# Alan-404/Conformer

Hardware: AMD Instinct MI355X
Metric: encoder audio-frames/sec (B=32,T=1000,d=512,L=16) (higher is better)
Workload: dtype f32; 1 GPU; cfg2 Conformer-L Encoder.forward: B=32/GPU, T=1000 mel frames (T'=249), d=512, 16 blocks, 8 heads, k=31, fp32, eval, random-init weights, batch-sharded replicas; per_gpu_batch=32, mel_frames=1000

## Files before the change

conformer_amd/_lib.py:

```python
from __future__ import annotations

import ctypes
import os
from ctypes import c_char_p, c_float, c_int, c_int64, c_uint64, c_void_p

_HERE = os.path.dirname(os.path.abspath(__file__))
LIB_PATH = os.environ.get("CONFORMER_AMD_LIB") or os.path.join(_HERE, "lib", "libconformer_hip.so")

_P, _I, _L, _F, _U = c_void_p, c_int, c_int64, c_float, c_uint64
ABI_VERSION = 4

SIGNATURES = {
    "cfm_version": (c_int, []),
    "cfm_abi_version": (c_int, []),
    "cfm_gemm_bias_stats_f32": (c_int, [_P, _P, _P, _P, _P, _L, _I, _I, _L, _L, _P]),
    "cfm_gemm_bias_residual_stats_f32": (c_int, [_P, _P, _P, _P, _F, _P, _P, _L, _I, _I, _L, _L, _L, _P]),
    "cfm_gemm_splitk_f32": (c_int, [_I, _P, _P, _P, _P, _F, _P, _P, _I, _L, _I, _I, _L, _L, _L, _P]),
    "cfm_gemm_lnfold_f32": (c_int, [_I, _P, _P, _I, _F, _P, _P, _P, _P, _L, _I, _I, _L, _L, _P]),
    "cfm_layernorm_fwd_stats_f32": (c_int, [_P, _P, _P, _P, _P, _L, _I, _F, _P]),
    "cfm_ffn_pack_elems": (ctypes.c_int64, [_I, _I]),
    "cfm_ffn_pack_f32": (c_int, [_P, _P, _P, _I, _I, _P]),
    "cfm_rowgemm_pack_f32": (c_int, [_P, _P, _I, _I, _I, _P]),
    "cfm_rowchain_f32": (c_int, [_I, _I, _I, _I, _P, _L, _P, _P, _P, _L, _P, _L, _P, _I, _F, _P, _P, _P, _P, _F, _I, _P, _L, _P, _P, _P, _F,
                                 _P, _P, _P, _F, _P, _L, _L, _I, _P]),
    "cfm_ffn_tile_stride_f4": (ctypes.c_int64, [_I]),
    "cfm_ffn_rotate": (c_int, []),
    "cfm_ffn_fused_f32": (c_int, [_P, _L, _P, _I, _F, _P, _P, _P, _P, _F, _P, _L, _I, _P, _P, _P, _F, _L, _I, _I, _P]),
    "cfm_strerror": (c_char_p, [_I]),
    "cfm_device_check": (c_int, []),
    "cfm_subsampled_length": (c_int64, [_L]),
    "cfm_subsampled_lengths_i64": (c_int, [_P, _P, _I, _P]),
    "cfm_layernorm_fwd_f32": (c_int, [_P, _P, _P, _P, _P, _P, _L, _I, _F, _P]),
    "cfm_gemm_bias_f32": (c_int, [_P, _P, _P, _P, _L, _I, _I, _L, _L, _P]),
    "cfm_gemm_bias_swish_f32": (c_int, [_P, _P, _P, _P, _L, _I, _I, _L, _L, _P]),
    "cfm_gemm_bias_relu_f32": (c_int, [_P, _P, _P, _P, _L, _I, _I, _L, _L, _P]),
    "cfm_gemm_bias_glu_f32": (c_int, [_P, _P, _P, _P, _L, _I, _I, _L, _L, _P]),
    "cfm_gemm_bias_residual_f32": (c_int, [_P, _P, _P, _P, _F, _P, _L, _I, _I, _L, _L, _L, _P]),
    "cfm_gemm_mfma16_f32": (c_int, [_I, _I, _P, _I, _P, _I, _P, _P, _F, _P, _I, _P, _I, _L, _I, _I, _L, _L, _L, _F, _U, _P]),
    "cfm_layernorm_fwd_out16_f32": (c_int, [_I, _P, _P, _P, _P, _P, _P, _L, _I, _F, _P]),
    "cfm_cast16_f32": (c_int, [_I, _P, _P, _L, _P]),
    "cfm_cast16_multi_f32": (c_int, [_I, _P, _I, _P]),
    "cfm_relpos_attention_mfma16_f32": (c_int, [_I, _P, _P, _P, _L, _P, _L, _P, _P, _P, _P, _L, _P, _I, _I, _I, _I, _F, _U, _P]),
    "cfm_relpos_attention_rows_mfma16_f32": (c_int, [_I, _P, _P, _P, _L, _P, _L, _P, _P, _P, _P, _L, _I, _I, _I, _I, _I, _I, _P]),
    "cfm_relpos_attention_io16_mfma16_f32": (c_int, [_I, _P, _P, _P, _I, _L, _P, _L, _P, _P, _P, _P, _I, _L, _I, _I, _I, _I, _P]),
    "cfm_subsample_conv2_relu_mfma16_f32": (c_int, [_I, _P, _I, _P, _I, _P, _P, _I, _I, _I, _I, _I, _P]),
    "cfm_subsample_conv1_relu_out16_f32": (c_int, [_I, _P, _P, _P, _P, _I, _I, _I, _I, _P]),
    "cfm_gemm_bwd_batched_mfma16_f32": (c_int, [_I, _P, _I, _L, _P, _I, _I, _L, _P, _I, _L, _F, _P, _L, _I, _I, _I, _L, _I, _I, _I, _I,
                                                _L, _L, _L, _L, _L, _L, _F, _U, _I, _P]),
    "cfm_subsample_conv2_bwd_weight_mfma16_f32": (c_int, [_I, _P, _P, _P, _I, _I, _I, _I, _P]),
    "cfm_subsample_conv2_bwd_input_mfma16_f32": (c_int, [_I, _P, _P, _P, _I, _I, _I, _I, _P]),
    "cfm_subsample_conv2_rowtab_elems": (ctypes.c_int64, [_I, _I, _I]),
    "cfm_subsample_conv2_bwd_weight_h16_mfma16_f32": (c_int, [_I, _P, _I, _P, _P, _P, _P, _I, _I, _I, _I, _P]),
    "cfm_relu_bwd_out16_f32": (c_int, [_I, _P, _P, _P, _L, _P]),
    "cfm_dwconv_bn_swish_fwd_out16_f32": (c_int, [_I, _P, _P, _P, _P, _P, _P, _P, _F, _P, _I, _I, _I, _I, _P]),
    "cfm_glu_bwd_out16_f32": (c_int, [_I, _P, _P, _P, _L, _I, _P]),
    "cfm_subsample_conv2_bwd_input_fwdkernel_mfma16_f32": (c_int, [_I, _P, _I, _P, _P, _P, _I, _I, _I, _I, _P]),
    "cfm_subsample_conv2_bwd_input_fwdkernel_out16_mfma16_f32": (c_int, [_I, _P, _I, _P, _P, _P, _I, _I, _I, _I, _P]),
    "cfm_subsample_conv1_bwd_d16_f32": (c_int, [_I, _P, _P, _P, _P, _P, _P, _I, _I, _I, _I, _P]),
    "cfm_reflect_pad_f32": (c_int, [_P, _P, _I, _L, _I, _L, _P]),
    "cfm_power_mel_log_f32": (c_int, [_P, _L, _P, _P, _I, _I, _I, _I, _F, _P]),
    "cfm_power_mel_log_mfma_f32": (c_int, [_P, _L, _P, _P, _I, _I, _I, _I, _I, _F, _P]),
    "cfm_dft_frames_f32": (c_int, [_P, _P, _P, _L, _I, _I, _I, _P]),
    "cfm_specaugment_apply_f32": (c_int, [_P, _I, _I, _I, _P, _I, _F, _P]),
    "cfm_gemm_bias_swish_save_f32": (c_int, [_P, _P, _P, _P, _P, _L, _I, _I, _L, _L, _P]),
    "cfm_gemm_bwd_f32": (c_int, [_P, _I, _L, _P, _I, _L, _P, _L, _F, _P, _L, _I, _I, _L, _I, _P]),
    "cfm_gemm_bwd_batched_f32": (c_int, [_P, _I, _L, _P, _I, _L, _P, _L, _F, _P, _L, _I, _I, _L, _I, _I, _I, _I,
                                         _L, _L, _L, _L, _L, _L, _F, _U, _P]),
    "cfm_gemm_train_f32": (c_int, [_I, _P, _P, _P, _P, _F, _P, _P, _L, _I, _I, _L, _L, _L, _F, _U, _P]),
    "cfm_relpos_attention_train_f32": (c_int, [_P, _P, _P, _L, _P, _L, _P, _P, _P, _P, _L, _P, _I, _I, _I, _I, _F, _U, _P]),
    "cfm_dropout_f32": (c_int, [_P, _P, _L, _F, _U, _P]),
    "cfm_dropout_out16_f32": (c_int, [_I, _P, _P, _L, _F, _U, _P]),
    "cfm_layernorm_bwd_dx_f32": (c_int, [_P, _P, _P, _P, _P, _P, _P, _L, _I, _P]),
    "cfm_layernorm_bwd_params_f32": (c_int, [_P, _P, _P, _P, _P, _P, _L, _I, _P]),
    "cfm_layernorm_bwd_f32": (c_int, [_P, _P, _P, _P, _P, _P, _P, _P, _P, _L, _I, _P, ctypes.c_size_t, _P]),
    "cfm_layernorm_bwd_workspace_bytes": (ctypes.c_size_t, [_L, _I]),
    "cfm_colsum_f32": (c_int, [_P, _L, _L, _I, _F, _P, _P]),
    "cfm_glu_fwd_f32": (c_int, [_P, _P, _L, _I, _P]),
    "cfm_glu_bwd_f32": (c_int, [_P, _P, _P, _L, _I, _P]),
    "cfm_dwconv_bn_swish_bwd_f32": (c_int, [_P, _P, _P, _P, _P, _P, _P, _P, _F, _I, _P, _P, _P, _P, _P, _P,
                                            _I, _I, _I, _I, _P]),
    "cfm_dwconv_bn_stats_workspace_bytes": (ctypes.c_size_t, [_I, _I, _I]),
    "cfm_dwconv_bn_stats_f32": (c_int, [_P, _P, _P, _P, _P, _P, _P, _F, _I, _I, _I, _I, _P, ctypes.c_size_t, _P]),
    "cfm_debug_attention_bwd_trace_f32": (c_int, [_P]),
    "cfm_debug_attention_bwd_trace_mfma16": (c_int, [_P]),
    "cfm_debug_gemm_mfma16_trace": (c_int, [_P]),
    "cfm_debug_gemm_mfma16_force_tile": (c_int, [_I]),
    "cfm_debug_gemm_last_tile": (c_int, [_I, _P]),
    "cfm_relpos_attention_bwd_mfma16_f32": (c_int, [_I, _P, _P, _P, _L, _P, _L, _P, _P, _P, _P, _P, _L, _P, _P, _P, _P, _L, _P, _L,
                                                    _P, _P, _I, _I, _I, _I, _F, _U, _P]),
    "cfm_relpos_attention_bwd_f32": (c_int, [_P, _P, _P, _L, _P, _L, _P, _P, _P, _P, _P, _L, _P, _P, _P, _P, _L, _P, _L, _P, _P,
                                             _I, _I, _I, _I, _F, _U, _I, _P]),
    "cfm_relu_bwd_f32": (c_int, [_P, _P, _P, _L, _P]),
    "cfm_subsample_conv2_bwd_weight_f32": (c_int, [_P, _P, _P, _I, _I, _I, _I, _P]),
    "cfm_pack_conv2_weight_t_f32": (c_int, [_P, _P, _I, _P]),
    "cfm_subsample_conv2_bwd_input_f32": (c_int, [_P, _P, _P, _I, _I, _I, _I, _P]),
    "cfm_subsample_conv1_bwd_f32": (c_int, [_P, _P, _P, _P, _P, _P, _I, _I, _I, _I, _P]),
    "cfm_adam_step_f32": (c_int, [_P, _I, _F, _F, _F, _F, _F, _F, _P]),
    "cfm_greedy_ctc_decode_f32": (c_int, [_P, _P, _P, _P, _P, _I, _I, _I, _I, _I, _P]),
    "cfm_ctc_beam_workspace_bytes": (ctypes.c_size_t, [_I, _I, _I, _I]),
    "cfm_ctc_beam_decode_f32": (c_int, [_P, _P, _I, _I, _I, _I, _I, _I, _F, _F, _I, _P, ctypes.c_size_t, _P, _P, _P, _P, _P]),
    "cfm_ngram_lm_pack_bytes": (ctypes.c_size_t, [_I, _P, _I, _L, _I, _L]),
    "cfm_ngram_lm_pack": (c_int, [_I, _P, _P, _P, _P, _I, _P, _P, _I, _I, _I, _I, _P, _P, _P, _P, ctypes.c_size_t]),
    "cfm_ngram_lm_score_f64": (c_int, [_P, _P, _P, _I, _I, _P, _P]),
    "cfm_ctc_beam_lm_workspace_bytes": (ctypes.c_size_t, [_I, _I, _I, _I]),
    "cfm_ctc_beam_lm_decode_f32": (c_int, [_P, _P, _I, _I, _I, _I, _I, _I, _F, _F, _I, _P, ctypes.c_double, ctypes.c_double,
                                           ctypes.c_double, _I, _P, ctypes.c_size_t, _P, _P, _P, _P, _P, _P]),
    "cfm_hotword_pack_bytes": (ctypes.c_size_t, [_I, _L, _I, _L, _I, _L]),
    "cfm_hotword_pack": (c_int, [_I, _P, _P, _I, _P, _P, _I, _P, _P, _P, _P, ctypes.c_size_t]),
    "cfm_hotword_count": (c_int, [_P, _P, _P, _I, ctypes.c_double, _P, _P, _P]),
    "cfm_ctc_beam_hw_workspace_bytes": (ctypes.c_size_t, [_I, _I, _I, _I]),
    "cfm_ctc_beam_hw_decode_f32": (c_int, [_P, _P, _I, _I, _I, _I, _I, _I, _F, _F, _I, _P, ctypes.c_double, ctypes.c_double,
                                           ctypes.c_double, _I, _P, ctypes.c_double, _P, ctypes.c_size_t, _P, _P, _P, _P, _P,
                                           _P]),
    "cfm_ctc_beam_stream_state_bytes": (ctypes.c_size_t, [_I, _I, _I, _I, _I, _I]),
    "cfm_ctc_beam_stream_init": (c_int, [_I, _I, _I, _I, _P, _I, _P, _P, ctypes.c_size_t, _P]),
    "cfm_ctc_beam_stream_step_f32": (c_int, [_P, _P, _I, _I, _I, _I, _I, _I, _F, _F, _I, _P, ctypes.c_double, ctypes.c_double,
                                             ctypes.c_double, _I, _P, ctypes.c_double, _P, ctypes.c_size_t, _I, _I, _P, _P, _P,
                                             _P, _P, _P]),
    "cfm_ctc_beam_stream_finish_f32": (c_int, [_I, _I, _I, _I, _P, ctypes.c_double, ctypes.c_double, ctypes.c_double, _I, _P,
                                               ctypes.c_double, _P, ctypes.c_size_t, _I, _P, _P, _P, _P, _P, _P]),
    "cfm_ctc_beam_stream_reset_slots": (c_int, [_I, _I, _I, _I, _P, _I, _P, _P, _I, _P, ctypes.c_size_t, _P]),
    "cfm_lstm_fwd_carry_f32": (c_int, [_P, _P, _P, _P, _P, _P, _P, _P, _I, _I, _I, _P]),
    "cfm_lstm_fwd_frag_carry_f32": (c_int, [_P, _P, _P, _P, _P, _P, _P, _P, _P, _I, _I, _I, _P]),
    "cfm_lstm_fwd_mfma16_carry_f32": (c_int, [_I, _P, _P, _P, _P, _P, _P, _P, _P, _P, _I, _I, _I, _P]),
    "cfm_lstm_fwd_f32": (c_int, [_P, _P, _P, _P, _P, _P, _P, _I, _I, _I, _P]),
    "cfm_lstm_fwd_frag_f32": (c_int, [_P, _P, _P, _P, _P, _P, _P, _P, _I, _I, _I, _P]),
    "cfm_lstm_bwd_frag_f32": (c_int, [_P, _P, _P, _P, _P, _P, _P, _P, _I, _I, _I, _P]),
    "cfm_debug_lstm_trace": (c_int, [_P]),
    "cfm_debug_dw16_trace": (c_int, [_P]),
    "cfm_linear_bwd_weight_mfma16_f32": (c_int, [_I, _P, _I, _L, _P, _I, _L, _P, _L, _P, _I, _I, _L, _F, _P]),
    "cfm_lstm_fwd_mfma16_f32": (c_int, [_I, _P, _P, _P, _P, _P, _P, _P, _P, _I, _I, _I, _P]),
    "cfm_lstm_bwd_mfma16_f32": (c_int, [_I, _P, _P, _P, _P, _P, _P, _P, _P, _I, _I, _I, _P]),
    "cfm_lstm_bwd_f32": (c_int, [_P, _P, _P, _P, _P, _P, _P, _I, _I, _I, _P]),
    "cfm_swish_bn_eval_f32": (c_int, [_P, _P, _P, _P, _P, _F, _P, _L, _I, _P]),
    "cfm_swish_bn_stats_f32": (c_int, [_P, _P, _P, _P, _P, _F, _L, _I, _P]),
    "cfm_swish_bn_bwd_f32": (c_int, [_P, _P, _P, _P, _P, _F, _I, _P, _P, _P, _L, _I, _P]),
    "cfm_split_pack_elems": (ctypes.c_int64, [_I, _I, _I]),
    "cfm_split_pack_bf16_f32": (c_int, [_I, _P, _P, _I, _I, _P]),
    "cfm_gemm_split_bf16_f32": (c_int, [_I, _I, _P, _P, _P, _P, _F, _P, _L, _I, _I, _L, _L, _L, _P]),
    "cfm_subsample_conv2_relu_split_bf16_f32": (c_int, [_I, _P, _P, _P, _P, _I, _I, _I, _I, _P]),
    "cfm_ctc_workspace_floats": (ctypes.c_int64, [_I, _I, _I]),
    "cfm_ctc_loss_fwd_f32": (c_int, [_P, _P, _P, _L, _L, _P, _P, _I, _I, _I, _I, _I, _P, _P, _P]),
    "cfm_ctc_loss_bwd_f32": (c_int, [_P, _P, _P, _L, _L, _P, _P, _I, _I, _I, _I, _I, _P, _P, _P, _P]),
    "cfm_ctc_align_workspace_bytes": (ctypes.c_size_t, [_I, _I, _I]),
    "cfm_ctc_align_f32": (c_int, [_P, _P, _P, _P, _I, _I, _I, _I, _I, _P, ctypes.c_size_t, _P, _P, _P, _P, _P, _P, _P, _P]),
    "cfm_relpos_attention_rows_f32": (c_int, [_P, _P, _P, _L, _P, _L, _P, _P, _P, _P, _L, _I, _I, _I, _I, _I, _I, _I, _P, _P]),
    "cfm_relpos_attention_slots_f32": (c_int, [_P, _P, _P, _L, _P, _L, _P, _P, _P, _P, _P, _P, _L, _I, _I, _I, _I, _I, _I, _P, _P]),
    "cfm_relpos_attention_slots_mfma16_f32": (c_int, [_I, _P, _P, _P, _I, _L, _P, _L, _P, _P, _P, _P, _P, _P, _L, _I, _I, _I, _I, _I, _I,
                                                      _P, _P]),
    "cfm_debug_attention_trace_f32": (c_int, [_P, _P, _P, _L, _P, _L, _P, _P, _P, _P, _L, _I, _I, _I, _I, _P, _P]),
    "cfm_debug_set_bwd_tile": (c_int, [_I]),
    "cfm_debug_set_attention_waves": (c_int, [_I]),
    "cfm_debug_gemm_cfg_f32": (c_int, [_I, _P, _P, _P, _P, _F, _P, _L, _I, _I, _P, _P]),
    "cfm_debug_set_conv2_bk": (c_int, [_I]),
    "cfm_debug_ffn_trace": (c_int, [_P, _I]),
    "cfm_debug_ffn_variant": (c_int, [_I]),
    "cfm_debug_ffn_layout": (c_int, [_I, _I]),
    "cfm_relpos_table_f32": (c_int, [_P, _P, _I, _I, _P]),
    "cfm_relpos_attention_fwd_f32": (c_int, [_P, _P, _P, _L, _P, _L, _P, _P, _P, _P, _L, _P, _I, _I, _I, _I, _P]),
    "cfm_dwconv_bn_swish_fwd_f32": (c_int, [_P, _P, _P, _P, _P, _P, _P, _F, _P, _I, _I, _I, _I, _P]),
    "cfm_convmod_glu_dwconv_f32": (c_int, [_P, _L, _P, _I, _F, _P, _P, _P, _P, _P, _P, _P, _P, _P, _F, _P, _L, _I, _I, _I, _I, _P]),
    "cfm_debug_convmod_variant": (c_int, [_I]),
    "cfm_subsample_conv1_relu_f32": (c_int, [_P, _P, _P, _P, _I, _I, _I, _I, _P]),
    "cfm_pack_conv2_weight_f32": (c_int, [_P, _P, _I, _P]),
    "cfm_subsample_conv2_relu_f32": (c_int, [_P, _P, _P, _P, _I, _I, _I, _I, _P]),
    "cfm_pack_linear_weight_f32": (c_int, [_P, _P, _I, _I, _I, _P]),
    "cfm_conv2_wino_plane_elems": (c_int64, [_I, _I, _I, _I]),
    "cfm_pack_conv2_wino_weight_f32": (c_int, [_P, _P, _I, _P]),
    "cfm_subsample_conv2_wino_relu_f32": (c_int, [_P, _P, _P, _P, _P, _I, _I, _I, _I, _P]),
}


class ConformerHipError(RuntimeError):
    pass


_lib = None


def load() -> ctypes.CDLL:
    global _lib
    if _lib is not None:
        return _lib
    if not os.path.exists(LIB_PATH):
        raise ConformerHipError(
            f"{LIB_PATH} is missing: build it with `python -m conformer_amd.build` "
            "(there is no CPU/eager fallback for the Conformer hot path)")
    import torch
    lib = ctypes.CDLL(LIB_PATH, mode=ctypes.RTLD_GLOBAL)
    try:
        lib.cfm_abi_version.restype = c_int
        got = int(lib.cfm_abi_version())
    except AttributeError:
        got = 0
    if got != ABI_VERSION:
        raise ConformerHipError(f"{LIB_PATH} implements C-ABI revision {got}, this binding needs {ABI_VERSION}: rebuild it with "
                                "`python -m conformer_amd.build`")
    for name, (res, args) in SIGNATURES.items():
        fn = getattr(lib, name)
        fn.restype = res
        fn.argtypes = args
    _lib = lib
    return lib


class CastItem(ctypes.Structure):
    _fields_ = [("src", ctypes.c_void_p), ("dst", ctypes.c_void_p), ("rows", ctypes.c_int64), ("cols", ctypes.c_int64),
                ("transpose", ctypes.c_int)]


CALLS = [0]


def check(status: int, what: str) -> None:
    CALLS[0] += 1
    if status != 0:
        msg = load().cfm_strerror(status).decode()
        raise ConformerHipError(f"{what} failed: {msg} (status {status})")
```

conformer_amd/csrc/conv2_wino_f32.hip:

```cpp
#include <algorithm>
#include <utility>

#include "gemm_shared.h"

namespace {

#define WINO_MFMA_SLICE(FA, FB)                                                                             \
    _Pragma("unroll") for (int e = 0; e < 4; ++e)                                                           \
    _Pragma("unroll") for (int mt = 0; mt < TM; ++mt)                                                       \
    _Pragma("unroll") for (int nt = 0; nt < TN; ++nt)                                                       \
        acc[mt][nt] = __builtin_amdgcn_mfma_f32_32x32x2f32(FB[nt][e], FA[mt][e], acc[mt][nt], 0, 0, 0)

template <typename Fn, int... I>
__device__ __forceinline__ void static_for_seq(Fn& f, std::integer_sequence<int, I...>) {
    (f(std::integral_constant<int, I>{}), ...);
}
template <int N, typename Fn>
__device__ __forceinline__ void static_for(Fn&& f) {
    static_for_seq(f, std::make_integer_sequence<int, N>{});
}

__host__ __device__ constexpr int wino_nt(int a) { return a == 1 ? 1 : 2; }
__host__ __device__ constexpr int wino_terms(int p) { return wino_nt(p / 3) * wino_nt(p % 3); }

struct WinoArgs {
    const float* h1; const float* w; float* planes;
    int64_t M;
    unsigned h1_bytes;
    int T1, F1, C, TI, TJ, nb;
    int odd_t, odd_f;
    unsigned tiles_n;
    unsigned grp_blk[4];
    unsigned grp_tm[3][4];
    unsigned grp_pat[3];
};


template <int ST, int SF>
__device__ __forceinline__ void wino_tile(const WinoArgs& g, int p, int64_t m0, int n0, float* lds) {
    constexpr int BM = 256, BN = 256, WN = 4, TM = 4, TN = 2, BK = 16, LDSR = BK + 4, NT = ST * SF, SPC = 2 * NT;
    constexpr int NPX = (ST == 2 ? 2 : 1) * (SF == 2 ? 2 : 1);
    float* As = lds;
    float* Bs = lds + 2 * BM * LDSR;
    const int a = p / 3, b = p - 3 * (p / 3);
    const int sg_t = a >> 1, sg_f = b >> 1;

    const int tid = threadIdx.x, lane = tid & 63;
    const int wave = __builtin_amdgcn_readfirstlane(tid >> 6);
    const int wr = wave / WN, wc = wave % WN;
    const int li = lane & 31, hf = lane >> 5;

    constexpr int CPR = BK / 4, RPP = 512 / CPR, PA = BM / RPP, PB = BN / RPP;
    const int chunk = tid & (CPR - 1), srow = tid / CPR;
    unsigned row_off[PA];
    const int TJp = g.TJ - (b == 2 ? g.odd_f : 0);
    const int64_t pos_per_b = (int64_t)(g.TI - (a == 2 ? g.odd_t : 0)) * TJp, Mp = g.nb * pos_per_b;
#pragma unroll
    for (int i = 0; i < PA; ++i) {
        int64_t m = m0 + srow + RPP * i;
        if (m >= Mp) m = Mp - 1;
        const int64_t bb = m / pos_per_b;
        const int r = (int)(m - bb * pos_per_b);
        const int ib = r / TJp, jb = r - ib * TJp;
        row_off[i] = (unsigned)((((bb * g.T1 + 4 * ib) * g.F1 + 4 * jb) * (int64_t)g.C + chunk * 4) * 4);
    }
    const __amdgpu_buffer_rsrc_t h1_rsrc = __builtin_amdgcn_make_buffer_rsrc(const_cast<float*>(g.h1), (short)0, (int)g.h1_bytes, 0x00020000);
    const unsigned pix_t[3] = {(unsigned)((ST == 2 ? 4 * sg_t : 2) * g.F1 * g.C * 4), (unsigned)(2 * g.F1 * g.C * 4),
                               (unsigned)((1 + 2 * sg_t) * g.F1 * g.C * 4)};
    const unsigned pix_f[3] = {(unsigned)((SF == 2 ? 4 * sg_f : 2) * g.C * 4), (unsigned)(2 * g.C * 4), (unsigned)((1 + 2 * sg_f) * g.C * 4)};
    int64_t woff = 0;
    for (int q = 0; q < p; ++q) woff += wino_terms(q);
    const int K = NT * g.C;
    const __amdgpu_buffer_rsrc_t w_rsrc = __builtin_amdgcn_make_buffer_rsrc(const_cast<float*>(g.w + woff * g.C * g.C), (short)0,
                                                                            K * g.C * 4, 0x00020000);
    const unsigned w_off = (unsigned)(((n0 + srow) * K + chunk * 4) * 4), w_step = (unsigned)(RPP * K * 4);

    f32x4 raw[PA][NPX], rb[PB];
    auto load_tile = [&](auto U_, int c32, int half) __attribute__((always_inline)) {
        constexpr int U = decltype(U_)::value, UT = U / SF, UF = U % SF;
        constexpr int NXT = (ST == 2 && UT == 0) ? 2 : 1, NYF = (SF == 2 && UF == 0) ? 2 : 1;
        constexpr int X1 = ST == 2 ? (UT == 0 ? 0 : 2) : 0, Y1 = SF == 2 ? (UF == 0 ? 0 : 2) : 0;
        const unsigned ci4 = (unsigned)(32 * c32 + 16 * half) * 4;
#pragma unroll
        for (int x = 0; x < NXT; ++x)
#pragma unroll
            for (int y = 0; y < NYF; ++y) {
                const unsigned po = pix_t[X1 + x] + pix_f[Y1 + y] + ci4;
#pragma unroll
                for (int i = 0; i < PA; ++i)
                    raw[i][x * NYF + y] = __builtin_bit_cast(f32x4, __builtin_amdgcn_raw_buffer_load_b128(h1_rsrc, row_off[i], po, 0));
            }
        const unsigned k4 = (unsigned)(NT * 32 * c32 + 32 * U + 16 * half) * 4;
#pragma unroll
        for (int i = 0; i < PB; ++i) rb[i] = __builtin_bit_cast(f32x4, __builtin_amdgcn_raw_buffer_load_b128(w_rsrc, w_off, k4 + w_step * i, 0));
    };
    auto store_tile = [&](auto U_, int buf) __attribute__((always_inline)) {
        constexpr int U = decltype(U_)::value, UT = U / SF, UF = U % SF;
        constexpr int NXT = (ST == 2 && UT == 0) ? 2 : 1, NYF = (SF == 2 && UF == 0) ? 2 : 1;
#pragma unroll
        for (int i = 0; i < PA; ++i) {
            const f32x4* px = raw[i];
            f32x4 v;
            if constexpr (NXT == 2 && NYF == 2) v = (px[0] - px[1]) - (px[2] - px[3]);
            else if constexpr (NXT * NYF == 2) v = px[0] - px[1];
            else v = px[0];
            *reinterpret_cast<f32x4*>(As + (buf * BM + srow + RPP * i) * LDSR + chunk * 4) = v;
        }
#pragma unroll
        for (int i = 0; i < PB; ++i)
            *reinterpret_cast<f32x4*>(Bs + (buf * BN + srow + RPP * i) * LDSR + chunk * 4) = rb[i];
    };

    f32x16 acc[TM][TN];
#pragma unroll
    for (int i = 0; i < TM; ++i)
#pragma unroll
        for (int j = 0; j < TN; ++j)
#pragma unroll
            for (int r = 0; r < 16; ++r) acc[i][j][r] = 0.f;

    const int a_row = wr * (BM / 2) + li, b_row = wc * (BN / WN) + li;
    f32x4 fa0[TM], fb0[TN], fa1[TM], fb1[TN];
    auto read_frags = [&](f32x4 (&fa)[TM], f32x4 (&fb)[TN], int buf, int c) __attribute__((always_inline)) {
#pragma unroll
        for (int t = 0; t < TM; ++t)
            fa[t] = *reinterpret_cast<const f32x4*>(As + (buf * BM + a_row + 32 * t) * LDSR + 8 * c + 4 * hf);
#pragma unroll
        for (int t = 0; t < TN; ++t)
            fb[t] = *reinterpret_cast<const f32x4*>(Bs + (buf * BN + b_row + 32 * t) * LDSR + 8 * c + 4 * hf);
    };

    const int nch = g.C / 32;
    load_tile(std::integral_constant<int, 0>{}, 0, 0);
    store_tile(std::integral_constant<int, 0>{}, 0);
    load_tile(std::integral_constant<int, 0>{}, 0, 1);
    __syncthreads();
    read_frags(fa0, fb0, 0, 0);
    for (int c32 = 0; c32 < nch; ++c32) {
        static_for<SPC>([&](auto S_) __attribute__((always_inline)) {
            constexpr int S = decltype(S_)::value;
            constexpr int S1 = (S + 1) % SPC, S2 = (S + 2) % SPC;
            const int cur = S & 1;
            const bool more = S + 1 < SPC || c32 + 1 < nch;
            read_frags(fa1, fb1, cur, 1);
            __builtin_amdgcn_sched_barrier(0);
            WINO_MFMA_SLICE(fa0, fb0);
            __builtin_amdgcn_sched_barrier(0);
            if (more) store_tile(std::integral_constant<int, S1 / 2>{}, cur ^ 1);
            load_tile(std::integral_constant<int, S2 / 2>{}, S + 2 < SPC ? c32 : min(c32 + 1, nch - 1), S2 & 1);
            __syncthreads();
            if (more) read_frags(fa0, fb0, cur ^ 1, 0);
            __builtin_amdgcn_sched_barrier(0);
            WINO_MFMA_SLICE(fa1, fb1);
            __builtin_amdgcn_sched_barrier(0);
        });
    }

    __syncthreads();
    GemmArgs ge{};
    ge.C = g.planes + (int64_t)p * g.M * g.C;
    ge.M = Mp; ge.N = g.C; ge.K = K; ge.ldc = g.C; ge.alpha = 1.f;
    gemm_epilogue_rows<BM, BN, EPI_BIAS, TM, TN, 2, false, EPF_INFER | EPF_NO_BIAS, WN>(ge, acc, m0, n0, wr, wc, lane,
                                                                                        lds + wave * 32 * (32 * TN + 4));
}

__global__ __launch_bounds__(512, 2) void conv2_wino_gemm_kernel(const WinoArgs g) {
    constexpr int LDS_STAGE = 2 * (256 + 256) * 20;
    static_assert(8 * 32 * (32 * 2 + 4) <= LDS_STAGE, "the row-major epilogue scratch must fit the staging buffers");
    __shared__ __attribute__((aligned(16))) float lds[LDS_STAGE];
    const unsigned bid = blockIdx.x;
    const int grp = bid < g.grp_blk[1] ? 0 : (bid < g.grp_blk[2] ? 1 : 2);
    const unsigned local = bid - g.grp_blk[grp], per_xcd = (g.grp_blk[grp + 1] - g.grp_blk[grp]) / 8;
    unsigned tile = (local & 7u) * per_xcd + (local >> 3);
    unsigned k = 0, lo = 0;
    for (; k < 4; ++k) {
        const unsigned seg = (g.grp_tm[grp][k] - lo) * (4 - k) * g.tiles_n;
        if (tile < seg) break;
        tile -= seg;
        lo = g.grp_tm[grp][k];
    }
    if (k == 4) return;
    const unsigned tn = tile % g.tiles_n, rest = tile / g.tiles_n;
    const unsigned pi = k + rest % (4 - k), tm = lo + rest / (4 - k);
    const int p = (int)((g.grp_pat[grp] >> (4 * pi)) & 15u);
    const int64_t m0 = (int64_t)tm * 256;
    const int n0 = (int)tn * 256;
    const int nta = wino_nt(p / 3), ntb = wino_nt(p % 3);
    if (nta == 2 && ntb == 2) wino_tile<2, 2>(g, p, m0, n0, lds);
    else if (nta == 2) wino_tile<2, 1>(g, p, m0, n0, lds);
    else if (ntb == 2) wino_tile<1, 2>(g, p, m0, n0, lds);
    else wino_tile<1, 1>(g, p, m0, n0, lds);
}

__global__ __launch_bounds__(256) void conv2_wino_combine_kernel(const float* __restrict__ planes, const float* __restrict__ b2,
                                                                 float* __restrict__ h2, int64_t M, int T2, int F2, int TI,
                                                                 int TJ, int C) {
    const int c4n = C / 4;
    const int64_t idx = (int64_t)blockIdx.x * blockDim.x + threadIdx.x;
    if (idx >= M * c4n) return;
    const int64_t m = idx / c4n;
    const int c = (int)(idx - m * c4n) * 4;
    const int64_t per_b = (int64_t)TI * TJ;
    const int64_t bb = m / per_b;
    const int r = (int)(m - bb * per_b);
    const int ib = r / TJ, jb = r - ib * TJ;
    const int64_t plane = M * (int64_t)C;
    const int TIs = TI - (T2 & 1), TJs = TJ - (F2 & 1);
    f32x4 P[9];
#pragma unroll
    for (int q = 0; q < 9; ++q) {
        const bool st = q / 3 == 2, sf = q % 3 == 2;
        const int64_t mq = (bb * (st ? TIs : TI) + ib) * (sf ? TJs : TJ) + jb;
        P[q] = f32x4{0.f, 0.f, 0.f, 0.f};
        if ((!st || ib < TIs) && (!sf || jb < TJs))
            P[q] = __builtin_nontemporal_load(reinterpret_cast<const f32x4*>(planes + q * plane + mq * C + c));
    }
    const f32x4 bias = *reinterpret_cast<const f32x4*>(b2 + c);
#pragma unroll
    for (int rt = 0; rt < 2; ++rt) {
        const int t2 = 2 * ib + rt;
        if (t2 >= T2) continue;
        const f32x4 u0 = P[3 * rt + 0] + P[3 * rt + 1], u1 = P[3 * rt + 1] + P[3 * rt + 2];
        const f32x4 v0 = P[3 * rt + 3] + P[3 * rt + 4], v1 = P[3 * rt + 4] + P[3 * rt + 5];
#pragma unroll
        for (int s = 0; s < 2; ++s) {
            const int f2 = 2 * jb + s;
            if (f2 >= F2) continue;
            const f32x4 y = (s == 0 ? u0 + v0 : u1 + v1) + bias;
            f32x4 o;
#pragma unroll
            for (int e = 0; e < 4; ++e) o[e] = fmaxf(y[e], 0.f);
            *reinterpret_cast<f32x4*>(h2 + (((bb * T2 + t2) * F2) + f2) * (int64_t)C + c) = o;
        }
    }
}

__global__ __launch_bounds__(256) void pack_conv2_wino_kernel(const float* __restrict__ w2, float* __restrict__ wp, int C) {
    const int p = blockIdx.y, nt = wino_terms(p);
    const int64_t idx = (int64_t)blockIdx.x * blockDim.x + threadIdx.x;
    const int64_t K = (int64_t)nt * C;
    if (idx >= K * C) return;
    const int64_t co = idx / K;
    const int k = (int)(idx - co * K);
    const int c32 = k / (32 * nt), rem = k - c32 * 32 * nt, u = rem / 32, ci = 32 * c32 + (rem & 31);
    int64_t off = 0;
    for (int q = 0; q < p; ++q) off += wino_terms(q);
    const int a = p / 3, b = p % 3, sfn = wino_nt(b);
    const int ut = u / sfn, uf = u % sfn;
    auto taps = [](int pat, int term, int (&tp)[2]) {
        if (pat == 1) { tp[0] = 0; tp[1] = 2; return 2; }
        tp[0] = term == 0 ? 2 * (pat >> 1) : 1;
        return 1;
    };
    int tt[2], tf[2];
    const int ntt = taps(a, ut, tt), ntf = taps(b, uf, tf);
    double s = 0.0;
    const float* wc = w2 + (co * C + ci) * 9;
    for (int x = 0; x < ntt; ++x)
        for (int y = 0; y < ntf; ++y) s += (double)wc[tf[y] * 3 + tt[x]];
    wp[off * C * C + idx] = (float)s;
}

}

extern "C" int64_t cfm_conv2_wino_plane_elems(int B, int F1, int T1, int C) {
    if (B <= 0 || F1 < 3 || T1 < 3 || C <= 0) return 0;
    const int64_t TI = ((T1 - 1) / 2 + 1) / 2, TJ = ((F1 - 1) / 2 + 1) / 2;
    return 9 * (int64_t)B * TI * TJ * C;
}

extern "C" int cfm_pack_conv2_wino_weight_f32(const float* w2, float* wp, int C, cfm_stream_t stream) {
    CFM_REQUIRE(w2 && wp, CFM_ERR_NULL);
    CFM_REQUIRE(C > 0 && C % 32 == 0, CFM_ERR_BAD_SHAPE);
    const int64_t most = 4 * (int64_t)C * C;
    hipLaunchKernelGGL(pack_conv2_wino_kernel, dim3((unsigned)((most + 255) / 256), 9), dim3(256), 0,
                       static_cast<hipStream_t>(stream), w2, wp, C);
    return cfm_launch_status();
}

extern "C" int cfm_subsample_conv2_wino_relu_f32(const float* h1, const float* wp, const float* b2, float* planes, float* h2,
                                                 int B, int F1, int T1, int C, cfm_stream_t stream) {
    CFM_REQUIRE(h1 && wp && b2 && planes && h2, CFM_ERR_NULL);
    CFM_REQUIRE(B > 0 && F1 >= 3 && T1 >= 3, CFM_ERR_BAD_SHAPE);
    CFM_REQUIRE(C > 0 && C % 256 == 0, CFM_ERR_UNSUPPORTED);
    CFM_REQUIRE(CFM_ALIGNED16(h1) && CFM_ALIGNED16(wp) && CFM_ALIGNED16(b2) && CFM_ALIGNED16(planes) && CFM_ALIGNED16(h2),
                CFM_ERR_ALIGN);
    const int64_t utt_bytes = (int64_t)T1 * F1 * C * 4, limit = (1LL << 32) - (1LL << 26);
    CFM_REQUIRE(utt_bytes <= limit && 5LL * F1 * C * 4 < (1LL << 26), CFM_ERR_UNSUPPORTED);
    const int T2 = (T1 - 1) / 2, F2 = (F1 - 1) / 2;
    WinoArgs g{};
    g.w = wp;
    g.T1 = T1; g.F1 = F1; g.C = C; g.TI = (T2 + 1) / 2; g.TJ = (F2 + 1) / 2;
    g.odd_t = T2 & 1; g.odd_f = F2 & 1;
    g.tiles_n = (unsigned)(C / 256);
    const int64_t per_b = (int64_t)g.TI * g.TJ;
    const int group = (int)std::min<int64_t>(B, limit / utt_bytes);
    hipStream_t s = static_cast<hipStream_t>(stream);
    for (int b0 = 0; b0 < B; b0 += group) {
        const int nb = std::min(group, B - b0);
        g.h1 = h1 + b0 * (utt_bytes / 4);
        g.h1_bytes = (unsigned)(nb * utt_bytes);
        g.M = nb * per_b;
        g.nb = nb;
        g.planes = planes + 9 * (b0 * per_b) * C;
        static const int group_pat[3][4] = {{0, 2, 6, 8}, {1, 7, 3, 5}, {-1, -1, -1, 4}};
        g.grp_blk[0] = 0;
        for (int q = 0; q < 3; ++q) {
            int pat[4];
            unsigned tm[4], total = 0;
            for (int i = 0; i < 4; ++i) {
                const int p = group_pat[q][i];
                const int64_t Mp = p < 0 ? 0 : (int64_t)nb * (g.TI - (p / 3 == 2 ? g.odd_t : 0)) * (g.TJ - (p % 3 == 2 ? g.odd_f : 0));
                const unsigned t = (unsigned)((Mp + 255) / 256);
                int j = i;
                for (; j > 0 && tm[j - 1] > t; --j) { tm[j] = tm[j - 1]; pat[j] = pat[j - 1]; }
                tm[j] = t; pat[j] = p < 0 ? 0 : p;
                total += t;
            }
            g.grp_pat[q] = 0;
            for (int i = 0; i < 4; ++i) { g.grp_tm[q][i] = tm[i]; g.grp_pat[q] |= (unsigned)pat[i] << (4 * i); }
            g.grp_blk[q + 1] = g.grp_blk[q] + (total * g.tiles_n + 7) / 8 * 8;
        }
        hipLaunchKernelGGL(conv2_wino_gemm_kernel, dim3(g.grp_blk[3]), dim3(512), 0, s, g);
        int st = cfm_launch_status();
        if (st) return st;
        const int64_t threads = g.M * (C / 4);
        hipLaunchKernelGGL(conv2_wino_combine_kernel, dim3((unsigned)((threads + 255) / 256)), dim3(256), 0, s, g.planes, b2,
                           h2 + (int64_t)b0 * T2 * F2 * C, g.M, T2, F2, g.TI, g.TJ, C);
        st = cfm_launch_status();
        if (st) return st;
    }
    return 0;
}
```

conformer_amd/model/utils/convolution.py:

```python
from typing import Optional, Tuple

import torch
import torch.nn as nn
import torch.nn.functional as F

from ... import autograd as ag
from ... import ops
from ._guard import PackCache, active_dropout, refuse_dropout
from .activation import GLU, Swish


class ConvolutionModule(nn.Module):
    def __init__(self, channels: int, kernel_size: int, dropout_rate: float = 0.0) -> None:
        super().__init__()
        self.layer_norm = nn.LayerNorm(normalized_shape=channels)
        self.pointwise_conv_1 = nn.Conv1d(channels, channels * 2, kernel_size=1)
        self.glu = GLU(dim=1)
        self.deepwise_conv = nn.Conv1d(channels, channels, kernel_size=kernel_size, padding=(kernel_size - 1) // 2,
                                       groups=channels)
        self.batch_norm = nn.BatchNorm1d(num_features=channels)
        self.swish = Swish()
        self.pointwise_conv_2 = nn.Conv1d(channels, channels, kernel_size=1)
        self.dropout = nn.Dropout(p=dropout_rate)
        self._packs = PackCache()

    def depthwise_eval(self, g: torch.Tensor, for_gemm: bool = False) -> torch.Tensor:
        bn = self.batch_norm
        return ops.dwconv_bn_swish(g, self.deepwise_conv.weight, self.deepwise_conv.bias, bn.weight, bn.bias,
                                   bn.running_mean, bn.running_var, bn.eps, for_gemm=for_gemm)

    def fused(self, x: torch.Tensor, residual: Optional[torch.Tensor] = None, stats: Optional[torch.Tensor] = None,
              emit_stats: bool = False, stream=None):
        refuse_dropout(self, "ConvolutionModule")
        bn = self.batch_norm
        train_bn = bn.training or bn.running_mean is None
        if train_bn and (bn.momentum is None or not bn.track_running_stats):
            raise NotImplementedError("ConvolutionModule: only the default BatchNorm1d(momentum=0.1, "
                                      "track_running_stats=True) is built")
        if train_bn and not ag.needs_grad(self, x, residual):
            h = ops.layernorm(x, self.layer_norm.weight, self.layer_norm.bias, self.layer_norm.eps, for_gemm=True)
            g = ops.linear_glu(h, self.pointwise_conv_1.weight, self.pointwise_conv_1.bias)
            bm, bv = ops.dwconv_bn_batch_stats(g, self.deepwise_conv.weight, self.deepwise_conv.bias, bn.running_mean,
                                               bn.running_var, bn.momentum)
            bn.num_batches_tracked += 1
            s = ops.dwconv_bn_swish(g, self.deepwise_conv.weight, self.deepwise_conv.bias, bn.weight, bn.bias, bm, bv,
                                    bn.eps, for_gemm=True)
            if residual is None:
                return ops.linear(s, self.pointwise_conv_2.weight, self.pointwise_conv_2.bias)
            return ops.linear_residual(s, self.pointwise_conv_2.weight, self.pointwise_conv_2.bias, residual, 1.0)
        if ag.needs_grad(self, x, residual):
            if residual is not None and residual is not x:
                raise NotImplementedError("ConvolutionModule.fused: pass residual=x (block.py:23)")
            out = ag.ConvModuleFn.apply(x, self.layer_norm.weight, self.layer_norm.bias, self.pointwise_conv_1.weight,
                                        self.pointwise_conv_1.bias, self.deepwise_conv.weight, self.deepwise_conv.bias,
                                        bn.weight, bn.bias, bn.running_mean, bn.running_var,
                                        self.pointwise_conv_2.weight, self.pointwise_conv_2.bias,
                                        self.layer_norm.eps, bn.eps, train_bn, bn.momentum if train_bn else 0.0,
                                        active_dropout(self.dropout))
            if train_bn:
                bn.num_batches_tracked += 1
            return out if residual is not None else out - x
        if stats is not None:
            ln, pw1 = self.layer_norm, self.pointwise_conv_1
            wf, bf, cs = self._packs.get("ln_fold", (pw1.weight, pw1.bias, ln.weight, ln.bias),
                                         lambda: ops.fold_layernorm(pw1.weight, pw1.bias, ln.weight, ln.bias))
            dw = self.deepwise_conv
            if stream is None and x.dim() == 3 and ops.convmod_fused_ok(x.shape[0], x.shape[1], x.shape[2], dw.weight.shape[-1]):
                g = None
                s = ops.convmod_glu_dwconv(x, stats, wf, bf, cs, ln.eps, dw.weight, dw.bias, bn.weight, bn.bias, bn.running_mean,
                                           bn.running_var, bn.eps)
            else:
                g = ops.linear_lnfold(x, stats, wf, bf, cs, ln.eps, glu=True)
        else:
            h = ops.layernorm(x, self.layer_norm.weight, self.layer_norm.bias, self.layer_norm.eps, for_gemm=stream is None)
            g = ops.linear_glu(h, self.pointwise_conv_1.weight, self.pointwise_conv_1.bias)
        if g is not None:
            s = self.depthwise_eval(g, for_gemm=True) if stream is None else stream.depthwise(self, g)
        if residual is None:
            if emit_stats:
                return ops.linear(s, self.pointwise_conv_2.weight, self.pointwise_conv_2.bias, emit_stats=True)
            return ops.linear(s, self.pointwise_conv_2.weight, self.pointwise_conv_2.bias)
        return ops.linear_residual(s, self.pointwise_conv_2.weight, self.pointwise_conv_2.bias, residual, 1.0, emit_stats=emit_stats)

    def forward(self, x: torch.Tensor) -> torch.Tensor:
        return self.fused(x)


class ConvolutionSubsampling(nn.Module):
    def __init__(self, channels: int) -> None:
        super().__init__()
        self.conv_1 = nn.Conv2d(1, channels, kernel_size=3, stride=2)
        self.act_1 = nn.ReLU()
        self.conv_2 = nn.Conv2d(channels, channels, kernel_size=3, stride=2)
        self.act_2 = nn.ReLU()
        self._packs = PackCache()

    @staticmethod
    def out_lengths(lengths: Optional[torch.Tensor]) -> Optional[torch.Tensor]:
        if lengths is None:
            return None
        if lengths.is_cuda and lengths.dtype == torch.int64:
            return ops.subsampled_lengths(lengths)
        return torch.div(torch.div(lengths - 1, 2, rounding_mode="floor") - 1, 2, rounding_mode="floor")

    def channel_last(self, x: torch.Tensor) -> torch.Tensor:
        if ag.needs_grad(self, x):
            if x.requires_grad:
                raise NotImplementedError("ConvolutionSubsampling: the gradient w.r.t. the input spectrogram is not "
                                          "built (the reference never needs it: the input is data)")
            return ag.SubsampleStemFn.apply(x, self.conv_1.weight, self.conv_1.bias, self.conv_2.weight, self.conv_2.bias)
        w2p = self._packs.get("w2p", (self.conv_2.weight,), lambda: ops.pack_conv2_weight(self.conv_2.weight))
        w2w = None
        if ops.conv2_winograd_ok(self.conv_2.weight.shape[0]):
            w2w = self._packs.get("w2w", (self.conv_2.weight,), lambda: ops.pack_conv2_wino_weight(self.conv_2.weight))
        return ops.subsample_stem(x, self.conv_1.weight, self.conv_1.bias, w2p, self.conv_2.bias, w2w=w2w)

    def forward(self, x: torch.Tensor, lengths: Optional[torch.Tensor] = None) -> Tuple[torch.Tensor, Optional[torch.Tensor]]:
        h = self.channel_last(x)
        if h.dtype != torch.float32:
            h = h.float()
        B, T2, _ = h.shape
        C = self.conv_1.out_channels
        h = h.view(B, T2, -1, C).transpose(2, 3).reshape(B, T2, -1)
        return h, self.out_lengths(lengths)


class DepthWiseSeperableConvolution(nn.Module):

    def __init__(self, in_channels: int, out_channels: int) -> None:
        super().__init__()
        self.depth_wise_conv = nn.Conv2d(in_channels, out_channels, kernel_size=3, stride=2, groups=in_channels)
        self.point_wise_conv = nn.Conv2d(out_channels, out_channels, kernel_size=1)

    def forward(self, x: torch.Tensor):
        return self.point_wise_conv(self.depth_wise_conv(x))


class DownsamplingConvolution(nn.Module):

    def __init__(self, channels: int) -> None:
        super().__init__()
        self.conv_1 = DepthWiseSeperableConvolution(1, channels)
        self.conv_2 = DepthWiseSeperableConvolution(channels, channels)

    def forward(self, x: torch.Tensor, lengths: Optional[torch.Tensor]):
        h = F.relu(self.conv_2(F.relu(self.conv_1(x.unsqueeze(1)))))
        B, C, Fp, Tp = h.shape
        h = h.permute(0, 3, 1, 2).reshape(B, Tp, C * Fp)
        return h, ConvolutionSubsampling.out_lengths(lengths)
```

conformer_amd/ops.py:

```python
from __future__ import annotations

import threading
import ctypes
from typing import Optional, Tuple

import torch

from . import _lib
from ._derived import DerivedCache


def _stream() -> int:
    return torch.cuda.current_stream().cuda_stream


def _req(t: torch.Tensor, name: str, dtype=torch.float32) -> torch.Tensor:
    if not isinstance(t, torch.Tensor) or not t.is_cuda:
        raise _lib.ConformerHipError(
            f"{name}: expected a tensor on a HIP device, got {getattr(t, 'device', type(t))}; "
            "the Conformer hot path only exists as gfx950 kernels (no CPU fallback)")
    if t.dtype != dtype:
        raise _lib.ConformerHipError(f"{name}: expected dtype {dtype}, got {t.dtype}")
    return t if t.is_contiguous() else t.contiguous()


def _p(t: Optional[torch.Tensor]) -> Optional[int]:
    return None if t is None else t.data_ptr()


def _f32_like(t: torch.Tensor) -> torch.Tensor:
    return torch.empty(t.shape, device=t.device, dtype=torch.float32)


PREC_F32, PREC_BF16, PREC_FP16 = 0, 1, 2
_DT16 = {PREC_BF16: torch.bfloat16, PREC_FP16: torch.float16}
_tls = threading.local()


def mfma16_prec() -> int:
    forced = getattr(_tls, "forced", None)
    if forced is not None:
        return forced
    if not torch.is_autocast_enabled("cuda"):
        return PREC_F32
    dt = torch.get_autocast_dtype("cuda")
    if dt == torch.bfloat16:
        return PREC_BF16
    if dt == torch.float16:
        return PREC_FP16
    raise _lib.ConformerHipError(f"autocast dtype {dt} is not supported by the gfx950 path")


class precision:

    def __init__(self, prec: int) -> None:
        self.prec, self.prev = prec, None

    def __enter__(self):
        self.prev = getattr(_tls, "forced", None)
        _tls.forced = self.prec
        return self

    def __exit__(self, *exc):
        _tls.forced = self.prev
        return False


def bf16_mfma_active() -> bool:
    return mfma16_prec() == PREC_BF16


_WEIGHT_COPIES = DerivedCache()
def weight16(w: torch.Tensor, prec: int, transposed: bool = False) -> Optional[torch.Tensor]:
    if w.shape[-1] % 8 or w.numel() % 4 or (transposed and w.shape[0] % 8):
        return None
    def make() -> torch.Tensor:
        if transposed:
            out = torch.empty(w.shape[1], w.shape[0], device=w.device, dtype=_DT16[prec])
            item = (_lib.CastItem * 1)()
            item[0].src, item[0].dst, item[0].rows, item[0].cols, item[0].transpose = w.data_ptr(), out.data_ptr(), w.shape[0], w.shape[1], 1
            _lib.check(_lib.load().cfm_cast16_multi_f32(prec, ctypes.addressof(item), 1, _stream()), "cfm_cast16_multi_f32")
        else:
            out = torch.empty(w.shape, device=w.device, dtype=_DT16[prec])
            _lib.check(_lib.load().cfm_cast16_f32(prec, w.data_ptr(), out.data_ptr(), w.numel(), _stream()), "cfm_cast16_f32")
        return out
    return _WEIGHT_COPIES.get((w.data_ptr(), transposed), (w,), make, extra=prec)


def refresh_weight16(params) -> int:
    by_prec = {}
    def queue(p, transposed, prec, shape2, out) -> bool:
        ok = len(shape2) == 2 and shape2[0] * shape2[1] == p.numel() and p.is_contiguous()
        if ok:
            by_prec.setdefault(prec, []).append((p.detach().reshape(shape2), out, transposed))
        return ok
    for p in params:
        for t in (False, True):
            _WEIGHT_COPIES.refresh((p.data_ptr(), t), (p,), lambda prec, shapes, out: queue(p, t, prec, shapes[0], out))
    n = 0
    for prec, items in by_prec.items():
        arr = (_lib.CastItem * len(items))()
        for i, (w2, out, transposed) in enumerate(items):
            arr[i].src, arr[i].dst = w2.data_ptr(), out.data_ptr()
            arr[i].rows, arr[i].cols, arr[i].transpose = w2.shape[0], w2.shape[1], int(transposed)
        _lib.check(_lib.load().cfm_cast16_multi_f32(prec, ctypes.addressof(arr), len(items), _stream()), "cfm_cast16_multi_f32")
        n += len(items)
    return n


_ZERO_BIAS = {}


def _zero_bias(n: int, device) -> torch.Tensor:
    t = _ZERO_BIAS.get((n, device))
    if t is None:
        t = _ZERO_BIAS[(n, device)] = torch.zeros(n, device=device, dtype=torch.float32)
    return t


_FP32_MATMUL = {"native": 0, "bf16x6": 3, "bf16x3": 2}
_fp32_planes = _FP32_MATMUL[__import__("os").environ.get("CONFORMER_AMD_FP32_MATMUL", "native")]


def set_fp32_matmul(mode: str) -> str:
    global _fp32_planes
    if mode not in _FP32_MATMUL:
        raise ValueError(f"fp32 matmul mode must be one of {sorted(_FP32_MATMUL)}, got {mode!r}")
    prev = fp32_matmul()
    _fp32_planes = _FP32_MATMUL[mode]
    return prev


def fp32_matmul() -> str:
    return {v: k for k, v in _FP32_MATMUL.items()}[_fp32_planes]


def weight_split(w: torch.Tensor, planes: int) -> Optional[torch.Tensor]:
    if w.dim() != 2 or w.shape[1] % 16:
        return None
    def make() -> torch.Tensor:
        lib = _lib.load()
        n, k = w.shape
        out = torch.empty(int(lib.cfm_split_pack_elems(planes, n, k)), device=w.device, dtype=torch.bfloat16)
        _lib.check(lib.cfm_split_pack_bf16_f32(planes, w.data_ptr(), out.data_ptr(), n, k, _stream()), "cfm_split_pack_bf16_f32")
        return out
    return _WEIGHT_COPIES.get((w.data_ptr(), "split"), (w,), make, extra=planes)


def unpack_weight_split(packed: torch.Tensor, planes: int, n: int, k: int) -> torch.Tensor:
    nb, ks = (n + 31) // 32, k // 16
    p = packed.view(nb, ks, planes, 2, 32, 8)
    return p.permute(2, 0, 4, 1, 3, 5).reshape(planes, nb * 32, k)[:, :n]


def _split_gemm(epi: int, a, w2, b, c, m, n, k, res=None, alpha: float = 1.0):
    if not _fp32_planes or a.dtype != torch.float32 or c.dtype != torch.float32:
        return None
    ws = weight_split(w2, _fp32_planes) if (epi != 3 or n % 32 == 0) else None
    if ws is None:
        return None
    _lib.check(_lib.load().cfm_gemm_split_bf16_f32(_fp32_planes, epi, a.data_ptr(), ws.data_ptr(), b.data_ptr(), _p(res), alpha,
                                                   c.data_ptr(), m, n, k, k, n, n, _stream()), "cfm_gemm_split_bf16_f32")
    return c


def out16_ok(k: int) -> int:
    prec = mfma16_prec()
    return prec if prec and k % 8 == 0 else 0


def _mfma16_gemm(prec: int, epi: int, a, w2, b, c, m, n, k, res=None, alpha: float = 1.0, z=None, drop_p: float = 0.0,
                 seed: int = 0):
    w16 = weight16(w2, prec)
    a16 = a.dtype != torch.float32
    if a16 and (w16 is None or a.dtype != _DT16[prec]):
        raise _lib.ConformerHipError(f"16-bit A operand ({a.dtype}) does not match the precision mode / weight shape")
    st = _lib.load().cfm_gemm_mfma16_f32(prec, epi, a.data_ptr(), int(a16), (w2 if w16 is None else w16).data_ptr(),
                                         int(w16 is not None), b.data_ptr(), _p(res), alpha, c.data_ptr(),
                                         int(c.dtype != torch.float32), _p(z), int(z is not None and z.dtype != torch.float32),
                                         m, n, k, k, n, n, float(drop_p), int(seed), _stream())
    _lib.check(st, "cfm_gemm_mfma16_f32")
    return c


def subsampled_length(n: int) -> int:
    return int(_lib.load().cfm_subsampled_length(int(n)))


def subsampled_lengths(lengths: torch.Tensor) -> torch.Tensor:
    lengths = _req(lengths, "lengths", torch.int64)
    out = torch.empty(lengths.shape, device=lengths.device, dtype=torch.int64)
    if lengths.numel():
        _lib.check(_lib.load().cfm_subsampled_lengths_i64(lengths.data_ptr(), out.data_ptr(), lengths.numel(), _stream()),
                   "cfm_subsampled_lengths_i64")
    return out


_LN_FOLD = __import__("os").environ.get("CONFORMER_AMD_LN_FOLD", "1") != "0"


def set_ln_fold(on: bool) -> bool:
    global _LN_FOLD
    prev, _LN_FOLD = _LN_FOLD, bool(on)
    return prev


def ln_fold_ok(d: int) -> bool:
    return bool(_LN_FOLD and not _fp32_planes and mfma16_prec() == PREC_F32 and d in (32, 64, 128, 256, 512))


def fold_layernorm(w: torch.Tensor, b: torch.Tensor, gamma: torch.Tensor, beta: torch.Tensor):
    w2 = w.detach().reshape(w.shape[0], -1)
    wf = (w2 * gamma.detach()[None, :]).contiguous()
    bf = (b.detach().double() + w2.double() @ beta.detach().double()).float().contiguous()
    cs = wf.double().sum(dim=1).float().contiguous()
    return wf, bf, cs


def linear_lnfold(a, stats, wf, bf, cs, eps: float, act: str = "none", glu: bool = False) -> torch.Tensor:
    a = _req(a, "A"); wf = _req(wf, "Wf"); bf = _req(bf, "bias_f"); cs = _req(cs, "colsum"); stats = _req(stats, "ln_stats")
    k = a.shape[-1]
    m = a.numel() // k
    n = wf.shape[0] // 2 if glu else wf.shape[0]
    if wf.shape[1] != k or stats.dim() != 3 or stats.shape[0] != m or stats.shape[2] != 2:
        raise _lib.ConformerHipError(f"linear_lnfold: A(...,{k}), Wf{tuple(wf.shape)}, stats{tuple(stats.shape)} do not match")
    c = torch.empty(*a.shape[:-1], n, device=a.device, dtype=torch.float32)
    epi = 3 if glu else {"none": 0, "swish": 1}[act]
    _lib.check(_lib.load().cfm_gemm_lnfold_f32(epi, a.data_ptr(), stats.data_ptr(), stats.shape[1], float(eps), wf.data_ptr(),
                                               bf.data_ptr(), cs.data_ptr(), c.data_ptr(), m, n, k, k, n, _stream()),
               "cfm_gemm_lnfold_f32")
    return c


_FFN_FUSED = __import__("os").environ.get("CONFORMER_AMD_FFN_FUSED", "1") != "0"


def set_ffn_fused(on: bool) -> bool:
    global _FFN_FUSED
    prev, _FFN_FUSED = _FFN_FUSED, bool(on)
    return prev


def ffn_fused_ok(d: int, hidden: int, rows: int) -> bool:
    if not (_FFN_FUSED and ln_fold_ok(d) and d in (128, 256, 512) and hidden % 128 == 0):
        return False
    blocks = (rows + 31) // 32
    rounds = (blocks + 255) // 256
    return blocks >= 0.9 * 256 * rounds


_FFN_LAYOUT_ENV = __import__("os").environ.get("CONFORMER_AMD_FFN_ROTATE")


def ffn_pack(w1f: torch.Tensor, w2: torch.Tensor) -> torch.Tensor:
    w1f = _req(w1f, "W1f"); w2 = _req(w2, "W2")
    hidden, d = w1f.shape
    if tuple(w2.shape) != (d, hidden):
        raise _lib.ConformerHipError(f"ffn_pack: W1f{tuple(w1f.shape)} and W2{tuple(w2.shape)} do not match")
    lib = _lib.load()
    if _FFN_LAYOUT_ENV is not None:
        lib.cfm_debug_ffn_layout(-1, int(_FFN_LAYOUT_ENV))
    wp = torch.zeros(int(lib.cfm_ffn_pack_elems(d, hidden)), device=w1f.device, dtype=torch.float32)
    _lib.check(lib.cfm_ffn_pack_f32(w1f.data_ptr(), w2.data_ptr(), wp.data_ptr(), d, hidden, _stream()), "cfm_ffn_pack_f32")
    return wp


def ffn_fused(x: torch.Tensor, stats: torch.Tensor, wp: torch.Tensor, b1f: torch.Tensor, cs: torch.Tensor, b2: torch.Tensor,
              alpha: float, eps: float, emit_stats: bool = False, closing_ln=None):
    x = _req(x, "x"); stats = _req(stats, "ln_stats"); wp = _req(wp, "Wp"); b1f = _req(b1f, "b1f"); cs = _req(cs, "colsum")
    b2 = _req(b2, "b2")
    d = x.shape[-1]
    rows = x.numel() // d
    hidden = b1f.numel()
    if stats.dim() != 3 or stats.shape[0] != rows or stats.shape[2] != 2 or wp.numel() != int(_lib.load().cfm_ffn_pack_elems(d, hidden)) or b2.numel() != d:
        raise _lib.ConformerHipError(f"ffn_fused: x(...,{d}), stats{tuple(stats.shape)}, Wp({wp.numel()}), hidden {hidden} do not match")
    y = torch.empty(x.shape, device=x.device, dtype=torch.float32)
    st_out, g2, bt2, eps2, mode = None, None, None, 0.0, 0
    if closing_ln is not None:
        g2 = _req(closing_ln[0], "ln.weight"); bt2 = _req(closing_ln[1], "ln.bias"); eps2 = float(closing_ln[2]); mode = 2
        if emit_stats:
            st_out = torch.empty(rows, 1, 2, device=x.device, dtype=torch.float32)
    elif emit_stats:
        mode = 1
        st_out = torch.empty(rows, d // 32, 2, device=x.device, dtype=torch.float32)
    _lib.check(_lib.load().cfm_ffn_fused_f32(x.data_ptr(), d, stats.data_ptr(), stats.shape[1], float(eps), wp.data_ptr(),
                                             b1f.data_ptr(), cs.data_ptr(), b2.data_ptr(), float(alpha), y.data_ptr(), d, mode,
                                             None if st_out is None else st_out.data_ptr(),
                                             None if g2 is None else g2.data_ptr(), None if bt2 is None else bt2.data_ptr(),
                                             eps2, rows, d, hidden, _stream()), "cfm_ffn_fused_f32")
    return (y, st_out) if emit_stats else y


_ROWCHAIN = __import__("os").environ.get("CONFORMER_AMD_ROWCHAIN", "0") == "1"


def set_rowchain(on: bool) -> bool:
    global _ROWCHAIN
    prev, _ROWCHAIN = _ROWCHAIN, bool(on)
    return prev


def rowchain_ok(d: int, hidden: int, rows: int) -> bool:
    return bool(_ROWCHAIN and ffn_fused_ok(d, hidden, rows))


def rowgemm_pack(w: torch.Tensor, glu: bool = False) -> torch.Tensor:
    w = _req(w.reshape(w.shape[0], -1), "W")
    n, d = w.shape
    wp = torch.empty(n * d, device=w.device, dtype=torch.float32)
    _lib.check(_lib.load().cfm_rowgemm_pack_f32(w.data_ptr(), wp.data_ptr(), n, d, 1 if glu else 0, _stream()), "cfm_rowgemm_pack_f32")
    return wp


def _rowchain(pre, core, post, mode, x, d, *, wpre=None, bpre=None, res=None, y1=None, stats=None, ln_eps=0.0, ffn=None, b2=None,
              alpha=0.0, y=None, stats_out=None, ln2=None, wpost=None, bpost=None, cspost=None, post_eps=0.0, z=None):
    rows = x.numel() // d
    ptr = lambda t: None if t is None else t.data_ptr()
    wp, b1f, cs1 = ffn if ffn is not None else (None, None, None)
    hidden = 0 if b1f is None else b1f.numel()
    g2, bt2, eps2 = ln2 if ln2 is not None else (None, None, 0.0)
    st = _lib.load().cfm_rowchain_f32(pre, core, post, mode, x.data_ptr(), d, ptr(wpre), ptr(bpre), ptr(res), d, ptr(y1), d,
                                      ptr(stats), 0 if stats is None else stats.shape[1], float(ln_eps), ptr(wp), ptr(b1f), ptr(cs1),
                                      ptr(b2), float(alpha), hidden, ptr(y), d, ptr(stats_out), ptr(g2), ptr(bt2), float(eps2),
                                      ptr(wpost), ptr(bpost), ptr(cspost), float(post_eps), ptr(z), 0 if z is None else z.shape[-1],
                                      rows, d, _stream())
    _lib.check(st, "cfm_rowchain_f32")


def rowchain_ffn_qkv(x, stats, ffn, b2, alpha: float, ffn_eps: float, wqkv_p, bqkv_f, csqkv, att_eps: float):
    x = _req(x, "x"); stats = _req(stats, "ln_stats")
    d = x.shape[-1]
    y = torch.empty(x.shape, device=x.device, dtype=torch.float32)
    qkv = torch.empty(*x.shape[:-1], 3 * d, device=x.device, dtype=torch.float32)
    _rowchain(0, 1, 1, 0, x, d, stats=stats, ln_eps=ffn_eps, ffn=ffn, b2=_req(b2, "b2"), alpha=alpha, y=y, wpost=wqkv_p,
              bpost=bqkv_f, cspost=csqkv, post_eps=att_eps, z=qkv)
    return y, qkv


def rowchain_out_glu(ctx, wout_p, bout, res, wglu_p, bglu_f, csglu, conv_eps: float):
    ctx = _req(ctx, "ctx"); res = _req(res, "residual")
    d = ctx.shape[-1]
    y2 = torch.empty(ctx.shape, device=ctx.device, dtype=torch.float32)
    g = torch.empty(ctx.shape, device=ctx.device, dtype=torch.float32)
    _rowchain(1, 0, 2, 0, ctx, d, wpre=wout_p, bpre=_req(bout, "bias"), res=res, y1=y2, ln_eps=conv_eps, wpost=wglu_p, bpost=bglu_f,
              cspost=csglu, z=g)
    return y2, g


def rowchain_pw2_ffn_ln(c, wpw2_p, bpw2, res, ffn, b2, alpha: float, ffn_eps: float, closing_ln, want_stats: bool = False):
    c = _req(c, "c"); res = _req(res, "residual")
    d = c.shape[-1]
    out = torch.empty(c.shape, device=c.device, dtype=torch.float32)
    st = torch.empty(c.numel() // d, 1, 2, device=c.device, dtype=torch.float32) if want_stats else None
    _rowchain(1, 1, 0, 2, c, d, wpre=wpw2_p, bpre=_req(bpw2, "bias"), res=res, ln_eps=ffn_eps, ffn=ffn, b2=_req(b2, "b2"), alpha=alpha,
              y=out, stats_out=st, ln2=(_req(closing_ln[0], "ln.weight"), _req(closing_ln[1], "ln.bias"), float(closing_ln[2])))
    return out, st


def layernorm(x: torch.Tensor, weight: torch.Tensor, bias: torch.Tensor, eps: float = 1e-5,
              out: Optional[torch.Tensor] = None, for_gemm: bool = False, emit_stats: bool = False):
    x = _req(x, "x"); weight = _req(weight, "weight"); bias = _req(bias, "bias")
    d = x.shape[-1]
    rows = x.numel() // d
    if emit_stats:
        y = torch.empty(x.shape, device=x.device, dtype=torch.float32)
        stats = torch.empty(rows, 1, 2, device=x.device, dtype=torch.float32)
        _lib.check(_lib.load().cfm_layernorm_fwd_stats_f32(x.data_ptr(), weight.data_ptr(), bias.data_ptr(), y.data_ptr(),
                                                           stats.data_ptr(), rows, d, eps, _stream()), "cfm_layernorm_fwd_stats_f32")
        return y, stats
    p16 = out16_ok(d) if for_gemm and out is None else 0
    if p16:
        y = torch.empty(x.shape, device=x.device, dtype=_DT16[p16])
        _lib.check(_lib.load().cfm_layernorm_fwd_out16_f32(p16, x.data_ptr(), weight.data_ptr(), bias.data_ptr(), y.data_ptr(),
                                                           None, None, rows, d, eps, _stream()), "cfm_layernorm_fwd_out16_f32")
        return y
    y = _f32_like(x) if out is None else _req(out, "out")
    if y.shape != x.shape:
        raise _lib.ConformerHipError(f"layernorm: out{tuple(y.shape)} does not match x{tuple(x.shape)}")
    st = _lib.load().cfm_layernorm_fwd_f32(x.data_ptr(), weight.data_ptr(), bias.data_ptr(), y.data_ptr(),
                                           None, None, rows, d, eps, _stream())
    _lib.check(st, "cfm_layernorm_fwd_f32")
    return y


def _gemm_common(a: torch.Tensor, w: torch.Tensor, b: torch.Tensor):
    a = _req(a, "A", a.dtype if isinstance(a, torch.Tensor) and a.dtype in _DT16.values() else torch.float32)
    w = _req(w, "W"); b = _req(b, "bias")
    k = a.shape[-1]
    m = a.numel() // k
    w2 = w.reshape(w.shape[0], -1)
    if w2.shape[1] != k:
        raise _lib.ConformerHipError(f"GEMM shape mismatch: A(...,{k}) vs W{tuple(w.shape)}")
    return a, w2, b, m, w2.shape[0], k


def _splitk(m: int, n: int, k: int) -> int:
    tiles = ((m + 63) // 64) * ((n + 63) // 64)
    if tiles > 192 or k < 1024 or n % 4 or m < 1:
        return 0
    return max(2, min(8, k // 512, -(-768 // tiles)))


def _splitk_gemm(epi: int, a, w2, b, c, m, n, k, res=None, alpha: float = 1.0):
    sp = _splitk(m, n, k)
    if not sp or a.dtype != torch.float32 or c.dtype != torch.float32 or _fp32_planes or mfma16_prec():
        return None
    ws = torch.empty(sp * m * n, device=a.device, dtype=torch.float32)
    _lib.check(_lib.load().cfm_gemm_splitk_f32(epi, a.data_ptr(), w2.data_ptr(), b.data_ptr(), _p(res), alpha, c.data_ptr(),
                                               ws.data_ptr(), sp, m, n, k, k, n, n, _stream()), "cfm_gemm_splitk_f32")
    return c


def linear(a, w, b, act: str = "none", for_gemm: bool = False, emit_stats: bool = False):
    a, w2, b, m, n, k = _gemm_common(a, w, b)
    if emit_stats:
        if act != "none" or not ln_fold_ok(n) or a.dtype != torch.float32:
            raise _lib.ConformerHipError("linear(emit_stats=True) needs the native fp32 path, act='none' and ln_fold_ok(N)")
        c = torch.empty(*a.shape[:-1], n, device=a.device, dtype=torch.float32)
        stats = torch.empty(m, n // 32, 2, device=a.device, dtype=torch.float32)
        _lib.check(_lib.load().cfm_gemm_bias_stats_f32(a.data_ptr(), w2.data_ptr(), b.data_ptr(), c.data_ptr(), stats.data_ptr(),
                                                       m, n, k, k, n, _stream()), "cfm_gemm_bias_stats_f32")
        return c, stats
    prec = mfma16_prec()
    p16 = out16_ok(n) if for_gemm else 0
    c = torch.empty(*a.shape[:-1], n, device=a.device, dtype=_DT16[p16] if p16 else torch.float32)
    if prec:
        return _mfma16_gemm(prec, {"none": 0, "swish": 1, "relu": 2}[act], a, w2, b, c, m, n, k)
    if _split_gemm({"none": 0, "swish": 1, "relu": 2}[act], a, w2, b, c, m, n, k) is not None:
        return c
    if act != "relu" and _splitk_gemm({"none": 0, "swish": 1}[act], a, w2, b, c, m, n, k) is not None:
        return c
    fn = {"none": "cfm_gemm_bias_f32", "swish": "cfm_gemm_bias_swish_f32", "relu": "cfm_gemm_bias_relu_f32"}[act]
    st = getattr(_lib.load(), fn)(a.data_ptr(), w2.data_ptr(), b.data_ptr(), c.data_ptr(), m, n, k, k, n, _stream())
    _lib.check(st, fn)
    return c


def linear_glu(a, w, b) -> torch.Tensor:
    a, w2, b, m, n2, k = _gemm_common(a, w, b)
    n = n2 // 2
    c = torch.empty(*a.shape[:-1], n, device=a.device, dtype=torch.float32)
    prec = mfma16_prec()
    if prec:
        return _mfma16_gemm(prec, 3, a, w2, b, c, m, n, k)
    if _split_gemm(3, a, w2, b, c, m, n, k) is not None:
        return c
    st = _lib.load().cfm_gemm_bias_glu_f32(a.data_ptr(), w2.data_ptr(), b.data_ptr(), c.data_ptr(), m, n, k, k, n,
                                           _stream())
    _lib.check(st, "cfm_gemm_bias_glu_f32")
    return c


def linear_residual(a, w, b, res: torch.Tensor, alpha: float = 1.0, emit_stats: bool = False):
    a, w2, b, m, n, k = _gemm_common(a, w, b)
    res = _req(res, "residual")
    if emit_stats:
        if not ln_fold_ok(n) or a.dtype != torch.float32:
            raise _lib.ConformerHipError("linear_residual(emit_stats=True) needs the native fp32 path and ln_fold_ok(N)")
        c = torch.empty(*a.shape[:-1], n, device=a.device, dtype=torch.float32)
        stats = torch.empty(m, n // 32, 2, device=a.device, dtype=torch.float32)
        _lib.check(_lib.load().cfm_gemm_bias_residual_stats_f32(a.data_ptr(), w2.data_ptr(), b.data_ptr(), res.data_ptr(), alpha,
                                                                c.data_ptr(), stats.data_ptr(), m, n, k, k, n, n, _stream()),
                   "cfm_gemm_bias_residual_stats_f32")
        return c, stats
    c = torch.empty(*a.shape[:-1], n, device=a.device, dtype=torch.float32)
    prec = mfma16_prec()
    if prec:
        return _mfma16_gemm(prec, 4, a, w2, b, c, m, n, k, res, alpha)
    if _split_gemm(4, a, w2, b, c, m, n, k, res, alpha) is not None:
        return c
    if _splitk_gemm(4, a, w2, b, c, m, n, k, res, alpha) is not None:
        return c
    st = _lib.load().cfm_gemm_bias_residual_f32(a.data_ptr(), w2.data_ptr(), b.data_ptr(), res.data_ptr(), alpha,
                                                c.data_ptr(), m, n, k, k, n, n, _stream())
    _lib.check(st, "cfm_gemm_bias_residual_f32")
    return c


def relpos_table(div_term: torch.Tensor, t: int) -> torch.Tensor:
    dt = _req(div_term, "div_term").reshape(-1)
    d = 2 * dt.numel()
    pe = torch.empty(2 * t - 1, d, device=dt.device, dtype=torch.float32)
    st = _lib.load().cfm_relpos_table_f32(dt.data_ptr(), pe.data_ptr(), t, d, _stream())
    _lib.check(st, "cfm_relpos_table_f32")
    return pe


def _req_pos(pos: torch.Tensor, T: int, d: int) -> None:
    if not (isinstance(pos, torch.Tensor) and pos.is_cuda and pos.dtype == torch.float32 and pos.dim() == 2
            and pos.stride(1) == 1 and pos.shape == (2 * T - 1, d)):
        raise _lib.ConformerHipError(f"pos: expected a ({2 * T - 1},{d}) fp32 HIP tensor with unit column stride")


def _key_split(B: int, n_heads: int, q_rows: int, T: int, keys_hint: Optional[int]) -> int:
    tiles = ((T if keys_hint is None else min(int(keys_hint), T)) + 31) // 32
    blocks = B * n_heads * ((q_rows + 127) // 128)
    return max(1, min(16, tiles // 8, -(-1024 // blocks)))


def _key_split16(B: int, n_heads: int, q_rows: int, T: int, keys_hint: Optional[int]) -> int:
    tiles = ((T if keys_hint is None else min(int(keys_hint), T)) + 31) // 32
    blocks = B * n_heads * ((q_rows + 127) // 128)
    return max(1, min(16, tiles // 8, 512 // blocks))


def relpos_attention(qkv: torch.Tensor, pos: torch.Tensor, u: torch.Tensor, v: torch.Tensor,
                     lengths: Optional[torch.Tensor], n_heads: int, for_gemm: bool = False) -> torch.Tensor:
    u = _req(u, "content_bias"); v = _req(v, "position_bias")
    prec = mfma16_prec()
    q16 = bool(prec) and isinstance(qkv, torch.Tensor) and qkv.dtype == _DT16[prec]
    if q16:
        if not (qkv.is_cuda and qkv.is_contiguous() and qkv.shape[-1] % 24 == 0):
            raise _lib.ConformerHipError("16-bit qkv: expected a contiguous HIP tensor with d % 8 == 0")
    else:
        qkv = _req(qkv, "qkv")
    B, T, d3 = qkv.shape
    d = d3 // 3
    dh = d // n_heads
    _req_pos(pos, T, d)
    ldp = pos.stride(0)
    if lengths is not None:
        lengths = _req(lengths, "lengths", torch.int64)
    base = qkv.data_ptr()
    c16 = bool(prec and for_gemm and d % 8 == 0)
    if q16 or c16:
        esz = 2 if q16 else 4
        ctx = torch.empty(B, T, d, device=qkv.device, dtype=_DT16[prec] if c16 else torch.float32)
        st = _lib.load().cfm_relpos_attention_io16_mfma16_f32(prec, base, base + esz * d, base + 2 * esz * d, int(q16), d3,
                                                              pos.data_ptr(), ldp, u.data_ptr(), v.data_ptr(), _p(lengths),
                                                              ctx.data_ptr(), int(c16), d, B, T, n_heads, dh, _stream())
        _lib.check(st, "cfm_relpos_attention_io16_mfma16_f32")
        return ctx
    ctx = torch.empty(B, T, d, device=qkv.device, dtype=torch.float32)
    if prec:
        st = _lib.load().cfm_relpos_attention_mfma16_f32(prec, base, base + 4 * d, base + 8 * d, d3, pos.data_ptr(), ldp,
                                                         u.data_ptr(), v.data_ptr(), _p(lengths), ctx.data_ptr(), d, None,
                                                         B, T, n_heads, dh, 0.0, 0, _stream())
        _lib.check(st, "cfm_relpos_attention_mfma16_f32")
        return ctx
    st = _lib.load().cfm_relpos_attention_fwd_f32(base, base + 4 * d, base + 8 * d, d3, pos.data_ptr(), ldp,
                                                  u.data_ptr(), v.data_ptr(), _p(lengths), ctx.data_ptr(), d, None,
                                                  B, T, n_heads, dh, _stream())
    _lib.check(st, "cfm_relpos_attention_fwd_f32")
    return ctx


def relpos_attention_rows(qkv: torch.Tensor, pos: torch.Tensor, u: torch.Tensor, v: torch.Tensor, lengths: torch.Tensor,
                          n_heads: int, q_begin: int, q_count: int, ctx: torch.Tensor, keys_hint: Optional[int] = None
                          ) -> torch.Tensor:
    qkv = _req(qkv, "qkv"); u = _req(u, "content_bias"); v = _req(v, "position_bias"); ctx = _req(ctx, "ctx")
    B, T, d3 = qkv.shape
    d = d3 // 3
    _req_pos(pos, T, d)
    if ctx.shape != (B, T, d) or not qkv.is_contiguous() or not ctx.is_contiguous():
        raise _lib.ConformerHipError("relpos_attention_rows: qkv (B,T,3d) and ctx (B,T,d) must be contiguous cache buffers")
    lengths = _req(lengths, "lengths", torch.int64)
    prec = mfma16_prec()
    if prec != PREC_F32:
        base = qkv.data_ptr()
        st = _lib.load().cfm_relpos_attention_rows_mfma16_f32(prec, base, base + 4 * d, base + 8 * d, d3, pos.data_ptr(), pos.stride(0),
                                                              u.data_ptr(), v.data_ptr(), lengths.data_ptr(), ctx.data_ptr(), d, B, T,
                                                              n_heads, d // n_heads, int(q_begin), int(q_count), _stream())
        _lib.check(st, "cfm_relpos_attention_rows_mfma16_f32")
        return ctx
    nsplit = _key_split(B, n_heads, q_count, T, keys_hint)
    ws = torch.empty(nsplit * B * q_count * (d + n_heads), device=qkv.device, dtype=torch.float32) if nsplit > 1 else None
    base = qkv.data_ptr()
    st = _lib.load().cfm_relpos_attention_rows_f32(base, base + 4 * d, base + 8 * d, d3, pos.data_ptr(), pos.stride(0),
                                                   u.data_ptr(), v.data_ptr(), lengths.data_ptr(), ctx.data_ptr(), d, B, T,
                                                   n_heads, d // n_heads, int(q_begin), int(q_count), nsplit, _p(ws), _stream())
    _lib.check(st, "cfm_relpos_attention_rows_f32")
    return ctx


def relpos_attention_slots(qkv: torch.Tensor, pos: torch.Tensor, u: torch.Tensor, v: torch.Tensor, lengths: torch.Tensor,
                           n_heads: int, q_begin: torch.Tensor, q_count: torch.Tensor, q_max: int,
                           ctx: Optional[torch.Tensor] = None, keys_hint: Optional[int] = None) -> torch.Tensor:
    u = _req(u, "content_bias"); v = _req(v, "position_bias")
    prec = mfma16_prec()
    q16 = isinstance(qkv, torch.Tensor) and qkv.dtype in (torch.bfloat16, torch.float16)
    if q16:
        if not prec or qkv.dtype != _DT16[prec]:
            raise _lib.ConformerHipError(f"relpos_attention_slots: a {qkv.dtype} cache needs torch.autocast of that type")
        if not (qkv.is_cuda and qkv.dim() == 3 and qkv.shape[-1] % 24 == 0):
            raise _lib.ConformerHipError("relpos_attention_slots: 16-bit qkv: expected a (S,T,3d) HIP tensor with d % 8 == 0")
    else:
        qkv = _req(qkv, "qkv")
    B, T, d3 = qkv.shape
    d = d3 // 3
    q_max = int(q_max)
    _req_pos(pos, T, d)
    if not qkv.is_contiguous():
        raise _lib.ConformerHipError("relpos_attention_slots: qkv (S,T,3d) must be a contiguous cache buffer")
    if ctx is None:
        ctx = torch.empty(B, q_max, d, device=qkv.device, dtype=torch.float32)
    ctx = _req(ctx, "ctx")
    if ctx.shape != (B, q_max, d) or not ctx.is_contiguous():
        raise _lib.ConformerHipError(f"relpos_attention_slots: ctx must be a contiguous ({B},{q_max},{d}) tensor")
    lengths = _req(lengths, "lengths", torch.int64)
    q_begin = _req(q_begin, "q_begin", torch.int64)
    q_count = _req(q_count, "q_count", torch.int64)
    for name, t in (("lengths", lengths), ("q_begin", q_begin), ("q_count", q_count)):
        if t.shape != (B,) or not t.is_contiguous():
            raise _lib.ConformerHipError(f"relpos_attention_slots: {name} must be a contiguous ({B},) int64 tensor")
    nsplit = (_key_split16 if prec else _key_split)(B, n_heads, q_max, T, keys_hint)
    ws = torch.empty(nsplit * B * q_max * (d + n_heads), device=qkv.device, dtype=torch.float32) if nsplit > 1 else None
    base = qkv.data_ptr()
    if prec != PREC_F32:
        esz = 2 if q16 else 4
        st = _lib.load().cfm_relpos_attention_slots_mfma16_f32(prec, base, base + esz * d, base + 2 * esz * d, int(q16), d3,
                                                               pos.data_ptr(), pos.stride(0), u.data_ptr(), v.data_ptr(),
                                                               q_begin.data_ptr(), q_count.data_ptr(), lengths.data_ptr(),
                                                               ctx.data_ptr(), d, B, T, n_heads, d // n_heads, q_max, nsplit,
                                                               _p(ws), _stream())
        _lib.check(st, "cfm_relpos_attention_slots_mfma16_f32")
        return ctx
    st = _lib.load().cfm_relpos_attention_slots_f32(base, base + 4 * d, base + 8 * d, d3, pos.data_ptr(), pos.stride(0),
                                                    u.data_ptr(), v.data_ptr(), q_begin.data_ptr(), q_count.data_ptr(),
                                                    lengths.data_ptr(), ctx.data_ptr(), d, B, T, n_heads, d // n_heads, q_max,
                                                    nsplit, _p(ws), _stream())
    _lib.check(st, "cfm_relpos_attention_slots_f32")
    return ctx


def dwconv_bn_swish(g, w, b, bn_w, bn_b, bn_mean, bn_var, eps: float = 1e-5, for_gemm: bool = False) -> torch.Tensor:
    g = _req(g, "g"); w = _req(w, "dw weight"); b = _req(b, "dw bias")
    B, T, C = g.shape
    K = w.shape[-1]
    p16 = out16_ok(C) if for_gemm and K in (3, 7, 15, 31) else 0
    if p16:
        y = torch.empty(g.shape, device=g.device, dtype=_DT16[p16])
        st = _lib.load().cfm_dwconv_bn_swish_fwd_out16_f32(p16, g.data_ptr(), w.data_ptr(), b.data_ptr(), _req(bn_w, "bn_w").data_ptr(),
                                                           _req(bn_b, "bn_b").data_ptr(), _req(bn_mean, "bn_mean").data_ptr(),
                                                           _req(bn_var, "bn_var").data_ptr(), eps, y.data_ptr(), B, T, C, K,
                                                           _stream())
        _lib.check(st, "cfm_dwconv_bn_swish_fwd_out16_f32")
        return y
    y = _f32_like(g)
    st = _lib.load().cfm_dwconv_bn_swish_fwd_f32(g.data_ptr(), w.data_ptr(), b.data_ptr(), _req(bn_w, "bn_w").data_ptr(),
                                                 _req(bn_b, "bn_b").data_ptr(), _req(bn_mean, "bn_mean").data_ptr(),
                                                 _req(bn_var, "bn_var").data_ptr(), eps, y.data_ptr(), B, T, C, K,
                                                 _stream())
    _lib.check(st, "cfm_dwconv_bn_swish_fwd_f32")
    return y


_CONVMOD_FUSED = __import__("os").environ.get("CONFORMER_AMD_CONVMOD_FUSED", "1") != "0"
_CONVMOD_MIN_ROW_EFF = 0.875


def set_convmod_fused(on: bool) -> bool:
    global _CONVMOD_FUSED
    prev, _CONVMOD_FUSED = _CONVMOD_FUSED, bool(on)
    return prev


def convmod_chunks(T: int, K: int) -> int:
    return 1 if T <= 256 else 1 + (T - 256 + (256 - K)) // (257 - K)


def convmod_fused_ok(B: int, T: int, C: int, K: int) -> bool:
    if not (_CONVMOD_FUSED and ln_fold_ok(C) and C % 64 == 0 and K in (3, 7, 15, 31) and B > 0 and T > 0):
        return False
    chunks = convmod_chunks(T, K)
    blocks = B * chunks * (C // 64)
    rounds = (blocks + 255) // 256
    return blocks >= 0.9 * 256 * rounds and T >= _CONVMOD_MIN_ROW_EFF * 256 * chunks


def convmod_glu_dwconv(x, stats, wf, bf, cs, ln_eps: float, w, b, bn_w, bn_b, bn_mean, bn_var, bn_eps: float = 1e-5) -> torch.Tensor:
    x = _req(x, "x"); stats = _req(stats, "ln_stats"); wf = _req(wf, "Wf"); bf = _req(bf, "bias_f"); cs = _req(cs, "colsum")
    w = _req(w, "dw weight"); b = _req(b, "dw bias")
    if x.dim() != 3:
        raise _lib.ConformerHipError(f"convmod_glu_dwconv: x must be (B, T, C), got {tuple(x.shape)}")
    B, T, C = x.shape
    K = w.shape[-1]
    if (tuple(wf.shape) != (2 * C, C) or stats.dim() != 3 or stats.shape[0] != B * T or stats.shape[2] != 2 or w.numel() != C * K
            or bf.numel() != 2 * C or cs.numel() != 2 * C or b.numel() != C):
        raise _lib.ConformerHipError(f"convmod_glu_dwconv: x{tuple(x.shape)}, Wf{tuple(wf.shape)}, stats{tuple(stats.shape)}, "
                                     f"dw weight{tuple(w.shape)} do not match")
    bn = [_req(t, n) for t, n in ((bn_w, "bn_w"), (bn_b, "bn_b"), (bn_mean, "bn_mean"), (bn_var, "bn_var"))]
    if any(t.numel() != C for t in bn):
        raise _lib.ConformerHipError(f"convmod_glu_dwconv: the BatchNorm tensors must have {C} values")
    y = torch.empty(B, T, C, device=x.device, dtype=torch.float32)
    if B * T:
        _lib.check(_lib.load().cfm_convmod_glu_dwconv_f32(x.data_ptr(), C, stats.data_ptr(), stats.shape[1], float(ln_eps), wf.data_ptr(),
                                                          bf.data_ptr(), cs.data_ptr(), w.data_ptr(), b.data_ptr(), bn[0].data_ptr(),
                                                          bn[1].data_ptr(), bn[2].data_ptr(), bn[3].data_ptr(), float(bn_eps),
                                                          y.data_ptr(), C, B, T, C, K, _stream()), "cfm_convmod_glu_dwconv_f32")
    return y


def pack_conv2_weight(w2: torch.Tensor) -> torch.Tensor:
    w2 = _req(w2, "conv_2.weight")
    C = w2.shape[0]
    out = torch.empty(C, 9 * C, device=w2.device, dtype=torch.float32)
    _lib.check(_lib.load().cfm_pack_conv2_weight_f32(w2.data_ptr(), out.data_ptr(), C, _stream()), "cfm_pack_conv2_weight_f32")
    return out


_CONV2_WINOGRAD = __import__("os").environ.get("CONFORMER_AMD_CONV2_WINOGRAD", "1") == "1"


def set_conv2_winograd(on: bool) -> bool:
    global _CONV2_WINOGRAD
    prev, _CONV2_WINOGRAD = _CONV2_WINOGRAD, bool(on)
    return prev


def conv2_winograd_ok(C: int) -> bool:
    return bool(_CONV2_WINOGRAD and C % 256 == 0 and not mfma16_prec() and not _fp32_planes)


def pack_conv2_wino_weight(w2: torch.Tensor) -> torch.Tensor:
    w2 = _req(w2, "conv_2.weight")
    C = w2.shape[0]
    out = torch.empty(25 * C * C, device=w2.device, dtype=torch.float32)
    _lib.check(_lib.load().cfm_pack_conv2_wino_weight_f32(w2.data_ptr(), out.data_ptr(), C, _stream()),
               "cfm_pack_conv2_wino_weight_f32")
    return out


def pack_linear_weight(wl: torch.Tensor, C: int, F2: int) -> torch.Tensor:
    wl = _req(wl, "linear.weight")
    out = _f32_like(wl)
    _lib.check(_lib.load().cfm_pack_linear_weight_f32(wl.data_ptr(), out.data_ptr(), wl.shape[0], C, F2, _stream()),
               "cfm_pack_linear_weight_f32")
    return out


def subsample_stem(x: torch.Tensor, w1, b1, w2p, b2, w2w=None) -> torch.Tensor:
    x = _req(x, "x"); w1 = _req(w1, "conv_1.weight"); b1 = _req(b1, "conv_1.bias")
    w2p = _req(w2p, "packed conv_2.weight"); b2 = _req(b2, "conv_2.bias")
    B, F, T = x.shape
    C = w1.shape[0]
    F1, T1 = (F - 1) // 2, (T - 1) // 2
    F2, T2 = (F1 - 1) // 2, (T1 - 1) // 2
    lib = _lib.load()
    p16 = out16_ok(C) if C % 64 == 0 else 0
    if p16:
        h1 = torch.empty(B, T1, F1, C, device=x.device, dtype=_DT16[p16])
        _lib.check(lib.cfm_subsample_conv1_relu_out16_f32(p16, x.data_ptr(), w1.data_ptr(), b1.data_ptr(), h1.data_ptr(), B, F,
                                                          T, C, _stream()), "cfm_subsample_conv1_relu_out16_f32")
        h2 = torch.empty(B, T2, F2 * C, device=x.device, dtype=_DT16[p16])
    else:
        h1 = torch.empty(B, T1, F1, C, device=x.device, dtype=torch.float32)
        _lib.check(lib.cfm_subsample_conv1_relu_f32(x.data_ptr(), w1.data_ptr(), b1.data_ptr(), h1.data_ptr(), B, F, T, C,
                                                    _stream()), "cfm_subsample_conv1_relu_f32")
        h2 = torch.empty(B, T2, F2 * C, device=x.device, dtype=torch.float32)
        if w2w is not None and conv2_winograd_ok(C):
            planes = torch.empty(int(lib.cfm_conv2_wino_plane_elems(B, F1, T1, C)), device=x.device, dtype=torch.float32)
            _lib.check(lib.cfm_subsample_conv2_wino_relu_f32(h1.data_ptr(), _req(w2w, "Winograd conv_2.weight").data_ptr(),
                                                             b2.data_ptr(), planes.data_ptr(), h2.data_ptr(), B, F1, T1, C,
                                                             _stream()), "cfm_subsample_conv2_wino_relu_f32")
            return h2
    _conv2_relu(lib, h1, w2p, b2, h2, B, F1, T1, C)
    return h2


def _conv2_relu(lib, h1, w2p, b2, h2, B, F1, T1, C):
    prec = mfma16_prec()
    if prec and C % 64 == 0:
        w16 = weight16(w2p, prec)
        _lib.check(lib.cfm_subsample_conv2_relu_mfma16_f32(prec, h1.data_ptr(), int(h1.dtype != torch.float32),
                                                           (w2p if w16 is None else w16).data_ptr(), int(w16 is not None),
                                                           b2.data_ptr(), h2.data_ptr(), int(h2.dtype != torch.float32), B, F1,
                                                           T1, C, _stream()), "cfm_subsample_conv2_relu_mfma16_f32")
    elif _fp32_planes and C % 64 == 0:
        ws = weight_split(w2p.view(C, 9 * C), _fp32_planes)
        _lib.check(lib.cfm_subsample_conv2_relu_split_bf16_f32(_fp32_planes, h1.data_ptr(), ws.data_ptr(), b2.data_ptr(),
                                                               h2.data_ptr(), B, F1, T1, C, _stream()),
                   "cfm_subsample_conv2_relu_split_bf16_f32")
    else:
        _lib.check(lib.cfm_subsample_conv2_relu_f32(h1.data_ptr(), w2p.data_ptr(), b2.data_ptr(), h2.data_ptr(), B, F1, T1,
                                                    C, _stream()), "cfm_subsample_conv2_relu_f32")


_ZERO_ARENA = {}
_ZERO_CHUNK = 16 << 20


def _zeros_split(device, dtype, *shapes):
    sizes = [int(torch.Size(sh).numel()) for sh in shapes]
    padded = [(n + 3) // 4 * 4 for n in sizes]
    total = sum(padded)
    if total >= _ZERO_CHUNK // 4 or torch.cuda.is_current_stream_capturing():
        buf, off = torch.zeros(total, device=device, dtype=dtype), 0
    else:
        key = (device, dtype, torch.cuda.current_stream(device).cuda_stream)
        ent = _ZERO_ARENA.get(key)
        if ent is None or ent[1] + total > ent[0].numel():
            ent = [torch.zeros(_ZERO_CHUNK, device=device, dtype=dtype), 0]
            _ZERO_ARENA[key] = ent
        buf, off = ent[0], ent[1]
        ent[1] = off + total
    outs = []
    for sh, n, pn in zip(shapes, sizes, padded):
        outs.append(buf[off:off + n].view(sh))
        off += pn
    return outs


def layernorm_train(x, weight, bias, eps: float = 1e-5, for_gemm: bool = False):
    x = _req(x, "x"); weight = _req(weight, "weight"); bias = _req(bias, "bias")
    d = x.shape[-1]
    rows = x.numel() // d
    mean = torch.empty(rows, device=x.device, dtype=torch.float32)
    rstd = torch.empty(rows, device=x.device, dtype=torch.float32)
    p16 = out16_ok(d) if for_gemm else 0
    if p16:
        y = torch.empty(x.shape, device=x.device, dtype=_DT16[p16])
        _lib.check(_lib.load().cfm_layernorm_fwd_out16_f32(p16, x.data_ptr(), weight.data_ptr(), bias.data_ptr(), y.data_ptr(),
                                                           mean.data_ptr(), rstd.data_ptr(), rows, d, eps, _stream()),
                   "cfm_layernorm_fwd_out16_f32")
        return y, mean, rstd
    y = _f32_like(x)
    st = _lib.load().cfm_layernorm_fwd_f32(x.data_ptr(), weight.data_ptr(), bias.data_ptr(), y.data_ptr(),
                                           mean.data_ptr(), rstd.data_ptr(), rows, d, eps, _stream())
    _lib.check(st, "cfm_layernorm_fwd_f32")
    return y, mean, rstd


def layernorm_bwd(x, weight, dy, mean, rstd, dres=None):
    x = _req(x, "x"); dy = _req(dy, "dy"); weight = _req(weight, "weight")
    d = x.shape[-1]
    rows = x.numel() // d
    lib = _lib.load()
    dx = _f32_like(x)
    if dres is not None:
        dres = _req(dres, "dres")
    dw, db = _zeros_split(x.device, x.dtype, (d,), (d,))
    if d <= 2048:
        nws = int(lib.cfm_layernorm_bwd_workspace_bytes(rows, d))
        ws = torch.empty(nws // 4, device=x.device, dtype=torch.float32)
        _lib.check(lib.cfm_layernorm_bwd_f32(x.data_ptr(), weight.data_ptr(), dy.data_ptr(), mean.data_ptr(), rstd.data_ptr(),
                                             _p(dres), dx.data_ptr(), dw.data_ptr(), db.data_ptr(), rows, d, ws.data_ptr(), nws,
                                             _stream()),
                   "cfm_layernorm_bwd_f32")
        return dx, dw, db
    _lib.check(lib.cfm_layernorm_bwd_dx_f32(x.data_ptr(), weight.data_ptr(), dy.data_ptr(), mean.data_ptr(),
                                            rstd.data_ptr(), _p(dres), dx.data_ptr(), rows, d, _stream()),
               "cfm_layernorm_bwd_dx_f32")
    _lib.check(lib.cfm_layernorm_bwd_params_f32(x.data_ptr(), dy.data_ptr(), mean.data_ptr(), rstd.data_ptr(),
                                                dw.data_ptr(), db.data_ptr(), rows, d, _stream()),
               "cfm_layernorm_bwd_params_f32")
    return dx, dw, db


def linear_swish_save(a, w, b):
    a, w2, b, m, n, k = _gemm_common(a, w, b)
    c = torch.empty(*a.shape[:-1], n, device=a.device, dtype=torch.float32)
    z = _f32_like(c)
    st = _lib.load().cfm_gemm_bias_swish_save_f32(a.data_ptr(), w2.data_ptr(), b.data_ptr(), c.data_ptr(), z.data_ptr(),
                                                  m, n, k, k, n, _stream())
    _lib.check(st, "cfm_gemm_bias_swish_save_f32")
    return c, z


_SEED_GEN = {}


def _mix64(*vals: int) -> int:
    z = 0x243F6A8885A308D3
    for v in vals:
        z = ((z ^ (v & 0xFFFFFFFFFFFFFFFF)) * 0x9E3779B97F4A7C15) & 0xFFFFFFFFFFFFFFFF
        z ^= z >> 29
        z = (z * 0xBF58476D1CE4E5B9) & 0xFFFFFFFFFFFFFFFF
        z ^= z >> 32
    return z & 0x3FFFFFFFFFFFFFFF


def _rank() -> int:
    import os
    if torch.distributed.is_available() and torch.distributed.is_initialized():
        return torch.distributed.get_rank()
    return int(os.environ.get("RANK", "0"))


def new_seeds(n: int):
    if torch.cuda.is_available():
        g = torch.cuda.default_generators[torch.cuda.current_device()]
        seed, off = g.initial_seed(), g.get_offset()
        g.set_offset(off + 4 * n)
        return [_mix64(seed, _rank(), off + 4 * i) for i in range(n)]
    key = (torch.initial_seed(), _rank())
    if _SEED_GEN.get("key") != key:
        _SEED_GEN["key"], _SEED_GEN["off"] = key, 0
    off = _SEED_GEN["off"]
    _SEED_GEN["off"] = off + 4 * n
    return [_mix64(key[0], key[1], off + 4 * i) for i in range(n)]


def linear_train(epi: str, a, w, b, *, residual=None, alpha: float = 1.0, drop_p: float = 0.0, seed: int = 0,
                 save_z: bool = False, for_gemm: bool = False):
    a, w2, b, m, n, k = _gemm_common(a, w, b)
    p16 = out16_ok(n) if for_gemm else 0
    c = torch.empty(*a.shape[:-1], n, device=a.device, dtype=_DT16[p16] if p16 else torch.float32)
    z = torch.empty(*a.shape[:-1], n, device=a.device, dtype=_DT16[p16] if p16 and epi == "swish" else torch.float32) if save_z else None
    code = {"bias": 0, "swish": 1, "residual": 4}[epi]
    if residual is not None:
        residual = _req(residual, "residual")
    prec = mfma16_prec()
    if prec:
        _mfma16_gemm(prec, code, a, w2, b, c, m, n, k, residual, alpha, z, drop_p, seed)
        return (c, z) if save_z else c
    st = _lib.load().cfm_gemm_train_f32(code, a.data_ptr(), w2.data_ptr(), b.data_ptr(), _p(residual), alpha, c.data_ptr(),
                                        _p(z), m, n, k, k, n, n, float(drop_p), int(seed), _stream())
    _lib.check(st, "cfm_gemm_train_f32")
    return (c, z) if save_z else c


def dropout_apply(x, drop_p: float, seed: int, for_gemm: bool = False):
    x = _req(x, "x")
    prec = mfma16_prec() if for_gemm else 0
    if prec and x.numel() % 8 == 0 and x.shape[-1] % 8 == 0:
        y = torch.empty(x.shape, device=x.device, dtype=_DT16[prec])
        _lib.check(_lib.load().cfm_dropout_out16_f32(prec, x.data_ptr(), y.data_ptr(), x.numel(), float(max(drop_p, 0.0)), int(seed),
                                                     _stream()), "cfm_dropout_out16_f32")
        return y
    if drop_p <= 0.0:
        return x
    y = _f32_like(x)
    _lib.check(_lib.load().cfm_dropout_f32(x.data_ptr(), y.data_ptr(), x.numel(), float(drop_p), int(seed), _stream()),
               "cfm_dropout_f32")
    return y


def glu_fwd(z):
    z = _req(z, "z")
    n = z.shape[-1] // 2
    rows = z.numel() // (2 * n)
    y = torch.empty(*z.shape[:-1], n, device=z.device, dtype=torch.float32)
    _lib.check(_lib.load().cfm_glu_fwd_f32(z.data_ptr(), y.data_ptr(), rows, n, _stream()), "cfm_glu_fwd_f32")
    return y


def glu_bwd(z, dy, for_gemm: bool = False):
    z = _req(z, "z"); dy = _req(dy, "dy")
    n = dy.shape[-1]
    rows = dy.numel() // n
    p16 = out16_ok(2 * n) if for_gemm and n % 8 == 0 else 0
    if p16:
        dz = torch.empty(z.shape, device=z.device, dtype=_DT16[p16])
        _lib.check(_lib.load().cfm_glu_bwd_out16_f32(p16, z.data_ptr(), dy.data_ptr(), dz.data_ptr(), rows, n, _stream()),
                   "cfm_glu_bwd_out16_f32")
        return dz
    dz = _f32_like(z)
    _lib.check(_lib.load().cfm_glu_bwd_f32(z.data_ptr(), dy.data_ptr(), dz.data_ptr(), rows, n, _stream()),
               "cfm_glu_bwd_f32")
    return dz


def colsum(x2d, alpha: float = 1.0, rows=None, cols=None, ld=None, out=None):
    rows = x2d.shape[0] if rows is None else rows
    cols = x2d.shape[1] if cols is None else cols
    ld = x2d.stride(0) if ld is None else ld
    if out is None:
        out = torch.zeros(cols, device=x2d.device, dtype=x2d.dtype)
    _lib.check(_lib.load().cfm_colsum_f32(x2d.data_ptr(), ld, rows, cols, alpha, out.data_ptr(), _stream()),
               "cfm_colsum_f32")
    return out


def gemm_bwd(A, a_col: bool, B, b_col: bool, I: int, J: int, Kc: int, *, alpha: float = 1.0, Z=None, out=None,
             lda=None, ldb=None, ldc=None, ldz=None, allow_split: bool = False, accumulate: bool = False,
             nbatch: int = 1, nb1: int = 1, sa=(0, 0), sb=(0, 0), sc=(0, 0), a_ptr=None, b_ptr=None, c_ptr=None,
             drop_p: float = 0.0, drop_seed: int = 0, prec: int = 0, b16: bool = False, pad4: bool = False,
             c16: bool = False):
    lda = A.stride(-2) if lda is None else lda
    ldb = B.stride(-2) if ldb is None else ldb
    if out is None:
        out = (torch.zeros if allow_split else torch.empty)(I, J, device=A.device, dtype=_DT16[prec] if c16 else A.dtype)
    ldc = out.stride(-2) if ldc is None else ldc
    ldz = 0 if Z is None else (Z.stride(-2) if ldz is None else ldz)
    head = (A.data_ptr() if a_ptr is None else a_ptr, int(a_col), lda, B.data_ptr() if b_ptr is None else b_ptr, int(b_col))
    z16 = Z is not None and Z.dtype != torch.float32
    tail = (ldb, _p(Z), int(z16), ldz, alpha, out.data_ptr() if c_ptr is None else c_ptr, ldc, int(c16), I, J, Kc, int(allow_split),
            int(accumulate), nbatch, nb1, sa[0], sa[1], sb[0], sb[1], sc[0], sc[1], float(drop_p), int(drop_seed))
    if prec:
        _lib.check(_lib.load().cfm_gemm_bwd_batched_mfma16_f32(prec, *head, int(b16), *tail, int(pad4), _stream()),
                   "cfm_gemm_bwd_batched_mfma16_f32")
    else:
        if b16 or c16 or z16:
            raise _lib.ConformerHipError("16-bit operands / results need a 16-bit precision mode")
        _lib.check(_lib.load().cfm_gemm_bwd_batched_f32(*head, *tail[:2], *tail[3:7], *tail[8:], _stream()), "cfm_gemm_bwd_batched_f32")
    return out


def linear_bwd(x2d, w, dy2d, *, alpha: float = 1.0, Z=None, need_dx: bool = True, drop_p: float = 0.0, drop_seed: int = 0,
               dx16: bool = False):
    m, k = x2d.shape
    n = w.shape[0]
    w2 = w.reshape(n, -1)
    dx = None
    prec = mfma16_prec()
    dy16 = dy2d.dtype != torch.float32
    z_ok = Z is not None and n % 8 == 0 and k % 8 == 0 and Z.stride(0) % 8 == 0
    if dy16 and not (prec and dy2d.dtype == _DT16[prec]):
        raise _lib.ConformerHipError("a 16-bit dY needs the matching 16-bit precision mode")
    if dy16 and not (n % 8 == 0 and k % 8 == 0 and (z_ok or (Z is None and alpha == 1.0))):
        dy2d, dy16 = dy2d.float(), False
    if x2d.dtype != torch.float32:
        if not (prec and x2d.dtype == _DT16[prec]):
            raise _lib.ConformerHipError("a 16-bit x needs the matching 16-bit precision mode")
        if k % 8 or x2d.stride(0) % 8 or x2d.stride(1) != 1:
            x2d = x2d.float()
    if dy2d.stride(0) & 3:
        padded = torch.zeros(m, (n + 3) // 4 * 4, device=dy2d.device, dtype=dy2d.dtype)
        padded[:, :n] = dy2d
        dy2d = padded[:, :n]
    if need_dx and dy16 and Z is None:
        wt16 = weight16(w2, prec, transposed=True)
        dx = torch.empty(m, k, device=dy2d.device, dtype=torch.float32)
        _lib.check(_lib.load().cfm_gemm_mfma16_f32(prec, 0, dy2d.data_ptr(), 1, wt16.data_ptr(), 1, _zero_bias(k, dy2d.device).data_ptr(),
                                                   None, 1.0, dx.data_ptr(), 0, None, 0, m, k, n, dy2d.stride(0), k, k, 0.0, 0, _stream()),
                   "cfm_gemm_mfma16_f32")
    elif need_dx and prec and z_ok:
        wt16 = weight16(w2, prec, transposed=True)
        dx = torch.empty(m, k, device=dy2d.device, dtype=_DT16[prec] if dx16 else torch.float32)
        _lib.check(_lib.load().cfm_gemm_mfma16_f32(prec, 5, dy2d.data_ptr(), int(dy16), wt16.data_ptr(), 1, None, None, alpha, dx.data_ptr(),
                                                   int(dx16), Z.data_ptr(), int(Z.dtype != torch.float32), m, k, n, dy2d.stride(0),
                                                   Z.stride(0), k, float(drop_p), int(drop_seed), _stream()), "cfm_gemm_mfma16_f32")
    elif need_dx:
        w16 = weight16(w2, prec) if prec else None
        c16 = bool(dx16 and prec and Z is not None and k % 8 == 0 and n % 8 == 0)
        dx = gemm_bwd(dy2d, False, w2 if w16 is None else w16, True, m, k, n, alpha=alpha, Z=Z, drop_p=drop_p,
                      drop_seed=drop_seed, prec=prec, b16=w16 is not None, c16=c16)
    dw, db = _zeros_split(dy2d.device, torch.float32, (n, k), (n,))
    x16 = x2d.dtype != torch.float32
    if (prec and (x16 or dy16) and n % 8 == 0 and k % 8 == 0 and x2d.stride(1) == 1 and dy2d.stride(1) == 1
            and x2d.stride(0) % (8 if x16 else 4) == 0 and dy2d.stride(0) % (8 if dy16 else 4) == 0
            and x2d.data_ptr() % 16 == 0 and dy2d.data_ptr() % 16 == 0):
        _lib.check(_lib.load().cfm_linear_bwd_weight_mfma16_f32(prec, dy2d.data_ptr(), int(dy16), dy2d.stride(0), x2d.data_ptr(),
                                                                int(x16), x2d.stride(0), dw.data_ptr(), k, db.data_ptr(), n, k, m,
                                                                alpha, _stream()), "cfm_linear_bwd_weight_mfma16_f32")
    else:
        if dy16:
            raise _lib.ConformerHipError("a 16-bit dY needs the aligned 16-bit weight-gradient kernel (N % 8 == 0, K % 8 == 0)")
        gemm_bwd(dy2d, True, x2d, True, n, k, m, alpha=alpha, allow_split=True, out=dw, prec=prec, b16=x16)
        colsum(dy2d, alpha, out=db)
    return dx, dw.view_as(w), db


def dwconv_bn_batch_stats(g, w, b, running_mean, running_var, momentum: float = 0.1):
    g = _req(g, "g")
    B, T, C = g.shape
    K = w.shape[-1]
    lib = _lib.load()
    nws = int(lib.cfm_dwconv_bn_stats_workspace_bytes(B, T, C))
    buf = torch.empty(2 * C + (nws + 3) // 4, device=g.device, dtype=torch.float32)
    mean, var, ws = buf[:C], buf[C:2 * C], buf[2 * C:]
    st = lib.cfm_dwconv_bn_stats_f32(g.data_ptr(), w.data_ptr(), b.data_ptr(), mean.data_ptr(), var.data_ptr(),
                                     _p(running_mean), _p(running_var), momentum, B, T, C, K, ws.data_ptr(), nws, _stream())
    _lib.check(st, "cfm_dwconv_bn_stats_f32")
    return mean, var


def dwconv_bn_swish_bwd(g, dy, w, b, bn_w, bn_b, bn_mean, bn_var, eps: float = 1e-5, train_stats: bool = False):
    g = _req(g, "g"); dy = _req(dy, "dy")
    B, T, C = g.shape
    K = w.shape[-1]
    dc = _f32_like(g)
    dg = _f32_like(g)
    dw, db, dga, dbe = _zeros_split(g.device, g.dtype, tuple(w.shape), (C,), (C,), (C,))
    st = _lib.load().cfm_dwconv_bn_swish_bwd_f32(g.data_ptr(), dy.data_ptr(), w.data_ptr(), b.data_ptr(), bn_w.data_ptr(),
                                                 bn_b.data_ptr(), bn_mean.data_ptr(), bn_var.data_ptr(), eps,
                                                 int(train_stats), dc.data_ptr(), dg.data_ptr(), dw.data_ptr(), db.data_ptr(),
                                                 dga.data_ptr(), dbe.data_ptr(), B, T, C, K, _stream())
    _lib.check(st, "cfm_dwconv_bn_swish_bwd_f32")
    return dg, dw, db, dga, dbe


def relpos_attention_train(qkv, pos, u, v, lengths, n_heads, drop_p: float = 0.0, seed: int = 0):
    u = _req(u, "content_bias"); v = _req(v, "position_bias")
    qkv = _req(qkv, "qkv")
    B, T, d3 = qkv.shape
    d = d3 // 3
    dh = d // n_heads
    if not (isinstance(pos, torch.Tensor) and pos.is_cuda and pos.dtype == torch.float32 and pos.dim() == 2
            and pos.stride(1) == 1 and pos.shape == (2 * T - 1, d)):
        raise _lib.ConformerHipError(f"pos: expected a ({2 * T - 1},{d}) fp32 HIP tensor with unit column stride")
    if lengths is not None:
        lengths = _req(lengths, "lengths", torch.int64)
        if lengths.numel() != B:
            raise _lib.ConformerHipError(f"lengths: expected {B} entries, got {lengths.numel()}")
    ctx = torch.empty(B, T, d, device=qkv.device, dtype=torch.float32)
    lse = torch.empty(B, n_heads, T, device=qkv.device, dtype=torch.float32)
    base = qkv.data_ptr()
    prec = mfma16_prec()
    if prec:
        st = _lib.load().cfm_relpos_attention_mfma16_f32(prec, base, base + 4 * d, base + 8 * d, d3, pos.data_ptr(),
                                                         pos.stride(0), u.data_ptr(), v.data_ptr(), _p(lengths),
                                                         ctx.data_ptr(), d, lse.data_ptr(), B, T, n_heads, dh, float(drop_p),
                                                         int(seed), _stream())
        _lib.check(st, "cfm_relpos_attention_mfma16_f32")
        return ctx, lse
    st = _lib.load().cfm_relpos_attention_train_f32(base, base + 4 * d, base + 8 * d, d3, pos.data_ptr(), pos.stride(0),
                                                    u.data_ptr(), v.data_ptr(), _p(lengths), ctx.data_ptr(), d,
                                                    lse.data_ptr(), B, T, n_heads, dh, float(drop_p), int(seed), _stream())
    _lib.check(st, "cfm_relpos_attention_train_f32")
    return ctx, lse


def relpos_attention_bwd(qkv, pos, u, v, lengths, n_heads, ctx, lse, dctx, drop_p: float = 0.0, seed: int = 0):
    qkv = _req(qkv, "qkv"); pos = _req(pos, "pos"); ctx = _req(ctx, "ctx"); lse = _req(lse, "lse")
    dctx = _req(dctx, "dctx")
    B, T, d3 = qkv.shape
    d = d3 // 3
    dh = d // n_heads
    if pos.shape != (2 * T - 1, d) or ctx.shape != (B, T, d) or dctx.shape != (B, T, d) or lse.shape != (B, n_heads, T):
        raise _lib.ConformerHipError(f"relpos_attention_bwd: qkv{tuple(qkv.shape)} with {n_heads} heads needs pos ({2 * T - 1},{d}), "
                                     f"ctx / dctx ({B},{T},{d}) and lse ({B},{n_heads},{T}); got pos{tuple(pos.shape)}, "
                                     f"ctx{tuple(ctx.shape)}, dctx{tuple(dctx.shape)}, lse{tuple(lse.shape)}")
    if lengths is not None:
        lengths = _req(lengths, "lengths", torch.int64)
        if lengths.numel() != B:
            raise _lib.ConformerHipError(f"lengths: expected {B} entries, got {lengths.numel()}")
    ctx, dctx = ctx.contiguous(), dctx.contiguous()
    P = 2 * T - 1
    dqkv, dpos, du, dvb = _zeros_split(qkv.device, qkv.dtype, (B, T, d3), (P, d), (n_heads, dh), (n_heads, dh))
    base, dbase = qkv.data_ptr(), dqkv.data_ptr()
    args = (base, base + 4 * d, base + 8 * d, d3, pos.data_ptr(), pos.stride(0), u.data_ptr(), v.data_ptr(), _p(lengths),
            ctx.data_ptr(), dctx.data_ptr(), d, lse.data_ptr(), dbase, dbase + 4 * d, dbase + 8 * d, d3, dpos.data_ptr(), d,
            du.data_ptr(), dvb.data_ptr(), B, T, n_heads, dh, float(drop_p), int(seed))
    prec = mfma16_prec()
    if prec and dh > 16:
        _lib.check(_lib.load().cfm_relpos_attention_bwd_mfma16_f32(prec, *args, _stream()), "cfm_relpos_attention_bwd_mfma16_f32")
    else:
        _lib.check(_lib.load().cfm_relpos_attention_bwd_f32(*args, prec, _stream()), "cfm_relpos_attention_bwd_f32")
    return dqkv, dpos, du, dvb


def subsample_stem_train(x, w1, b1, w2p, b2):
    x = _req(x, "x")
    B, F, T = x.shape
    C = w1.shape[0]
    F1, T1 = (F - 1) // 2, (T - 1) // 2
    F2, T2 = (F1 - 1) // 2, (T1 - 1) // 2
    lib = _lib.load()
    p16 = out16_ok(C) if C % 64 == 0 and B * T1 * F1 * C < 2 ** 31 else 0
    if p16:
        h1 = torch.empty(B, T1, F1, C, device=x.device, dtype=_DT16[p16])
        _lib.check(lib.cfm_subsample_conv1_relu_out16_f32(p16, x.data_ptr(), w1.data_ptr(), b1.data_ptr(), h1.data_ptr(), B, F,
                                                          T, C, _stream()), "cfm_subsample_conv1_relu_out16_f32")
    else:
        h1 = torch.empty(B, T1, F1, C, device=x.device, dtype=torch.float32)
        _lib.check(lib.cfm_subsample_conv1_relu_f32(x.data_ptr(), w1.data_ptr(), b1.data_ptr(), h1.data_ptr(), B, F, T, C,
                                                    _stream()), "cfm_subsample_conv1_relu_f32")
    h2 = torch.empty(B, T2, F2 * C, device=x.device, dtype=torch.float32)
    _conv2_relu(lib, h1, w2p, b2, h2, B, F1, T1, C)
    return h2, h1


def subsample_stem_bwd(x, w1, b1, w2, h1, h2, dh2):
    lib = _lib.load()
    B, F, T = x.shape
    C = w1.shape[0]
    F1, T1 = (F - 1) // 2, (T - 1) // 2
    F2, T2 = (F1 - 1) // 2, (T1 - 1) // 2
    dh2 = _req(dh2, "dh2")
    prec = mfma16_prec() if C % 64 == 0 else 0
    h16 = h1.dtype != torch.float32
    if h16 and (not prec or h1.dtype != _DT16[prec]):
        raise _lib.ConformerHipError("a 16-bit h1 needs the matching precision mode in the backward")
    dw2p, db2, dw1, db1 = _zeros_split(x.device, torch.float32, (C, 9 * C), (C,), tuple(w1.shape), (C,))
    if h16:
        dz2 = torch.empty(dh2.shape, device=x.device, dtype=_DT16[prec])
        _lib.check(lib.cfm_relu_bwd_out16_f32(prec, h2.data_ptr(), dh2.data_ptr(), dz2.data_ptr(), dz2.numel(), _stream()),
                   "cfm_relu_bwd_out16_f32")
        rowtab = torch.empty(int(lib.cfm_subsample_conv2_rowtab_elems(B, F1, T1)), device=x.device, dtype=torch.int32)
        _lib.check(lib.cfm_subsample_conv2_bwd_weight_h16_mfma16_f32(prec, dz2.data_ptr(), 1, h1.data_ptr(), rowtab.data_ptr(),
                                                                     dw2p.data_ptr(), db2.data_ptr(), B, F1, T1, C, _stream()),
                   "cfm_subsample_conv2_bwd_weight_h16_mfma16_f32")
    else:
        dz2 = _f32_like(dh2)
        _lib.check(lib.cfm_relu_bwd_f32(h2.data_ptr(), dh2.data_ptr(), dz2.data_ptr(), dz2.numel(), _stream()),
                   "cfm_relu_bwd_f32")
        colsum(dz2.view(-1, C), out=db2)
        if prec:
            _lib.check(lib.cfm_subsample_conv2_bwd_weight_mfma16_f32(prec, dz2.data_ptr(), h1.data_ptr(), dw2p.data_ptr(), B, F1,
                                                                     T1, C, _stream()), "cfm_subsample_conv2_bwd_weight_mfma16_f32")
        else:
            _lib.check(lib.cfm_subsample_conv2_bwd_weight_f32(dz2.data_ptr(), h1.data_ptr(), dw2p.data_ptr(), B, F1, T1, C,
                                                              _stream()), "cfm_subsample_conv2_bwd_weight_f32")
    w2c = torch.empty(9 * C * C, device=x.device, dtype=torch.float32)
    _lib.check(lib.cfm_pack_conv2_weight_t_f32(w2.data_ptr(), w2c.data_ptr(), C, _stream()), "cfm_pack_conv2_weight_t_f32")
    d16 = bool(prec and h16)
    dh1 = torch.empty(h1.shape, device=h1.device, dtype=_DT16[prec] if d16 else torch.float32)
    if prec:
        w2c16 = torch.empty(9 * C * C, device=x.device, dtype=_DT16[prec])
        _lib.check(lib.cfm_cast16_f32(prec, w2c.data_ptr(), w2c16.data_ptr(), w2c.numel(), _stream()), "cfm_cast16_f32")
        fn = lib.cfm_subsample_conv2_bwd_input_fwdkernel_out16_mfma16_f32 if d16 else lib.cfm_subsample_conv2_bwd_input_fwdkernel_mfma16_f32
        _lib.check(fn(prec, dz2.data_ptr(), int(dz2.dtype != torch.float32), w2c16.data_ptr(), _zero_bias(C, x.device).data_ptr(),
                      dh1.data_ptr(), B, F1, T1, C, _stream()), "cfm_subsample_conv2_bwd_input_fwdkernel_mfma16_f32")
    else:
        _lib.check(lib.cfm_subsample_conv2_bwd_input_f32(dz2.data_ptr(), w2c.data_ptr(), dh1.data_ptr(), B, F1, T1, C,
                                                         _stream()), "cfm_subsample_conv2_bwd_input_f32")
    if d16:
        _lib.check(lib.cfm_subsample_conv1_bwd_d16_f32(prec, x.data_ptr(), w1.data_ptr(), b1.data_ptr(), dh1.data_ptr(), dw1.data_ptr(),
                                                       db1.data_ptr(), B, F, T, C, _stream()), "cfm_subsample_conv1_bwd_d16_f32")
    else:
        _lib.check(lib.cfm_subsample_conv1_bwd_f32(x.data_ptr(), w1.data_ptr(), b1.data_ptr(), dh1.data_ptr(), dw1.data_ptr(),
                                                   db1.data_ptr(), B, F, T, C, _stream()), "cfm_subsample_conv1_bwd_f32")
    dw2 = dw2p.view(C, 3, 3, C).permute(0, 3, 1, 2).contiguous()
    return dw1, db1, dw2, db2


def lstm_forward(x, w_ih, w_hh, bias, lengths=None, save: bool = False, state=None):
    x = _req(x, "x")
    return lstm_recurrence(linear(x, w_ih, bias), w_hh, lengths, save, state)


def lstm_recurrence(gx, w_hh, lengths=None, save: bool = False, state=None):
    gx = _req(gx, "gates_x"); w_hh = _req(w_hh, "weight_hh")
    B, T, _ = gx.shape
    H = w_hh.shape[1]
    hs = None
    if state is not None:
        hs, c = state
        for name, t in (("state h", hs), ("state c", c)):
            if not (isinstance(t, torch.Tensor) and t.is_cuda and t.dtype == torch.float32 and t.is_contiguous()
                    and tuple(t.shape) == (B, H)):
                raise ValueError(f"lstm_forward: {name} must be a contiguous fp32 ({B}, {H}) tensor on the HIP device")
    y = torch.empty(B, T, H, device=gx.device, dtype=torch.float32)
    if hs is None:
        c = torch.empty(B, H, device=gx.device, dtype=torch.float32)
    gates = torch.empty(B, T, 4 * H, device=gx.device, dtype=torch.float32) if save else None
    cells = torch.empty(B, T, H, device=gx.device, dtype=torch.float32) if save else None
    if lengths is not None:
        lengths = _req(lengths, "lengths", torch.int64)
    prec = mfma16_prec()
    w16 = weight16(w_hh, prec) if prec and H % 16 == 0 else None
    if w16 is not None:
        h16 = torch.empty(2 * ((B + 31) // 32) * 32 * H, device=gx.device, dtype=_DT16[prec])
        w16 = w16.view(4, H // 8, 8, H // 16, 2, 8).permute(1, 3, 4, 0, 2, 5).contiguous()
        if hs is not None:
            _lib.check(_lib.load().cfm_lstm_fwd_mfma16_carry_f32(prec, gx.data_ptr(), w16.data_ptr(), _p(lengths), y.data_ptr(),
                                                                 hs.data_ptr(), c.data_ptr(), h16.data_ptr(), _p(gates), _p(cells),
                                                                 B, T, H, _stream()), "cfm_lstm_fwd_mfma16_carry_f32")
            return (y, gates, cells) if save else y
        _lib.check(_lib.load().cfm_lstm_fwd_mfma16_f32(prec, gx.data_ptr(), w16.data_ptr(), _p(lengths), y.data_ptr(), c.data_ptr(),
                                                       h16.data_ptr(), _p(gates), _p(cells), B, T, H, _stream()),
                   "cfm_lstm_fwd_mfma16_f32")
        return (y, gates, cells) if save else y
    if H % 16 == 0:
        wf = w_hh.view(4, H // 4, 4, H // 16, 4, 4).permute(1, 3, 4, 0, 2, 5).contiguous()
        hf = torch.empty(2 * ((B + 15) // 16) * 16 * H, device=gx.device, dtype=torch.float32)
        if hs is not None:
            _lib.check(_lib.load().cfm_lstm_fwd_frag_carry_f32(gx.data_ptr(), wf.data_ptr(), _p(lengths), y.data_ptr(), hs.data_ptr(),
                                                               c.data_ptr(), hf.data_ptr(), _p(gates), _p(cells), B, T, H, _stream()),
                       "cfm_lstm_fwd_frag_carry_f32")
            return (y, gates, cells) if save else y
        _lib.check(_lib.load().cfm_lstm_fwd_frag_f32(gx.data_ptr(), wf.data_ptr(), _p(lengths), y.data_ptr(), c.data_ptr(),
                                                     hf.data_ptr(), _p(gates), _p(cells), B, T, H, _stream()),
                   "cfm_lstm_fwd_frag_f32")
        return (y, gates, cells) if save else y
    if hs is not None:
        _lib.check(_lib.load().cfm_lstm_fwd_carry_f32(gx.data_ptr(), w_hh.data_ptr(), _p(lengths), y.data_ptr(), hs.data_ptr(),
                                                      c.data_ptr(), _p(gates), _p(cells), B, T, H, _stream()), "cfm_lstm_fwd_carry_f32")
        return (y, gates, cells) if save else y
    _lib.check(_lib.load().cfm_lstm_fwd_f32(gx.data_ptr(), w_hh.data_ptr(), _p(lengths), y.data_ptr(), c.data_ptr(), _p(gates),
                                            _p(cells), B, T, H, _stream()), "cfm_lstm_fwd_f32")
    return (y, gates, cells) if save else y


def swish_bn_eval(h, bn_mean, bn_var, bn_weight, bn_bias, eps: float = 1e-5):
    h = _req(h, "h")
    C = h.shape[-1]
    out = _f32_like(h)
    _lib.check(_lib.load().cfm_swish_bn_eval_f32(h.data_ptr(), _req(bn_mean, "bn_mean").data_ptr(),
                                                 _req(bn_var, "bn_var").data_ptr(), _req(bn_weight, "bn_weight").data_ptr(),
                                                 _req(bn_bias, "bn_bias").data_ptr(), eps, out.data_ptr(), h.numel() // C, C,
                                                 _stream()), "cfm_swish_bn_eval_f32")
    return out


def lstm_backward(x, w_ih, w_hh, y, gates, cells, dy, lengths=None, need_dx: bool = True):
    lib = _lib.load()
    B, T, D = x.shape
    H = w_hh.shape[1]
    dy = _req(dy, "dy")
    dG = torch.empty(B, T, 4 * H, device=x.device, dtype=torch.float32)
    dc = torch.empty(B, H, device=x.device, dtype=torch.float32)
    prec = mfma16_prec()
    wt16 = weight16(w_hh, prec, transposed=True) if prec and H % 16 == 0 else None
    if wt16 is not None:
        wt16 = wt16.view(H // 16, 16, 4 * H // 16, 2, 8).permute(0, 2, 3, 1, 4).contiguous()
        dg16 = torch.empty(2 * ((B + 15) // 16) * 16 * 4 * H, device=x.device, dtype=_DT16[prec])
        _lib.check(lib.cfm_lstm_bwd_mfma16_f32(prec, dy.data_ptr(), gates.data_ptr(), cells.data_ptr(), wt16.data_ptr(), _p(lengths),
                                               dG.data_ptr(), dc.data_ptr(), dg16.data_ptr(), B, T, H, _stream()),
                   "cfm_lstm_bwd_mfma16_f32")
    elif H % 16 == 0:
        wtf = w_hh.t().reshape(H // 16, 16, 4 * H // 16, 4, 4).permute(0, 2, 3, 1, 4).contiguous()
        dgf = torch.empty(2 * ((B + 15) // 16) * 16 * 4 * H, device=x.device, dtype=torch.float32)
        _lib.check(lib.cfm_lstm_bwd_frag_f32(dy.data_ptr(), gates.data_ptr(), cells.data_ptr(), wtf.data_ptr(), _p(lengths),
                                             dG.data_ptr(), dc.data_ptr(), dgf.data_ptr(), B, T, H, _stream()),
                   "cfm_lstm_bwd_frag_f32")
    else:
        whh_t = w_hh.t().contiguous()
        _lib.check(lib.cfm_lstm_bwd_f32(dy.data_ptr(), gates.data_ptr(), cells.data_ptr(), whh_t.data_ptr(), _p(lengths),
                                        dG.data_ptr(), dc.data_ptr(), B, T, H, _stream()), "cfm_lstm_bwd_f32")
    dG2, x2 = dG.view(B * T, 4 * H), x.reshape(B * T, D)
    h_prev = torch.zeros(y.shape, device=y.device, dtype=torch.float32)
    h_prev[:, 1:] = y[:, :-1]
    dx = gemm_bwd(dG2, False, w_ih, True, B * T, D, 4 * H, prec=prec).view(B, T, D) if need_dx else None
    dw_ih, dw_hh, db = _zeros_split(x.device, x.dtype, (4 * H, D), (4 * H, H), (4 * H,))
    gemm_bwd(dG2, True, x2, True, 4 * H, D, B * T, allow_split=True, out=dw_ih, prec=prec)
    gemm_bwd(dG2, True, h_prev.view(B * T, H), True, 4 * H, H, B * T, allow_split=True, out=dw_hh, prec=prec)
    colsum(dG2, out=db)
    return dx, dw_ih, dw_hh, db


def swish_bn_batch_stats(h, running_mean, running_var, momentum: float = 0.1):
    h = _req(h, "h")
    C = h.shape[-1]
    mean = torch.empty(C, device=h.device, dtype=torch.float32)
    var = torch.empty(C, device=h.device, dtype=torch.float32)
    _lib.check(_lib.load().cfm_swish_bn_stats_f32(h.data_ptr(), mean.data_ptr(), var.data_ptr(), _p(running_mean),
                                                  _p(running_var), momentum, h.numel() // C, C, _stream()),
               "cfm_swish_bn_stats_f32")
    return mean, var


def swish_bn_bwd(h, dz, bn_mean, bn_var, bn_weight, eps: float = 1e-5, train_stats: bool = False):
    h = _req(h, "h"); dz = _req(dz, "dz")
    C = h.shape[-1]
    dh = _f32_like(h)
    dga, dbe = _zeros_split(h.device, h.dtype, (C,), (C,))
    _lib.check(_lib.load().cfm_swish_bn_bwd_f32(h.data_ptr(), dz.data_ptr(), bn_mean.data_ptr(), bn_var.data_ptr(),
                                                bn_weight.data_ptr(), eps, int(train_stats), dh.data_ptr(), dga.data_ptr(),
                                                dbe.data_ptr(), h.numel() // C, C, _stream()), "cfm_swish_bn_bwd_f32")
    return dh, dga, dbe


CTC_MAX_TARGET = 1023


def _ctc_geometry(logits, targets, input_lengths, target_lengths):
    logits = _req(logits, "logits")
    if logits.dim() != 3:
        raise _lib.ConformerHipError(f"ctc_loss: logits must be (B,T,V), got {tuple(logits.shape)}")
    B = logits.shape[0]
    targets = _req(targets.to(logits.device), "targets", torch.int64)
    in_len = _req(torch.as_tensor(input_lengths).to(logits.device), "input_lengths", torch.int64)
    tg_len = _req(torch.as_tensor(target_lengths).to(logits.device), "target_lengths", torch.int64)
    if in_len.numel() != B or tg_len.numel() != B:
        raise _lib.ConformerHipError("ctc_loss: input_lengths / target_lengths must hold one entry per utterance")
    if targets.dim() == 2:
        if targets.shape[0] != B:
            raise _lib.ConformerHipError("ctc_loss: 2-D targets must be (B, max_target_length)")
        off, stride, lmax = None, targets.shape[1], targets.shape[1]
    elif targets.dim() == 1:
        off = (torch.cumsum(tg_len, 0) - tg_len).contiguous()
        stride, lmax = 0, int(tg_len.max())
    else:
        raise _lib.ConformerHipError("ctc_loss: targets must be 1-D (concatenated) or 2-D (padded)")
    lmax = max(lmax, 1)
    if lmax > CTC_MAX_TARGET:
        raise NotImplementedError(f"ctc_loss: targets longer than {CTC_MAX_TARGET} labels are not built")
    return logits, targets, off, stride, in_len, tg_len, lmax


def ctc_loss_forward(logits, targets, input_lengths, target_lengths, blank: int = 0):
    logits, targets, off, stride, in_len, tg_len, lmax = _ctc_geometry(logits, targets, input_lengths, target_lengths)
    B, T, V = logits.shape
    lib = _lib.load()
    ws = torch.empty(int(lib.cfm_ctc_workspace_floats(B, T, lmax)), device=logits.device, dtype=torch.float32)
    loss = torch.empty((), device=logits.device, dtype=torch.float32)
    _lib.check(lib.cfm_ctc_loss_fwd_f32(logits.data_ptr(), targets.data_ptr(), _p(off), stride, targets.numel(),
                                        in_len.data_ptr(), tg_len.data_ptr(), B, T, V, lmax, int(blank), ws.data_ptr(),
                                        loss.data_ptr(), _stream()), "cfm_ctc_loss_fwd_f32")
    return loss, (logits, targets, off, stride, in_len, tg_len, lmax, int(blank), ws)


def ctc_loss_backward(ctx, grad_out):
    logits, targets, off, stride, in_len, tg_len, lmax, blank, ws = ctx
    B, T, V = logits.shape
    g = _req(grad_out.reshape(1), "grad_out")
    dlogits = _f32_like(logits)
    _lib.check(_lib.load().cfm_ctc_loss_bwd_f32(logits.data_ptr(), targets.data_ptr(), _p(off), stride, targets.numel(),
                                                in_len.data_ptr(), tg_len.data_ptr(), B, T, V, lmax, blank, ws.data_ptr(),
                                                g.data_ptr(), dlogits.data_ptr(), _stream()), "cfm_ctc_loss_bwd_f32")
    return dlogits


def ctc_nll(ctx) -> torch.Tensor:
    return ctx[-1][-ctx[0].shape[0]:]
```

include/conformer_hip.h:

```cpp
#ifndef CONFORMER_HIP_H
#define CONFORMER_HIP_H

#include <stddef.h>
#include <stdint.h>

#ifdef __cplusplus
extern "C" {
#endif

typedef void* cfm_stream_t;

enum cfm_status {
    CFM_OK = 0,
    CFM_ERR_BAD_SHAPE = -1,
    CFM_ERR_UNSUPPORTED = -2,
    CFM_ERR_NULL = -3,
    CFM_ERR_LAUNCH = -4,
    CFM_ERR_DEVICE = -5,
    CFM_ERR_ALIGN = -6
};

int cfm_version(void);
int cfm_abi_version(void);
#define CFM_ABI_VERSION 4
const char* cfm_strerror(int status);
int cfm_device_check(void);

int cfm_layernorm_fwd_f32(const float* x, const float* gamma, const float* beta, float* y,
                          float* mean_or_null, float* rstd_or_null,
                          int64_t rows, int d, float eps, cfm_stream_t stream);

int cfm_gemm_bias_f32(const float* A, const float* W, const float* bias, float* C,
                      int64_t M, int N, int K, int64_t lda, int64_t ldc, cfm_stream_t stream);
int cfm_gemm_bias_swish_f32(const float* A, const float* W, const float* bias, float* C,
                            int64_t M, int N, int K, int64_t lda, int64_t ldc, cfm_stream_t stream);
int cfm_gemm_bias_relu_f32(const float* A, const float* W, const float* bias, float* C,
                           int64_t M, int N, int K, int64_t lda, int64_t ldc, cfm_stream_t stream);
int cfm_gemm_bias_glu_f32(const float* A, const float* W, const float* bias, float* C,
                          int64_t M, int n_out, int K, int64_t lda, int64_t ldc, cfm_stream_t stream);
int cfm_gemm_bias_residual_f32(const float* A, const float* W, const float* bias, const float* R,
                               float alpha, float* C, int64_t M, int N, int K,
                               int64_t lda, int64_t ldr, int64_t ldc, cfm_stream_t stream);

int cfm_gemm_splitk_f32(int epi, const float* A, const float* W, const float* bias, const float* R_or_null,
                        float alpha, float* C, float* workspace, int splits, int64_t M, int N, int K,
                        int64_t lda, int64_t ldr, int64_t ldc, cfm_stream_t stream);

int cfm_gemm_bias_stats_f32(const float* A, const float* W, const float* bias, float* C, float* stats_out,
                            int64_t M, int N, int K, int64_t lda, int64_t ldc, cfm_stream_t stream);
int cfm_gemm_bias_residual_stats_f32(const float* A, const float* W, const float* bias, const float* R,
                                     float alpha, float* C, float* stats_out, int64_t M, int N, int K,
                                     int64_t lda, int64_t ldr, int64_t ldc, cfm_stream_t stream);
int cfm_gemm_lnfold_f32(int epi, const float* A, const float* ln_stats, int ln_parts, float ln_eps,
                        const float* Wf, const float* bias_f, const float* colsum, float* C,
                        int64_t M, int N, int K, int64_t lda, int64_t ldc, cfm_stream_t stream);
int cfm_layernorm_fwd_stats_f32(const float* x, const float* gamma, const float* beta, float* y,
                                float* stats_out, int64_t rows, int d, float eps, cfm_stream_t stream);

int64_t cfm_ffn_pack_elems(int d, int hidden);
int cfm_ffn_pack_f32(const float* W1f, const float* W2, float* Wp, int d, int hidden, cfm_stream_t stream);
int cfm_ffn_fused_f32(const float* X, int64_t ldx, const float* ln_stats, int ln_parts, float ln_eps, const float* Wp,
                      const float* b1f, const float* colsum1, const float* b2, float alpha, float* Y, int64_t ldy,
                      int mode, float* stats_out, const float* gamma2, const float* beta2, float eps2, int64_t M,
                      int d, int hidden, cfm_stream_t stream);

int cfm_rowgemm_pack_f32(const float* W, float* Wp, int N, int d, int glu, cfm_stream_t stream);
int cfm_rowchain_f32(int pre, int core, int post, int mode, const float* X, int64_t ldx, const float* Wpre_packed,
                     const float* bpre, const float* R, int64_t ldr, float* Y1, int64_t ldy1, const float* ln_stats,
                     int ln_parts, float ln_eps, const float* Wffn_packed, const float* b1f, const float* colsum1,
                     const float* b2, float alpha, int hidden, float* Y, int64_t ldy, float* stats_out,
                     const float* gamma2, const float* beta2, float eps2, const float* Wpost_packed, const float* bpost,
                     const float* cspost, float post_eps, float* Z, int64_t ldz, int64_t M, int d, cfm_stream_t stream);
int64_t cfm_ffn_tile_stride_f4(int d);
int cfm_ffn_rotate(void);

int cfm_relpos_table_f32(const float* div_term, float* pe, int T, int d, cfm_stream_t stream);

int cfm_relpos_attention_fwd_f32(const float* q, const float* k, const float* v, int64_t ld,
                                 const float* pos, int64_t ldp, const float* u, const float* vbias,
                                 const int64_t* lengths_or_null, float* ctx, int64_t ldo,
                                 float* lse_or_null, int B, int T, int H, int dh, cfm_stream_t stream);

int cfm_dwconv_bn_swish_fwd_f32(const float* g, const float* w, const float* bias,
                                const float* bn_weight, const float* bn_bias,
                                const float* bn_mean, const float* bn_var, float bn_eps,
                                float* y, int B, int T, int C, int K, cfm_stream_t stream);

int cfm_convmod_glu_dwconv_f32(const float* x, int64_t ldx, const float* ln_stats, int ln_parts, float ln_eps,
                               const float* Wf, const float* bias_f, const float* colsum, const float* dw_w,
                               const float* dw_b, const float* bn_w, const float* bn_b, const float* bn_mean,
                               const float* bn_var, float bn_eps, float* y, int64_t ldy, int B, int T, int C, int K,
                               cfm_stream_t stream);

int cfm_subsample_conv1_relu_f32(const float* x, const float* w1, const float* b1, float* h1,
                                 int B, int F, int T, int C, cfm_stream_t stream);
int cfm_pack_conv2_weight_f32(const float* w2, float* w2p, int C, cfm_stream_t stream);
int cfm_subsample_conv2_relu_f32(const float* h1, const float* w2p, const float* b2, float* h2,
                                 int B, int F1, int T1, int C, cfm_stream_t stream);
int cfm_pack_linear_weight_f32(const float* wl, float* wlp, int d_out, int C, int F2, cfm_stream_t stream);
int64_t cfm_conv2_wino_plane_elems(int B, int F1, int T1, int C);
int cfm_pack_conv2_wino_weight_f32(const float* w2, float* wwp, int C, cfm_stream_t stream);
int cfm_subsample_conv2_wino_relu_f32(const float* h1, const float* wwp, const float* b2, float* planes, float* h2,
                                      int B, int F1, int T1, int C, cfm_stream_t stream);

#define CFM_PREC_F32 0
#define CFM_PREC_BF16 1
#define CFM_PREC_FP16 2
int cfm_gemm_mfma16_f32(int prec, int epi, const void* A, int a_is_16bit, const void* W, int w_is_16bit,
                        const float* bias, const float* R_or_null, float alpha, void* C, int c_is_16bit,
                        void* Z_or_null, int z_is_16bit, int64_t M, int N, int K, int64_t lda, int64_t ldr,
                        int64_t ldc, float drop_p, uint64_t drop_seed, cfm_stream_t stream);
#define CFM_CAST_BATCH 48
typedef struct cfm_cast_item {
    const float* src;
    void* dst;
    int64_t rows, cols;
    int transpose;
} cfm_cast_item;
int cfm_cast16_multi_f32(int prec, const cfm_cast_item* items, int count, cfm_stream_t stream);
int cfm_layernorm_fwd_out16_f32(int prec, const float* x, const float* gamma, const float* beta, void* y16,
                                float* mean_or_null, float* rstd_or_null, int64_t rows, int d, float eps,
                                cfm_stream_t stream);
int cfm_cast16_f32(int prec, const float* src, void* dst, int64_t n, cfm_stream_t stream);
int cfm_relpos_attention_mfma16_f32(int prec, const float* q, const float* k, const float* v, int64_t ld,
                                    const float* pos, int64_t ldp, const float* u, const float* vbias,
                                    const int64_t* lengths_or_null, float* ctx, int64_t ldo, float* lse_or_null, int B,
                                    int T, int H, int dh, float drop_p, uint64_t drop_seed, cfm_stream_t stream);
int cfm_relpos_attention_rows_mfma16_f32(int prec, const float* q, const float* k, const float* v, int64_t ld,
                                         const float* pos, int64_t ldp, const float* u, const float* vbias,
                                         const int64_t* lengths, float* ctx, int64_t ldo, int B, int T, int H, int dh,
                                         int q_begin, int q_count, cfm_stream_t stream);
int cfm_relpos_attention_io16_mfma16_f32(int prec, const void* q, const void* k, const void* v, int qkv_is_16bit, int64_t ld,
                                         const float* pos, int64_t ldp, const float* u, const float* vbias,
                                         const int64_t* lengths_or_null, void* ctx, int ctx_is_16bit, int64_t ldo, int B, int T,
                                         int H, int dh, cfm_stream_t stream);
int cfm_subsample_conv2_relu_mfma16_f32(int prec, const void* h1, int h1_is_16bit, const void* w2p, int w_is_16bit,
                                        const float* b2, void* h2, int h2_is_16bit, int B, int F1, int T1, int C,
                                        cfm_stream_t stream);
int cfm_subsample_conv1_relu_out16_f32(int prec, const float* x, const float* w1, const float* b1, void* h1, int B, int F,
                                       int T, int C, cfm_stream_t stream);
int cfm_gemm_bwd_batched_mfma16_f32(int prec, const float* A, int a_col, int64_t lda, const void* B, int b_col,
                                    int b_is_16bit, int64_t ldb, const void* Z_or_null, int z_is_16bit, int64_t ldz, float alpha, void* C,
                                    int64_t ldc, int c_is_16bit, int I, int J, int64_t Kc, int allow_split, int accumulate,
                                    int nbatch, int nb1, int64_t sa0, int64_t sa1, int64_t sb0, int64_t sb1,
                                    int64_t sc0, int64_t sc1, float drop_p, uint64_t drop_seed,
                                    int operands_zero_padded4, cfm_stream_t stream);
int cfm_linear_bwd_weight_mfma16_f32(int prec, const void* dy, int dy_is_16bit, int64_t ldy, const void* x,
                                     int x_is_16bit, int64_t ldx, float* dw, int64_t ldw, float* db_or_null, int N,
                                     int K, int64_t M, float alpha, cfm_stream_t stream);
int64_t cfm_subsample_conv2_rowtab_elems(int B, int F1, int T1);
int cfm_subsample_conv2_bwd_weight_h16_mfma16_f32(int prec, const void* dz2, int dz2_is_16bit, const void* h1_16,
                                                  int* rowtab_scratch, float* dw2p, float* db2_or_null, int B, int F1, int T1,
                                                  int C, cfm_stream_t stream);
int cfm_dwconv_bn_swish_fwd_out16_f32(int prec, const float* g, const float* w, const float* bias, const float* bn_weight,
                                      const float* bn_bias, const float* bn_mean, const float* bn_var, float bn_eps,
                                      void* y16, int B, int T, int C, int K, cfm_stream_t stream);
int cfm_glu_bwd_out16_f32(int prec, const float* z, const float* dy, void* dz16, int64_t rows, int n, cfm_stream_t stream);
int cfm_relu_bwd_out16_f32(int prec, const float* y, const float* dy, void* dz16, int64_t n, cfm_stream_t stream);
int cfm_subsample_conv2_bwd_input_fwdkernel_mfma16_f32(int prec, const void* dz2, int dz2_is_16bit, const void* w2c16,
                                                       const float* zero_bias, float* dh1, int B, int F1, int T1,
                                                       int C, cfm_stream_t stream);
int cfm_subsample_conv2_bwd_input_fwdkernel_out16_mfma16_f32(int prec, const void* dz2, int dz2_is_16bit, const void* w2c16,
                                                             const float* zero_bias, void* dh1_16, int B, int F1, int T1, int C,
                                                             cfm_stream_t stream);
int cfm_subsample_conv1_bwd_d16_f32(int prec, const float* x, const float* w1, const float* b1, const void* dh1_16, float* dw1,
                                    float* db1, int B, int F, int T, int C, cfm_stream_t stream);
int cfm_subsample_conv2_bwd_weight_mfma16_f32(int prec, const float* dz2, const float* h1, float* dw2p, int B, int F1,
                                              int T1, int C, cfm_stream_t stream);
int cfm_subsample_conv2_bwd_input_mfma16_f32(int prec, const float* dz2, const float* w2c, float* dh1, int B, int F1,
                                             int T1, int C, cfm_stream_t stream);

int cfm_reflect_pad_f32(const float* x, float* xp, int B, int64_t L, int pad, int64_t ld_out, cfm_stream_t stream);
int cfm_power_mel_log_f32(const float* spec, int64_t ld_spec, const float* fb, float* out, int B, int T,
                          int n_bins, int n_mels, float floor_value, cfm_stream_t stream);
int cfm_power_mel_log_mfma_f32(const float* spec, int64_t ld_spec, const float* fbT, float* out, int B, int T,
                               int rows_per_utt, int n_bins, int n_mels, float floor_value, cfm_stream_t stream);
int cfm_dft_frames_f32(const float* wave, const float* basis, float* spec, int64_t rows, int n_cols, int n_fft,
                       int hop, cfm_stream_t stream);
int cfm_specaugment_apply_f32(float* spec, int B, int F, int T, const int* bands, int nbands, float value,
                              cfm_stream_t stream);


int cfm_gemm_bias_swish_save_f32(const float* A, const float* W, const float* bias, float* C, float* Z,
                                 int64_t M, int N, int K, int64_t lda, int64_t ldc, cfm_stream_t stream);

int cfm_gemm_bwd_f32(const float* A, int a_col, int64_t lda, const float* B, int b_col, int64_t ldb,
                     const float* Z_or_null, int64_t ldz, float alpha, float* C, int64_t ldc,
                     int I, int J, int64_t Kc, int allow_split, cfm_stream_t stream);
int cfm_gemm_bwd_batched_f32(const float* A, int a_col, int64_t lda, const float* B, int b_col, int64_t ldb,
                             const float* Z_or_null, int64_t ldz, float alpha, float* C, int64_t ldc,
                             int I, int J, int64_t Kc, int allow_split, int accumulate, int nbatch, int nb1,
                             int64_t sa0, int64_t sa1, int64_t sb0, int64_t sb1, int64_t sc0, int64_t sc1,
                             float drop_p, uint64_t drop_seed, cfm_stream_t stream);

int cfm_gemm_train_f32(int epi, const float* A, const float* W, const float* bias, const float* R_or_null,
                       float alpha, float* C, float* Z_or_null, int64_t M, int N, int K, int64_t lda,
                       int64_t ldr, int64_t ldc, float drop_p, uint64_t drop_seed, cfm_stream_t stream);
int cfm_relpos_attention_train_f32(const float* q, const float* k, const float* v, int64_t ld,
                                   const float* pos, int64_t ldp, const float* u, const float* vbias,
                                   const int64_t* lengths_or_null, float* ctx, int64_t ldo, float* lse,
                                   int B, int T, int H, int dh, float drop_p, uint64_t drop_seed,
                                   cfm_stream_t stream);
int cfm_dropout_f32(const float* x, float* y, int64_t n, float p, uint64_t seed, cfm_stream_t stream);
int cfm_dropout_out16_f32(int prec, const float* x, void* y16, int64_t n, float p, uint64_t seed, cfm_stream_t stream);

int cfm_layernorm_bwd_dx_f32(const float* x, const float* gamma, const float* dy, const float* mean,
                             const float* rstd, const float* dres_or_null, float* dx, int64_t rows, int d,
                             cfm_stream_t stream);
int cfm_layernorm_bwd_params_f32(const float* x, const float* dy, const float* mean, const float* rstd,
                                 float* dgamma, float* dbeta, int64_t rows, int d, cfm_stream_t stream);
size_t cfm_layernorm_bwd_workspace_bytes(int64_t rows, int d);
int cfm_layernorm_bwd_f32(const float* x, const float* gamma, const float* dy, const float* mean,
                          const float* rstd, const float* dres_or_null, float* dx, float* dgamma, float* dbeta,
                          int64_t rows, int d, void* workspace, size_t workspace_bytes, cfm_stream_t stream);

int cfm_colsum_f32(const float* X, int64_t ld, int64_t rows, int cols, float alpha, float* out,
                   cfm_stream_t stream);

int cfm_glu_fwd_f32(const float* z, float* y, int64_t rows, int n, cfm_stream_t stream);
int cfm_glu_bwd_f32(const float* z, const float* dy, float* dz, int64_t rows, int n, cfm_stream_t stream);

int cfm_dwconv_bn_swish_bwd_f32(const float* g, const float* dy, const float* w, const float* bias,
                                const float* bn_weight, const float* bn_bias, const float* bn_mean,
                                const float* bn_var, float bn_eps, int train_stats, float* dc_ws, float* dg,
                                float* dw, float* dbias, float* dgamma, float* dbeta, int B, int T, int C,
                                int K, cfm_stream_t stream);

size_t cfm_dwconv_bn_stats_workspace_bytes(int B, int T, int C);
int cfm_dwconv_bn_stats_f32(const float* g, const float* w, const float* bias, float* batch_mean,
                            float* batch_var, float* running_mean_or_null, float* running_var_or_null,
                            float momentum, int B, int T, int C, int K, void* workspace, size_t workspace_bytes,
                            cfm_stream_t stream);

int cfm_relpos_attention_bwd_f32(const float* q, const float* k, const float* v, int64_t ld, const float* pos,
                                 int64_t ldp, const float* u, const float* vbias, const int64_t* lengths_or_null,
                                 const float* ctx, const float* dctx, int64_t ldo, const float* lse, float* dq,
                                 float* dk, float* dv, int64_t ldg, float* dpos, int64_t lddp, float* du,
                                 float* dvbias, int B, int T, int H, int dh, float drop_p, uint64_t drop_seed,
                                 int prec, cfm_stream_t stream);

int cfm_relpos_attention_bwd_mfma16_f32(int prec, const float* q, const float* k, const float* v, int64_t ld,
                                        const float* pos, int64_t ldp, const float* u, const float* vbias,
                                        const int64_t* lengths_or_null, const float* ctx, const float* dctx, int64_t ldo,
                                        const float* lse, float* dq, float* dk, float* dv, int64_t ldg, float* dpos,
                                        int64_t lddp, float* du, float* dvbias, int B, int T, int H, int dh,
                                        float drop_p, uint64_t drop_seed, cfm_stream_t stream);

int cfm_debug_attention_bwd_trace_f32(void* trace_or_null);
int cfm_debug_attention_bwd_trace_mfma16(void* trace_or_null);
int cfm_debug_dw16_trace(void* trace_or_null);
int cfm_debug_lstm_trace(void* trace_or_null);
int cfm_debug_gemm_mfma16_force_tile(int tile);
int cfm_debug_gemm_mfma16_trace(void* trace_or_null);
int cfm_debug_gemm_last_tile(int family, int* out);

int cfm_debug_gemm_cfg_f32(int cfg, const float* A, const float* W, const float* bias, const float* R,
                           float alpha, float* C, int64_t M, int N, int K, void* trace_or_null,
                           cfm_stream_t stream);
int cfm_debug_ffn_trace(void* trace_or_null, int per_slice);
int cfm_debug_ffn_variant(int v);
int cfm_debug_convmod_variant(int v);
int cfm_debug_ffn_layout(int pad_f4, int rotate);
int cfm_debug_set_conv2_bk(int bk);

int cfm_relu_bwd_f32(const float* y, const float* dy, float* dz, int64_t n, cfm_stream_t stream);
int cfm_subsample_conv2_bwd_weight_f32(const float* dz2, const float* h1, float* dw2p, int B, int F1, int T1,
                                       int C, cfm_stream_t stream);
int cfm_pack_conv2_weight_t_f32(const float* w2, float* w2c, int C, cfm_stream_t stream);
int cfm_subsample_conv2_bwd_input_f32(const float* dz2, const float* w2c, float* dh1, int B, int F1, int T1,
                                      int C, cfm_stream_t stream);
int cfm_subsample_conv1_bwd_f32(const float* x, const float* w1, const float* b1, const float* dh1, float* dw1,
                                float* db1, int B, int F, int T, int C, cfm_stream_t stream);

typedef struct cfm_adam_tensor {
    float* param;
    const float* grad;
    float* exp_avg;
    float* exp_avg_sq;
    int64_t numel;
} cfm_adam_tensor;
int cfm_adam_step_f32(const cfm_adam_tensor* tensors, int n_tensors, float lr, float beta1, float beta2, float eps,
                      float bias_c1, float sqrt_bias_c2, cfm_stream_t stream);
int cfm_greedy_ctc_decode_f32(const float* logits, const int64_t* lengths_or_null, int64_t* frame_ids,
                              int64_t* tokens, int64_t* counts, int B, int T, int V, int pad_id, int unk_id,
                              cfm_stream_t stream);

size_t cfm_ctc_beam_workspace_bytes(int B, int T, int W, int K);
int cfm_ctc_beam_decode_f32(const float* logits, const int64_t* lengths_or_null, int B, int T, int V, int blank_id,
                            int beam_width, int max_candidates, float token_min_logp, float beam_prune_logp, int n_best,
                            void* workspace, size_t workspace_bytes, int64_t* tokens, int64_t* counts, float* scores,
                            int64_t* num_hyps, cfm_stream_t stream);

size_t cfm_ngram_lm_pack_bytes(int order, const int64_t* ngram_counts, int n_words, int64_t word_cp_total, int V,
                               int64_t tok_cp_total);
int cfm_ngram_lm_pack(int order, const int64_t* ngram_counts, const int32_t* ngram_words, const float* ngram_logp,
                      const float* ngram_backoff, int n_words, const int64_t* word_cp_offsets, const int32_t* word_cp, int bos_id,
                      int eos_id, int unk_id, int V, const int64_t* tok_cp_offsets, const int32_t* tok_cp, const int32_t* tok_kind,
                      void* out, size_t out_bytes);
int cfm_ngram_lm_score_f64(const void* lm_tables, const int32_t* words, const int64_t* offsets, int n_sentences, int boundary,
                           double* out, cfm_stream_t stream);
size_t cfm_ctc_beam_lm_workspace_bytes(int B, int T, int W, int K);
int cfm_ctc_beam_lm_decode_f32(const float* logits, const int64_t* lengths_or_null, int B, int T, int V, int blank_id,
                               int beam_width, int max_candidates, float token_min_logp, float beam_prune_logp, int n_best,
                               const void* lm_tables, double alpha, double beta, double unk_score_offset, int score_boundary,
                               void* workspace, size_t workspace_bytes, int64_t* tokens, int64_t* counts, float* scores,
                               float* am_scores, int64_t* num_hyps, cfm_stream_t stream);

size_t cfm_hotword_pack_bytes(int n_unigrams, int64_t uni_cp_total, int n_phrases, int64_t phrase_word_total, int V,
                              int64_t tok_cp_total);
int cfm_hotword_pack(int n_unigrams, const int64_t* uni_cp_offsets, const int32_t* uni_cp, int n_phrases,
                     const int64_t* phrase_offsets, const int32_t* phrase_words, int V, const int64_t* tok_cp_offsets,
                     const int32_t* tok_cp, const int32_t* tok_kind, void* out, size_t out_bytes);
int cfm_hotword_count(const void* hw_tables, const int32_t* tokens, const int64_t* offsets, int n_seqs, double weight,
                      int32_t* counts, double* bonus, int32_t* final_counts);
size_t cfm_ctc_beam_hw_workspace_bytes(int B, int T, int W, int K);
int cfm_ctc_beam_hw_decode_f32(const float* logits, const int64_t* lengths_or_null, int B, int T, int V, int blank_id,
                               int beam_width, int max_candidates, float token_min_logp, float beam_prune_logp, int n_best,
                               const void* lm_tables_or_null, double alpha, double beta, double unk_score_offset,
                               int score_boundary, const void* hw_tables, double hotword_weight, void* workspace,
                               size_t workspace_bytes, int64_t* tokens, int64_t* counts, float* scores, float* am_scores,
                               int64_t* num_hyps, cfm_stream_t stream);

size_t cfm_ctc_beam_stream_state_bytes(int B, int T_max, int W, int K, int lm, int hw);
int cfm_ctc_beam_stream_init(int B, int T_max, int beam_width, int max_candidates, const void* lm_tables_or_null,
                             int score_boundary, const void* hw_tables_or_null, void* state, size_t state_bytes,
                             cfm_stream_t stream);
int cfm_ctc_beam_stream_step_f32(const float* logits, const int64_t* lengths_or_null, int B, int Tc, int V, int blank_id,
                                 int beam_width, int max_candidates, float token_min_logp, float beam_prune_logp, int n_best,
                                 const void* lm_tables_or_null, double alpha, double beta, double unk_score_offset,
                                 int score_boundary, const void* hw_tables_or_null, double hotword_weight, void* state,
                                 size_t state_bytes, int T_max, int t_used, int64_t* tokens, int64_t* counts, float* scores,
                                 float* am_scores_or_null, int64_t* num_hyps, cfm_stream_t stream);
int cfm_ctc_beam_stream_finish_f32(int B, int beam_width, int max_candidates, int n_best, const void* lm_tables_or_null,
                                   double alpha, double beta, double unk_score_offset, int score_boundary,
                                   const void* hw_tables_or_null, double hotword_weight, void* state, size_t state_bytes,
                                   int T_max, int64_t* tokens, int64_t* counts, float* scores, float* am_scores_or_null,
                                   int64_t* num_hyps, cfm_stream_t stream);
int cfm_ctc_beam_stream_reset_slots(int B, int T_max, int beam_width, int max_candidates, const void* lm_tables_or_null,
                                    int score_boundary, const void* hw_tables_or_null, const int64_t* slots, int n_slots,
                                    void* state, size_t state_bytes, cfm_stream_t stream);

int cfm_lstm_fwd_f32(const float* gates_x, const float* w_hh, const int64_t* lengths_or_null, float* y, float* c_state,
                     float* save_gates_or_null, float* save_c_or_null, int B, int T, int H, cfm_stream_t stream);
int cfm_lstm_bwd_f32(const float* dy, const float* gates, const float* cells, const float* whh_t,
                     const int64_t* lengths_or_null, float* dgates, float* dc_state, int B, int T, int H,
                     cfm_stream_t stream);
int cfm_lstm_fwd_frag_f32(const float* gates_x, const float* w_hh_frag, const int64_t* lengths_or_null, float* y,
                          float* c_state, float* h_frag_scratch, float* save_gates_or_null, float* save_c_or_null, int B,
                          int T, int H, cfm_stream_t stream);
int cfm_lstm_bwd_frag_f32(const float* dy, const float* gates, const float* cells, const float* whh_t_frag,
                          const int64_t* lengths_or_null, float* dgates, float* dc_state, float* dg_frag_scratch, int B,
                          int T, int H, cfm_stream_t stream);
int cfm_lstm_fwd_mfma16_f32(int prec, const float* gates_x, const void* w_hh16, const int64_t* lengths_or_null, float* y,
                            float* c_state, void* h16_scratch, float* save_gates_or_null, float* save_c_or_null, int B,
                            int T, int H, cfm_stream_t stream);
int cfm_lstm_fwd_carry_f32(const float* gates_x, const float* w_hh, const int64_t* lengths_or_null, float* y, float* h_state,
                           float* c_state, float* save_gates_or_null, float* save_c_or_null, int B, int T, int H,
                           cfm_stream_t stream);
int cfm_lstm_fwd_frag_carry_f32(const float* gates_x, const float* w_hh_frag, const int64_t* lengths_or_null, float* y,
                                float* h_state, float* c_state, float* h_frag_scratch, float* save_gates_or_null,
                                float* save_c_or_null, int B, int T, int H, cfm_stream_t stream);
int cfm_lstm_fwd_mfma16_carry_f32(int prec, const float* gates_x, const void* w_hh16, const int64_t* lengths_or_null, float* y,
                                  float* h_state, float* c_state, void* h16_scratch, float* save_gates_or_null,
                                  float* save_c_or_null, int B, int T, int H, cfm_stream_t stream);
int cfm_lstm_bwd_mfma16_f32(int prec, const float* dy, const float* gates, const float* cells, const void* whh_t16,
                            const int64_t* lengths_or_null, float* dgates, float* dc_state, void* dg16_scratch, int B,
                            int T, int H, cfm_stream_t stream);
int cfm_swish_bn_eval_f32(const float* h, const float* bn_mean, const float* bn_var, const float* bn_weight,
                          const float* bn_bias, float eps, float* out, int64_t rows, int C, cfm_stream_t stream);
int cfm_swish_bn_stats_f32(const float* h, float* batch_mean, float* batch_var, float* running_mean_or_null,
                           float* running_var_or_null, float momentum, int64_t rows, int C, cfm_stream_t stream);
int cfm_swish_bn_bwd_f32(const float* h, const float* dz, const float* bn_mean, const float* bn_var,
                         const float* bn_weight, float eps, int train_stats, float* dh, float* dgamma, float* dbeta,
                         int64_t rows, int C, cfm_stream_t stream);

int64_t cfm_split_pack_elems(int planes, int N, int K);
int cfm_split_pack_bf16_f32(int planes, const float* w, void* dst, int N, int K, cfm_stream_t stream);
int cfm_gemm_split_bf16_f32(int planes, int epi, const float* A, const void* W_split, const float* bias,
                            const float* R_or_null, float alpha, float* C, int64_t M, int N, int K, int64_t lda,
                            int64_t ldr, int64_t ldc, cfm_stream_t stream);
int cfm_subsample_conv2_relu_split_bf16_f32(int planes, const float* h1, const void* w2p_split, const float* b2, float* h2,
                                            int B, int F1, int T1, int C, cfm_stream_t stream);

#define CFM_CTC_MAX_TARGET 1023
int64_t cfm_ctc_workspace_floats(int B, int T, int Lmax);
int cfm_ctc_loss_fwd_f32(const float* logits, const int64_t* targets, const int64_t* tgt_off_or_null,
                         int64_t tgt_stride, int64_t tgt_numel, const int64_t* in_len, const int64_t* tgt_len,
                         int B, int T, int V, int Lmax, int blank, float* workspace, float* loss, cfm_stream_t stream);
int cfm_ctc_loss_bwd_f32(const float* logits, const int64_t* targets, const int64_t* tgt_off_or_null,
                         int64_t tgt_stride, int64_t tgt_numel, const int64_t* in_len, const int64_t* tgt_len,
                         int B, int T, int V, int Lmax, int blank, float* workspace, const float* grad_out,
                         float* dlogits, cfm_stream_t stream);

#define CFM_CTC_ALIGN_MAX_FRAMES 16384
#define CFM_CTC_ALIGN_MAX_TARGET 4096
#define CFM_CTC_ALIGN_WAVE_MAX_TARGET 1023
size_t cfm_ctc_align_workspace_bytes(int B, int T, int Lmax);
int cfm_ctc_align_f32(const float* logits, const int64_t* targets, const int64_t* lengths_or_null,
                      const int64_t* target_lengths_or_null, int B, int T, int V, int Lmax, int blank_id, void* workspace,
                      size_t workspace_bytes, int64_t* frame_tokens, int64_t* frame_index, int64_t* token_start,
                      int64_t* token_end, float* token_score, double* score, unsigned char* ok, cfm_stream_t stream);

int cfm_relpos_attention_rows_f32(const float* q, const float* k, const float* v, int64_t ld, const float* pos,
                                  int64_t ldp, const float* u, const float* vbias, const int64_t* lengths_or_null,
                                  float* ctx, int64_t ldo, int B, int T, int H, int dh, int q_begin, int q_count,
                                  int nsplit, float* workspace_or_null, cfm_stream_t stream);
int cfm_relpos_attention_slots_f32(const float* q, const float* k, const float* v, int64_t ld, const float* pos, int64_t ldp,
                                   const float* u, const float* vbias, const int64_t* q_begin, const int64_t* q_count,
                                   const int64_t* lengths, float* ctx, int64_t ldo, int B, int T, int H, int dh, int q_max,
                                   int nsplit, float* workspace_or_null, cfm_stream_t stream);

int cfm_relpos_attention_slots_mfma16_f32(int prec, const void* q, const void* k, const void* v, int qkv_is_16bit, int64_t ld,
                                          const float* pos, int64_t ldp, const float* u, const float* vbias,
                                          const int64_t* q_begin, const int64_t* q_count, const int64_t* lengths, float* ctx,
                                          int64_t ldo, int B, int T, int H, int dh, int q_max, int nsplit,
                                          float* workspace_or_null, cfm_stream_t stream);

int cfm_debug_attention_trace_f32(const float* q, const float* k, const float* v, int64_t ld, const float* pos,
                                  int64_t ldp, const float* u, const float* vbias, const int64_t* lengths_or_null,
                                  float* ctx, int64_t ldo, int B, int T, int H, int dh, void* trace, cfm_stream_t stream);
int cfm_debug_set_attention_waves(int nw);
int cfm_debug_set_bwd_tile(int tile);

int64_t cfm_subsampled_length(int64_t n);
int cfm_subsampled_lengths_i64(const int64_t* lengths, int64_t* out, int n, cfm_stream_t stream);

#ifdef __cplusplus
}
#endif
#endif
```

Measured before the change: 1.704 million audio-frames/sec.

## Generalize conv2 Winograd to 3-output blocks per axis, default scheme 3x2

Extends the strided subsampling conv2 Winograd decomposition from 2x2 outputs per block to configurable 2 or 3 outputs per axis (time, frequency), with new interpolation patterns, weight packing, plane GEMM dispatch and a generic combine kernel. The default scheme becomes 3 in time and 2 in frequency, which lowers the number of multiplies per output in the stem convolution. It adds edge handling for partial blocks, an optional per-batch length input, and larger plane buffers. The trade-off is more plane GEMMs with fewer rows each and a heavier combine step.

New measurement: 1.719 million audio-frames/sec (median of 6 runs). No clear change (+0.9%).

```diff
diff --git a/conformer_amd/_lib.py b/conformer_amd/_lib.py
--- a/conformer_amd/_lib.py
+++ b/conformer_amd/_lib.py
@@ -168,6 +168,9 @@
     "cfm_conv2_wino_plane_elems": (c_int64, [_I, _I, _I, _I]),
     "cfm_pack_conv2_wino_weight_f32": (c_int, [_P, _P, _I, _P]),
     "cfm_subsample_conv2_wino_relu_f32": (c_int, [_P, _P, _P, _P, _P, _I, _I, _I, _I, _P]),
+    "cfm_conv2_wino3_plane_elems": (c_int64, [_I, _I, _I, _I, _I, _I]),
+    "cfm_pack_conv2_wino3_weight_f32": (c_int, [_P, _P, _I, _I, _I, _P]),
+    "cfm_subsample_conv2_wino3_relu_f32": (c_int, [_P, _P, _P, _P, _P, _P, _I, _I, _I, _I, _I, _I, _P]),
 }
 
 
diff --git a/conformer_amd/csrc/conv2_wino_f32.hip b/conformer_amd/csrc/conv2_wino_f32.hip
--- a/conformer_amd/csrc/conv2_wino_f32.hip
+++ b/conformer_amd/csrc/conv2_wino_f32.hip
@@ -20,30 +20,52 @@
     static_for_seq(f, std::make_integer_sequence<int, N>{});
 }
 
-__host__ __device__ constexpr int wino_nt(int a) { return a == 1 ? 1 : 2; }
-__host__ __device__ constexpr int wino_terms(int p) { return wino_nt(p / 3) * wino_nt(p % 3); }
-
+enum { WK1 = 0, WK2 = 1, WK1P = 2 };
+struct WinoDimPat { int kind, d0, d1, d2; float sgn; };
+__host__ __device__ constexpr int wino_np(int R) { return R == 2 ? 3 : 5; }
+__host__ __device__ constexpr WinoDimPat wino_dim_pat(int R, int a) {
+    if (R == 2) return a == 1 ? WinoDimPat{WK1, 2, 2, 2, 0.f} : WinoDimPat{WK2, 2 * a, 2, 1 + a, -1.f};
+    return a == 0 ? WinoDimPat{WK2, 0, 4, 1, -1.f} : a == 1 ? WinoDimPat{WK1P, 2, 4, 2, 1.f} : a == 2 ? WinoDimPat{WK1P, 2, 4, 2, -1.f}
+         : a == 3 ? WinoDimPat{WK2, 6, 2, 5, -1.f} : WinoDimPat{WK1, 3, 3, 3, 0.f};
+}
+__host__ __device__ constexpr int wino_nt(int R, int a) { return wino_dim_pat(R, a).kind == WK2 ? 2 : 1; }
+__host__ __device__ constexpr int wino_terms(int RT, int RF, int p) { return wino_nt(RT, p / wino_np(RF)) * wino_nt(RF, p % wino_np(RF)); }
+__host__ __device__ constexpr int wino_feed(int R, int a, int r) {
+    if (R == 2) return a == r || a == r + 1;
+    return r == 0 ? a <= 2 : r == 1 ? (a == 1 || a == 4 ? 1 : a == 2 ? -1 : 0) : (a >= 1 && a <= 3);
+}
+
+__host__ __device__ constexpr int wino_blocks(int R, int a, int n) {
+    const int rem = n % R;
+    const bool skip = R == 2 ? (a == 2 && rem == 1) : ((a == 3 && rem != 0) || (a == 4 && rem == 1));
+    return (n + R - 1) / R - (skip ? 1 : 0);
+}
+__host__ __device__ constexpr bool wino_edge_d4(int R, int a, int n) { return R == 3 && a <= 2 && n % 3 == 1; }
+
+struct WinoPat { unsigned tm, p, woff; };
 struct WinoArgs {
     const float* h1; const float* w; float* planes;
+    const int64_t* t2_len;
     int64_t M;
     unsigned h1_bytes;
-    int T1, F1, C, TI, TJ, nb;
-    int odd_t, odd_f;
+    int T1, F1, C, T2, F2, TI, TJ, nb;
     unsigned tiles_n;
     unsigned grp_blk[4];
-    unsigned grp_tm[3][4];
-    unsigned grp_pat[3];
+    unsigned grp_first[4];
+    WinoPat pat[25];
 };
 
 
-template <int ST, int SF>
-__device__ __forceinline__ void wino_tile(const WinoArgs& g, int p, int64_t m0, int n0, float* lds) {
-    constexpr int BM = 256, BN = 256, WN = 4, TM = 4, TN = 2, BK = 16, LDSR = BK + 4, NT = ST * SF, SPC = 2 * NT;
-    constexpr int NPX = (ST == 2 ? 2 : 1) * (SF == 2 ? 2 : 1);
+template <int RT, int RF, int KT, int KF>
+__device__ __forceinline__ void wino_tile(const WinoArgs& g, const WinoPat& e, int64_t m0, int n0, float* lds) {
+    constexpr int BM = 256, BN = 256, WN = 4, TM = 4, TN = 2, BK = 16, LDSR = BK + 4;
+    constexpr int ST = KT == WK2 ? 2 : 1, SF = KF == WK2 ? 2 : 1, NT = ST * SF, SPC = 2 * NT;
+    constexpr int NPX = (KT != WK1 ? 2 : 1) * (KF != WK1 ? 2 : 1);
+    constexpr bool AT = RT == 3 && KT != WK1, AF = RF == 3 && KF != WK1;
     float* As = lds;
     float* Bs = lds + 2 * BM * LDSR;
-    const int a = p / 3, b = p - 3 * (p / 3);
-    const int sg_t = a >> 1, sg_f = b >> 1;
+    const int p = (int)e.p, a = p / wino_np(RF), b = p - wino_np(RF) * a;
+    const WinoDimPat dt = wino_dim_pat(RT, a), df = wino_dim_pat(RF, b);
 
     const int tid = threadIdx.x, lane = tid & 63;
     const int wave = __builtin_amdgcn_readfirstlane(tid >> 6);
@@ -53,8 +75,10 @@
     constexpr int CPR = BK / 4, RPP = 512 / CPR, PA = BM / RPP, PB = BN / RPP;
     const int chunk = tid & (CPR - 1), srow = tid / CPR;
     unsigned row_off[PA];
-    const int TJp = g.TJ - (b == 2 ? g.odd_f : 0);
-    const int64_t pos_per_b = (int64_t)(g.TI - (a == 2 ? g.odd_t : 0)) * TJp, Mp = g.nb * pos_per_b;
+    bool zt[PA], zf[PA];
+    const int TIp = wino_blocks(RT, a, g.T2), TJp = wino_blocks(RF, b, g.F2);
+    const bool ef = AF && wino_edge_d4(RF, b, g.F2);
+    const int64_t pos_per_b = (int64_t)TIp * TJp, Mp = g.nb * pos_per_b;
 #pragma unroll
     for (int i = 0; i < PA; ++i) {
         int64_t m = m0 + srow + RPP * i;
@@ -62,24 +86,29 @@
         const int64_t bb = m / pos_per_b;
         const int r = (int)(m - bb * pos_per_b);
         const int ib = r / TJp, jb = r - ib * TJp;
-        row_off[i] = (unsigned)((((bb * g.T1 + 4 * ib) * g.F1 + 4 * jb) * (int64_t)g.C + chunk * 4) * 4);
+        row_off[i] = (unsigned)((((bb * g.T1 + 2 * RT * ib) * g.F1 + 2 * RF * jb) * (int64_t)g.C + chunk * 4) * 4);
+        zt[i] = false;
+        if constexpr (AT) {
+            const int n = g.t2_len ? (int)min(max(g.t2_len[bb], (int64_t)0), (int64_t)g.T2) : g.T2;
+            zt[i] = wino_edge_d4(RT, a, n) && ib == n / 3;
+        }
+        zf[i] = ef && jb == g.TJ - 1;
     }
     const __amdgpu_buffer_rsrc_t h1_rsrc = __builtin_amdgcn_make_buffer_rsrc(const_cast<float*>(g.h1), (short)0, (int)g.h1_bytes, 0x00020000);
-    const unsigned pix_t[3] = {(unsigned)((ST == 2 ? 4 * sg_t : 2) * g.F1 * g.C * 4), (unsigned)(2 * g.F1 * g.C * 4),
-                               (unsigned)((1 + 2 * sg_t) * g.F1 * g.C * 4)};
-    const unsigned pix_f[3] = {(unsigned)((SF == 2 ? 4 * sg_f : 2) * g.C * 4), (unsigned)(2 * g.C * 4), (unsigned)((1 + 2 * sg_f) * g.C * 4)};
-    int64_t woff = 0;
-    for (int q = 0; q < p; ++q) woff += wino_terms(q);
+    const unsigned line = (unsigned)(g.F1 * g.C * 4);
+    const unsigned pix_t[3] = {dt.d0 * line, dt.d1 * line, dt.d2 * line};
+    const unsigned pix_f[3] = {(unsigned)(df.d0 * g.C * 4), (unsigned)(df.d1 * g.C * 4), (unsigned)(df.d2 * g.C * 4)};
+    const float sg_t = dt.sgn, sg_f = df.sgn;
     const int K = NT * g.C;
-    const __amdgpu_buffer_rsrc_t w_rsrc = __builtin_amdgcn_make_buffer_rsrc(const_cast<float*>(g.w + woff * g.C * g.C), (short)0,
+    const __amdgpu_buffer_rsrc_t w_rsrc = __builtin_amdgcn_make_buffer_rsrc(const_cast<float*>(g.w + (int64_t)e.woff * g.C * g.C), (short)0,
                                                                             K * g.C * 4, 0x00020000);
     const unsigned w_off = (unsigned)(((n0 + srow) * K + chunk * 4) * 4), w_step = (unsigned)(RPP * K * 4);
 
     f32x4 raw[PA][NPX], rb[PB];
     auto load_tile = [&](auto U_, int c32, int half) __attribute__((always_inline)) {
         constexpr int U = decltype(U_)::value, UT = U / SF, UF = U % SF;
-        constexpr int NXT = (ST == 2 && UT == 0) ? 2 : 1, NYF = (SF == 2 && UF == 0) ? 2 : 1;
-        constexpr int X1 = ST == 2 ? (UT == 0 ? 0 : 2) : 0, Y1 = SF == 2 ? (UF == 0 ? 0 : 2) : 0;
+        constexpr int NXT = (KT == WK1P || (KT == WK2 && UT == 0)) ? 2 : 1, NYF = (KF == WK1P || (KF == WK2 && UF == 0)) ? 2 : 1;
+        constexpr int X1 = (KT == WK2 && UT == 1) ? 2 : 0, Y1 = (KF == WK2 && UF == 1) ? 2 : 0;
         const unsigned ci4 = (unsigned)(32 * c32 + 16 * half) * 4;
 #pragma unroll
         for (int x = 0; x < NXT; ++x)
@@ -87,22 +116,33 @@
             for (int y = 0; y < NYF; ++y) {
                 const unsigned po = pix_t[X1 + x] + pix_f[Y1 + y] + ci4;
 #pragma unroll
-                for (int i = 0; i < PA; ++i)
-                    raw[i][x * NYF + y] = __builtin_bit_cast(f32x4, __builtin_amdgcn_raw_buffer_load_b128(h1_rsrc, row_off[i], po, 0));
+                for (int i = 0; i < PA; ++i) {
+                    const bool edge = (AT && x == 1 && zt[i]) || (AF && y == 1 && zf[i]);
+                    raw[i][x * NYF + y] = __builtin_bit_cast(f32x4, __builtin_amdgcn_raw_buffer_load_b128(h1_rsrc, edge ? g.h1_bytes : row_off[i], po, 0));
+                }
             }
         const unsigned k4 = (unsigned)(NT * 32 * c32 + 32 * U + 16 * half) * 4;
 #pragma unroll
         for (int i = 0; i < PB; ++i) rb[i] = __builtin_bit_cast(f32x4, __builtin_amdgcn_raw_buffer_load_b128(w_rsrc, w_off, k4 + w_step * i, 0));
+    };
+    auto comb_t = [&](f32x4 q0, f32x4 q1) __attribute__((always_inline)) {
+        if constexpr (KT == WK2) return q0 - q1;
+        else { f32x4 v; _Pragma("unroll") for (int c = 0; c < 4; ++c) v[c] = __builtin_fmaf(sg_t, q0[c], q1[c]); return v; }
+    };
+    auto comb_f = [&](f32x4 q0, f32x4 q1) __attribute__((always_inline)) {
+        if constexpr (KF == WK2) return q0 - q1;
+        else { f32x4 v; _Pragma("unroll") for (int c = 0; c < 4; ++c) v[c] = __builtin_fmaf(sg_f, q0[c], q1[c]); return v; }
     };
     auto store_tile = [&](auto U_, int buf) __attribute__((always_inline)) {
         constexpr int U = decltype(U_)::value, UT = U / SF, UF = U % SF;
-        constexpr int NXT = (ST == 2 && UT == 0) ? 2 : 1, NYF = (SF == 2 && UF == 0) ? 2 : 1;
+        constexpr int NXT = (KT == WK1P || (KT == WK2 && UT == 0)) ? 2 : 1, NYF = (KF == WK1P || (KF == WK2 && UF == 0)) ? 2 : 1;
 #pragma unroll
         for (int i = 0; i < PA; ++i) {
             const f32x4* px = raw[i];
             f32x4 v;
-            if constexpr (NXT == 2 && NYF == 2) v = (px[0] - px[1]) - (px[2] - px[3]);
-            else if constexpr (NXT * NYF == 2) v = px[0] - px[1];
+            if constexpr (NXT == 2 && NYF == 2) v = comb_t(comb_f(px[0], px[1]), comb_f(px[2], px[3]));
+            else if constexpr (NXT == 2) v = comb_t(px[0], px[1]);
+            else if constexpr (NYF == 2) v = comb_f(px[0], px[1]);
             else v = px[0];
             *reinterpret_cast<f32x4*>(As + (buf * BM + srow + RPP * i) * LDSR + chunk * 4) = v;
         }
@@ -164,6 +204,7 @@
                                                                                         lds + wave * 32 * (32 * TN + 4));
 }
 
+template <int RT, int RF>
 __global__ __launch_bounds__(512, 2) void conv2_wino_gemm_kernel(const WinoArgs g) {
     constexpr int LDS_STAGE = 2 * (256 + 256) * 20;
     static_assert(8 * 32 * (32 * 2 + 4) <= LDS_STAGE, "the row-major epilogue scratch must fit the staging buffers");
@@ -172,29 +213,42 @@
     const int grp = bid < g.grp_blk[1] ? 0 : (bid < g.grp_blk[2] ? 1 : 2);
     const unsigned local = bid - g.grp_blk[grp], per_xcd = (g.grp_blk[grp + 1] - g.grp_blk[grp]) / 8;
     unsigned tile = (local & 7u) * per_xcd + (local >> 3);
+    const unsigned first = g.grp_first[grp], n = g.grp_first[grp + 1] - first;
     unsigned k = 0, lo = 0;
-    for (; k < 4; ++k) {
-        const unsigned seg = (g.grp_tm[grp][k] - lo) * (4 - k) * g.tiles_n;
+    for (; k < n; ++k) {
+        const unsigned t = g.pat[first + k].tm;
+        const unsigned seg = (t - lo) * (n - k) * g.tiles_n;
         if (tile < seg) break;
         tile -= seg;
-        lo = g.grp_tm[grp][k];
+        lo = t;
     }
-    if (k == 4) return;
+    if (k == n) return;
     const unsigned tn = tile % g.tiles_n, rest = tile / g.tiles_n;
-    const unsigned pi = k + rest % (4 - k), tm = lo + rest / (4 - k);
-    const int p = (int)((g.grp_pat[grp] >> (4 * pi)) & 15u);
-    const int64_t m0 = (int64_t)tm * 256;
+    const WinoPat e = g.pat[first + k + rest % (n - k)];
+    const int64_t m0 = (int64_t)(lo + rest / (n - k)) * 256;
     const int n0 = (int)tn * 256;
-    const int nta = wino_nt(p / 3), ntb = wino_nt(p % 3);
-    if (nta == 2 && ntb == 2) wino_tile<2, 2>(g, p, m0, n0, lds);
-    else if (nta == 2) wino_tile<2, 1>(g, p, m0, n0, lds);
-    else if (ntb == 2) wino_tile<1, 2>(g, p, m0, n0, lds);
-    else wino_tile<1, 1>(g, p, m0, n0, lds);
-}
-
+    const int kt = wino_dim_pat(RT, (int)e.p / wino_np(RF)).kind, kf = wino_dim_pat(RF, (int)e.p % wino_np(RF)).kind;
+    if (kt == WK2) {
+        if (kf == WK2) wino_tile<RT, RF, WK2, WK2>(g, e, m0, n0, lds);
+        else if (RF == 3 && kf == WK1P) wino_tile<RT, RF, WK2, RF == 3 ? WK1P : WK1>(g, e, m0, n0, lds);
+        else wino_tile<RT, RF, WK2, WK1>(g, e, m0, n0, lds);
+    } else if (RT == 3 && kt == WK1P) {
+        constexpr int KP = RT == 3 ? WK1P : WK1;
+        if (kf == WK2) wino_tile<RT, RF, KP, WK2>(g, e, m0, n0, lds);
+        else if (RF == 3 && kf == WK1P) wino_tile<RT, RF, KP, RF == 3 ? WK1P : WK1>(g, e, m0, n0, lds);
+        else wino_tile<RT, RF, KP, WK1>(g, e, m0, n0, lds);
+    } else {
+        if (kf == WK2) wino_tile<RT, RF, WK1, WK2>(g, e, m0, n0, lds);
+        else if (RF == 3 && kf == WK1P) wino_tile<RT, RF, WK1, RF == 3 ? WK1P : WK1>(g, e, m0, n0, lds);
+        else wino_tile<RT, RF, WK1, WK1>(g, e, m0, n0, lds);
+    }
+}
+
+template <int RT, int RF>
 __global__ __launch_bounds__(256) void conv2_wino_combine_kernel(const float* __restrict__ planes, const float* __restrict__ b2,
                                                                  float* __restrict__ h2, int64_t M, int T2, int F2, int TI,
                                                                  int TJ, int C) {
+    constexpr int NA = wino_np(RT), NB = wino_np(RF);
     const int c4n = C / 4;
     const int64_t idx = (int64_t)blockIdx.x * blockDim.x + threadIdx.x;
     if (idx >= M * c4n) return;
@@ -205,38 +259,56 @@
     const int r = (int)(m - bb * per_b);
     const int ib = r / TJ, jb = r - ib * TJ;
     const int64_t plane = M * (int64_t)C;
-    const int TIs = TI - (T2 & 1), TJs = TJ - (F2 & 1);
-    f32x4 P[9];
-#pragma unroll
-    for (int q = 0; q < 9; ++q) {
-        const bool st = q / 3 == 2, sf = q % 3 == 2;
-        const int64_t mq = (bb * (st ? TIs : TI) + ib) * (sf ? TJs : TJ) + jb;
+    f32x4 P[NA * NB];
+    static_for<NA * NB>([&](auto Q_) __attribute__((always_inline)) {
+        constexpr int q = decltype(Q_)::value;
+        const int TIq = wino_blocks(RT, q / NB, T2), TJq = wino_blocks(RF, q % NB, F2);
+        const int64_t mq = (bb * TIq + ib) * TJq + jb;
         P[q] = f32x4{0.f, 0.f, 0.f, 0.f};
-        if ((!st || ib < TIs) && (!sf || jb < TJs))
-            P[q] = __builtin_nontemporal_load(reinterpret_cast<const f32x4*>(planes + q * plane + mq * C + c));
-    }
+        if (ib < TIq && jb < TJq) P[q] = __builtin_nontemporal_load(reinterpret_cast<const f32x4*>(planes + q * plane + mq * C + c));
+    });
     const f32x4 bias = *reinterpret_cast<const f32x4*>(b2 + c);
-#pragma unroll
-    for (int rt = 0; rt < 2; ++rt) {
-        const int t2 = 2 * ib + rt;
-        if (t2 >= T2) continue;
-        const f32x4 u0 = P[3 * rt + 0] + P[3 * rt + 1], u1 = P[3 * rt + 1] + P[3 * rt + 2];
-        const f32x4 v0 = P[3 * rt + 3] + P[3 * rt + 4], v1 = P[3 * rt + 4] + P[3 * rt + 5];
-#pragma unroll
-        for (int s = 0; s < 2; ++s) {
-            const int f2 = 2 * jb + s;
-            if (f2 >= F2) continue;
-            const f32x4 y = (s == 0 ? u0 + v0 : u1 + v1) + bias;
-            f32x4 o;
-#pragma unroll
-            for (int e = 0; e < 4; ++e) o[e] = fmaxf(y[e], 0.f);
-            *reinterpret_cast<f32x4*>(h2 + (((bb * T2 + t2) * F2) + f2) * (int64_t)C + c) = o;
-        }
-    }
-}
-
-__global__ __launch_bounds__(256) void pack_conv2_wino_kernel(const float* __restrict__ w2, float* __restrict__ wp, int C) {
-    const int p = blockIdx.y, nt = wino_terms(p);
+    static_for<RT * RF>([&](auto O_) __attribute__((always_inline)) {
+        constexpr int rt = decltype(O_)::value / RF, s = decltype(O_)::value % RF;
+        const int t2 = RT * ib + rt, f2 = RF * jb + s;
+        if (t2 >= T2 || f2 >= F2) return;
+        f32x4 y{0.f, 0.f, 0.f, 0.f};
+        bool first_a = true;
+        static_for<NA>([&](auto A_) __attribute__((always_inline)) {
+            constexpr int a = decltype(A_)::value, sa = wino_feed(RT, a, rt);
+            if constexpr (sa != 0) {
+                f32x4 u{0.f, 0.f, 0.f, 0.f};
+                bool first_b = true;
+                static_for<NB>([&](auto B_) __attribute__((always_inline)) {
+                    constexpr int b = decltype(B_)::value, sb = wino_feed(RF, b, s);
+                    if constexpr (sb != 0) {
+                        u = first_b ? P[a * NB + b] : (sb > 0 ? u + P[a * NB + b] : u - P[a * NB + b]);
+                        first_b = false;
+                    }
+                });
+                y = first_a ? u : (sa > 0 ? y + u : y - u);
+                first_a = false;
+            }
+        });
+        y = y + bias;
+        f32x4 o;
+#pragma unroll
+        for (int e = 0; e < 4; ++e) o[e] = fmaxf(y[e], 0.f);
+        *reinterpret_cast<f32x4*>(h2 + (((bb * T2 + t2) * F2) + f2) * (int64_t)C + c) = o;
+    });
+}
+
+__device__ __forceinline__ int wino_taps(int R, int pat, int term, int (&tp)[2], double (&cf)[2]) {
+    cf[0] = cf[1] = 1.0;
+    if (R == 2 && pat == 1) { tp[0] = 0; tp[1] = 2; return 2; }
+    if (R == 3 && (pat == 1 || pat == 2)) { tp[0] = 0; tp[1] = 2; cf[0] = 0.5; cf[1] = pat == 1 ? 0.5 : -0.5; return 2; }
+    if (R == 3 && pat == 4) { tp[0] = 1; return 1; }
+    tp[0] = term == 0 ? (pat == 0 ? 0 : 2) : 1;
+    return 1;
+}
+__global__ __launch_bounds__(256) void pack_conv2_wino_kernel(const float* __restrict__ w2, float* __restrict__ wp, int C, int RT,
+                                                              int RF) {
+    const int p = blockIdx.y, nt = wino_terms(RT, RF, p);
     const int64_t idx = (int64_t)blockIdx.x * blockDim.x + threadIdx.x;
     const int64_t K = (int64_t)nt * C;
     if (idx >= K * C) return;
@@ -244,54 +316,36 @@
     const int k = (int)(idx - co * K);
     const int c32 = k / (32 * nt), rem = k - c32 * 32 * nt, u = rem / 32, ci = 32 * c32 + (rem & 31);
     int64_t off = 0;
-    for (int q = 0; q < p; ++q) off += wino_terms(q);
-    const int a = p / 3, b = p % 3, sfn = wino_nt(b);
+    for (int q = 0; q < p; ++q) off += wino_terms(RT, RF, q);
+    const int a = p / wino_np(RF), b = p % wino_np(RF), sfn = wino_nt(RF, b);
     const int ut = u / sfn, uf = u % sfn;
-    auto taps = [](int pat, int term, int (&tp)[2]) {
-        if (pat == 1) { tp[0] = 0; tp[1] = 2; return 2; }
-        tp[0] = term == 0 ? 2 * (pat >> 1) : 1;
-        return 1;
-    };
     int tt[2], tf[2];
-    const int ntt = taps(a, ut, tt), ntf = taps(b, uf, tf);
+    double ct[2], cf[2];
+    const int ntt = wino_taps(RT, a, ut, tt, ct), ntf = wino_taps(RF, b, uf, tf, cf);
     double s = 0.0;
     const float* wc = w2 + (co * C + ci) * 9;
     for (int x = 0; x < ntt; ++x)
-        for (int y = 0; y < ntf; ++y) s += (double)wc[tf[y] * 3 + tt[x]];
+        for (int y = 0; y < ntf; ++y) s += (ct[x] * cf[y]) * (double)wc[tf[y] * 3 + tt[x]];
     wp[off * C * C + idx] = (float)s;
 }
 
-}
-
-extern "C" int64_t cfm_conv2_wino_plane_elems(int B, int F1, int T1, int C) {
-    if (B <= 0 || F1 < 3 || T1 < 3 || C <= 0) return 0;
-    const int64_t TI = ((T1 - 1) / 2 + 1) / 2, TJ = ((F1 - 1) / 2 + 1) / 2;
-    return 9 * (int64_t)B * TI * TJ * C;
-}
-
-extern "C" int cfm_pack_conv2_wino_weight_f32(const float* w2, float* wp, int C, cfm_stream_t stream) {
-    CFM_REQUIRE(w2 && wp, CFM_ERR_NULL);
-    CFM_REQUIRE(C > 0 && C % 32 == 0, CFM_ERR_BAD_SHAPE);
-    const int64_t most = 4 * (int64_t)C * C;
-    hipLaunchKernelGGL(pack_conv2_wino_kernel, dim3((unsigned)((most + 255) / 256), 9), dim3(256), 0,
-                       static_cast<hipStream_t>(stream), w2, wp, C);
-    return cfm_launch_status();
-}
-
-extern "C" int cfm_subsample_conv2_wino_relu_f32(const float* h1, const float* wp, const float* b2, float* planes, float* h2,
-                                                 int B, int F1, int T1, int C, cfm_stream_t stream) {
+constexpr bool wino_scheme_ok(int rt, int rf) { return (rt == 2 || rt == 3) && (rf == 2 || rf == 3); }
+
+template <int RT, int RF>
+int wino_conv2_relu(const float* h1, const float* wp, const float* b2, float* planes, float* h2, const int64_t* t2_len, int B,
+                    int F1, int T1, int C, cfm_stream_t stream) {
     CFM_REQUIRE(h1 && wp && b2 && planes && h2, CFM_ERR_NULL);
     CFM_REQUIRE(B > 0 && F1 >= 3 && T1 >= 3, CFM_ERR_BAD_SHAPE);
     CFM_REQUIRE(C > 0 && C % 256 == 0, CFM_ERR_UNSUPPORTED);
     CFM_REQUIRE(CFM_ALIGNED16(h1) && CFM_ALIGNED16(wp) && CFM_ALIGNED16(b2) && CFM_ALIGNED16(planes) && CFM_ALIGNED16(h2),
                 CFM_ERR_ALIGN);
+    constexpr int NA = wino_np(RT), NB = wino_np(RF), NP = NA * NB;
     const int64_t utt_bytes = (int64_t)T1 * F1 * C * 4, limit = (1LL << 32) - (1LL << 26);
-    CFM_REQUIRE(utt_bytes <= limit && 5LL * F1 * C * 4 < (1LL << 26), CFM_ERR_UNSUPPORTED);
+    CFM_REQUIRE(utt_bytes <= limit && (2LL * RT + 1) * F1 * C * 4 < (1LL << 26), CFM_ERR_UNSUPPORTED);
     const int T2 = (T1 - 1) / 2, F2 = (F1 - 1) / 2;
     WinoArgs g{};
     g.w = wp;
-    g.T1 = T1; g.F1 = F1; g.C = C; g.TI = (T2 + 1) / 2; g.TJ = (F2 + 1) / 2;
-    g.odd_t = T2 & 1; g.odd_f = F2 & 1;
+    g.T1 = T1; g.F1 = F1; g.C = C; g.T2 = T2; g.F2 = F2; g.TI = (T2 + RT - 1) / RT; g.TJ = (F2 + RF - 1) / RF;
     g.tiles_n = (unsigned)(C / 256);
     const int64_t per_b = (int64_t)g.TI * g.TJ;
     const int group = (int)std::min<int64_t>(B, limit / utt_bytes);
@@ -300,35 +354,76 @@
         const int nb = std::min(group, B - b0);
         g.h1 = h1 + b0 * (utt_bytes / 4);
         g.h1_bytes = (unsigned)(nb * utt_bytes);
+        g.t2_len = t2_len ? t2_len + b0 : nullptr;
         g.M = nb * per_b;
         g.nb = nb;
-        g.planes = planes + 9 * (b0 * per_b) * C;
-        static const int group_pat[3][4] = {{0, 2, 6, 8}, {1, 7, 3, 5}, {-1, -1, -1, 4}};
+        g.planes = planes + NP * (b0 * per_b) * C;
+        unsigned n = 0;
         g.grp_blk[0] = 0;
         for (int q = 0; q < 3; ++q) {
-            int pat[4];
-            unsigned tm[4], total = 0;
-            for (int i = 0; i < 4; ++i) {
-                const int p = group_pat[q][i];
-                const int64_t Mp = p < 0 ? 0 : (int64_t)nb * (g.TI - (p / 3 == 2 ? g.odd_t : 0)) * (g.TJ - (p % 3 == 2 ? g.odd_f : 0));
-                const unsigned t = (unsigned)((Mp + 255) / 256);
-                int j = i;
-                for (; j > 0 && tm[j - 1] > t; --j) { tm[j] = tm[j - 1]; pat[j] = pat[j - 1]; }
-                tm[j] = t; pat[j] = p < 0 ? 0 : p;
-                total += t;
-            }
-            g.grp_pat[q] = 0;
-            for (int i = 0; i < 4; ++i) { g.grp_tm[q][i] = tm[i]; g.grp_pat[q] |= (unsigned)pat[i] << (4 * i); }
+            const unsigned first = g.grp_first[q] = n;
+            unsigned total = 0;
+            for (int pass = 0; pass < 2; ++pass)
+                for (int p = 0, woff = 0; p < NP; woff += wino_terms(RT, RF, p), ++p) {
+                    const int a = p / NB, b = p % NB;
+                    if (wino_terms(RT, RF, p) != 4 >> q || (q == 1 ? (wino_nt(RT, a) == 2) == (pass == 1) : pass == 1)) continue;
+                    const int64_t Mp = (int64_t)nb * wino_blocks(RT, a, T2) * wino_blocks(RF, b, F2);
+                    const unsigned t = (unsigned)((Mp + 255) / 256);
+                    unsigned j = n++;
+                    for (; j > first && g.pat[j - 1].tm > t; --j) g.pat[j] = g.pat[j - 1];
+                    g.pat[j] = WinoPat{t, (unsigned)p, (unsigned)woff};
+                    total += t;
+                }
             g.grp_blk[q + 1] = g.grp_blk[q] + (total * g.tiles_n + 7) / 8 * 8;
         }
-        hipLaunchKernelGGL(conv2_wino_gemm_kernel, dim3(g.grp_blk[3]), dim3(512), 0, s, g);
+        g.grp_first[3] = n;
+        hipLaunchKernelGGL((conv2_wino_gemm_kernel<RT, RF>), dim3(g.grp_blk[3]), dim3(512), 0, s, g);
         int st = cfm_launch_status();
         if (st) return st;
         const int64_t threads = g.M * (C / 4);
-        hipLaunchKernelGGL(conv2_wino_combine_kernel, dim3((unsigned)((threads + 255) / 256)), dim3(256), 0, s, g.planes, b2,
-                           h2 + (int64_t)b0 * T2 * F2 * C, g.M, T2, F2, g.TI, g.TJ, C);
+        hipLaunchKernelGGL((conv2_wino_combine_kernel<RT, RF>), dim3((unsigned)((threads + 255) / 256)), dim3(256), 0, s, g.planes,
+                           b2, h2 + (int64_t)b0 * T2 * F2 * C, g.M, T2, F2, g.TI, g.TJ, C);
         st = cfm_launch_status();
         if (st) return st;
     }
     return 0;
 }
+
+}
+
+extern "C" int64_t cfm_conv2_wino3_plane_elems(int B, int F1, int T1, int C, int rt, int rf) {
+    if (B <= 0 || F1 < 3 || T1 < 3 || C <= 0 || !wino_scheme_ok(rt, rf)) return 0;
+    const int64_t T2 = (T1 - 1) / 2, F2 = (F1 - 1) / 2;
+    return wino_np(rt) * wino_np(rf) * (int64_t)B * ((T2 + rt - 1) / rt) * ((F2 + rf - 1) / rf) * C;
+}
+
+extern "C" int cfm_pack_conv2_wino3_weight_f32(const float* w2, float* wp, int C, int rt, int rf, cfm_stream_t stream) {
+    CFM_REQUIRE(w2 && wp, CFM_ERR_NULL);
+    CFM_REQUIRE(C > 0 && C % 32 == 0, CFM_ERR_BAD_SHAPE);
+    CFM_REQUIRE(wino_scheme_ok(rt, rf), CFM_ERR_UNSUPPORTED);
+    const int64_t most = 4 * (int64_t)C * C;
+    hipLaunchKernelGGL(pack_conv2_wino_kernel, dim3((unsigned)((most + 255) / 256), wino_np(rt) * wino_np(rf)), dim3(256), 0,
+                       static_cast<hipStream_t>(stream), w2, wp, C, rt, rf);
+    return cfm_launch_status();
+}
+
+extern "C" int cfm_subsample_conv2_wino3_relu_f32(const float* h1, const float* wp, const float* b2, float* planes, float* h2,
+                                                  const int64_t* t2_len, int B, int F1, int T1, int C, int rt, int rf,
+                                                  cfm_stream_t stream) {
+    CFM_REQUIRE(wino_scheme_ok(rt, rf), CFM_ERR_UNSUPPORTED);
+    if (rt == 2) return rf == 2 ? wino_conv2_relu<2, 2>(h1, wp, b2, planes, h2, nullptr, B, F1, T1, C, stream)
+                                : wino_conv2_relu<2, 3>(h1, wp, b2, planes, h2, nullptr, B, F1, T1, C, stream);
+    return rf == 2 ? wino_conv2_relu<3, 2>(h1, wp, b2, planes, h2, t2_len, B, F1, T1, C, stream)
+                   : wino_conv2_relu<3, 3>(h1, wp, b2, planes, h2, t2_len, B, F1, T1, C, stream);
+}
+
+extern "C" int64_t cfm_conv2_wino_plane_elems(int B, int F1, int T1, int C) { return cfm_conv2_wino3_plane_elems(B, F1, T1, C, 2, 2); }
+
+extern "C" int cfm_pack_conv2_wino_weight_f32(const float* w2, float* wp, int C, cfm_stream_t stream) {
+    return cfm_pack_conv2_wino3_weight_f32(w2, wp, C, 2, 2, stream);
+}
+
+extern "C" int cfm_subsample_conv2_wino_relu_f32(const float* h1, const float* wp, const float* b2, float* planes, float* h2,
+                                                 int B, int F1, int T1, int C, cfm_stream_t stream) {
+    return wino_conv2_relu<2, 2>(h1, wp, b2, planes, h2, nullptr, B, F1, T1, C, stream);
+}
diff --git a/conformer_amd/model/utils/convolution.py b/conformer_amd/model/utils/convolution.py
--- a/conformer_amd/model/utils/convolution.py
+++ b/conformer_amd/model/utils/convolution.py
@@ -103,17 +103,20 @@
             return ops.subsampled_lengths(lengths)
         return torch.div(torch.div(lengths - 1, 2, rounding_mode="floor") - 1, 2, rounding_mode="floor")
 
-    def channel_last(self, x: torch.Tensor) -> torch.Tensor:
+    def channel_last(self, x: torch.Tensor, out_len: Optional[torch.Tensor] = None) -> torch.Tensor:
         if ag.needs_grad(self, x):
             if x.requires_grad:
                 raise NotImplementedError("ConvolutionSubsampling: the gradient w.r.t. the input spectrogram is not "
                                           "built (the reference never needs it: the input is data)")
             return ag.SubsampleStemFn.apply(x, self.conv_1.weight, self.conv_1.bias, self.conv_2.weight, self.conv_2.bias)
         w2p = self._packs.get("w2p", (self.conv_2.weight,), lambda: ops.pack_conv2_weight(self.conv_2.weight))
-        w2w = None
+        w2w, scheme = None, (2, 2)
         if ops.conv2_winograd_ok(self.conv_2.weight.shape[0]):
-            w2w = self._packs.get("w2w", (self.conv_2.weight,), lambda: ops.pack_conv2_wino_weight(self.conv_2.weight))
-        return ops.subsample_stem(x, self.conv_1.weight, self.conv_1.bias, w2p, self.conv_2.bias, w2w=w2w)
+            scheme = ops.conv2_wino_scheme(self.conv_2.weight.shape[0], (x.shape[1] - 1) // 2)
+            w2w = self._packs.get("w2w", (self.conv_2.weight,), lambda: ops.pack_conv2_wino_weight(self.conv_2.weight, scheme),
+                                  extra=scheme)
+        return ops.subsample_stem(x, self.conv_1.weight, self.conv_1.bias, w2p, self.conv_2.bias, w2w=w2w, scheme=scheme,
+                                  t2_len=out_len)
 
     def forward(self, x: torch.Tensor, lengths: Optional[torch.Tensor] = None) -> Tuple[torch.Tensor, Optional[torch.Tensor]]:
         h = self.channel_last(x)
diff --git a/conformer_amd/ops.py b/conformer_amd/ops.py
--- a/conformer_amd/ops.py
+++ b/conformer_amd/ops.py
@@ -712,12 +712,33 @@
     return bool(_CONV2_WINOGRAD and C % 256 == 0 and not mfma16_prec() and not _fp32_planes)
 
 
-def pack_conv2_wino_weight(w2: torch.Tensor) -> torch.Tensor:
+def _parse_wino_scheme(s) -> tuple:
+    rt, rf = (int(c) for c in s) if isinstance(s, str) else s
+    if rt not in (2, 3) or rf not in (2, 3):
+        raise ValueError(f"conv2 Winograd scheme {s!r}: outputs per block are 2 or 3 per axis, e.g. '32'")
+    return rt, rf
+
+
+_CONV2_WINO_SCHEME = _parse_wino_scheme(__import__("os").environ.get("CONFORMER_AMD_CONV2_WINO_SCHEME", "32"))
+
+
+def set_conv2_wino_scheme(scheme) -> tuple:
+    global _CONV2_WINO_SCHEME
+    prev, _CONV2_WINO_SCHEME = _CONV2_WINO_SCHEME, _parse_wino_scheme(scheme)
+    return prev
+
+
+def conv2_wino_scheme(C: int, F1: int) -> tuple:
+    return _CONV2_WINO_SCHEME
+
+
+def pack_conv2_wino_weight(w2: torch.Tensor, scheme=(2, 2)) -> torch.Tensor:
     w2 = _req(w2, "conv_2.weight")
     C = w2.shape[0]
-    out = torch.empty(25 * C * C, device=w2.device, dtype=torch.float32)
-    _lib.check(_lib.load().cfm_pack_conv2_wino_weight_f32(w2.data_ptr(), out.data_ptr(), C, _stream()),
-               "cfm_pack_conv2_wino_weight_f32")
+    rt, rf = _parse_wino_scheme(scheme)
+    out = torch.empty((2 * rt + 1) * (2 * rf + 1) * C * C, device=w2.device, dtype=torch.float32)
+    _lib.check(_lib.load().cfm_pack_conv2_wino3_weight_f32(w2.data_ptr(), out.data_ptr(), C, rt, rf, _stream()),
+               "cfm_pack_conv2_wino3_weight_f32")
     return out
 
 
@@ -729,7 +750,7 @@
     return out
 
 
-def subsample_stem(x: torch.Tensor, w1, b1, w2p, b2, w2w=None) -> torch.Tensor:
+def subsample_stem(x: torch.Tensor, w1, b1, w2p, b2, w2w=None, scheme=(2, 2), t2_len=None) -> torch.Tensor:
     x = _req(x, "x"); w1 = _req(w1, "conv_1.weight"); b1 = _req(b1, "conv_1.bias")
     w2p = _req(w2p, "packed conv_2.weight"); b2 = _req(b2, "conv_2.bias")
     B, F, T = x.shape
@@ -749,10 +770,19 @@
                                                     _stream()), "cfm_subsample_conv1_relu_f32")
         h2 = torch.empty(B, T2, F2 * C, device=x.device, dtype=torch.float32)
         if w2w is not None and conv2_winograd_ok(C):
-            planes = torch.empty(int(lib.cfm_conv2_wino_plane_elems(B, F1, T1, C)), device=x.device, dtype=torch.float32)
-            _lib.check(lib.cfm_subsample_conv2_wino_relu_f32(h1.data_ptr(), _req(w2w, "Winograd conv_2.weight").data_ptr(),
-                                                             b2.data_ptr(), planes.data_ptr(), h2.data_ptr(), B, F1, T1, C,
-                                                             _stream()), "cfm_subsample_conv2_wino_relu_f32")
+            rt, rf = scheme
+            w2w = _req(w2w, "Winograd conv_2.weight")
+            if w2w.numel() != (2 * rt + 1) * (2 * rf + 1) * C * C:
+                raise _lib.ConformerHipError(f"subsample_stem: the Winograd pack does not belong to scheme {scheme}")
+            if t2_len is not None and rt == 3:
+                t2_len = t2_len.to(device=x.device, dtype=torch.int64).contiguous()
+                if t2_len.numel() != B:
+                    raise _lib.ConformerHipError(f"subsample_stem: t2_len must have {B} values")
+            planes = torch.empty(int(lib.cfm_conv2_wino3_plane_elems(B, F1, T1, C, rt, rf)), device=x.device, dtype=torch.float32)
+            _lib.check(lib.cfm_subsample_conv2_wino3_relu_f32(h1.data_ptr(), w2w.data_ptr(), b2.data_ptr(), planes.data_ptr(),
+                                                              h2.data_ptr(), t2_len.data_ptr() if t2_len is not None and rt == 3 else 0,
+                                                              B, F1, T1, C, rt, rf, _stream()),
+                       "cfm_subsample_conv2_wino3_relu_f32")
             return h2
     _conv2_relu(lib, h1, w2p, b2, h2, B, F1, T1, C)
     return h2
diff --git a/include/conformer_hip.h b/include/conformer_hip.h
--- a/include/conformer_hip.h
+++ b/include/conformer_hip.h
@@ -102,6 +102,10 @@
 int cfm_pack_conv2_wino_weight_f32(const float* w2, float* wwp, int C, cfm_stream_t stream);
 int cfm_subsample_conv2_wino_relu_f32(const float* h1, const float* wwp, const float* b2, float* planes, float* h2,
                                       int B, int F1, int T1, int C, cfm_stream_t stream);
+int64_t cfm_conv2_wino3_plane_elems(int B, int F1, int T1, int C, int rt, int rf);
+int cfm_pack_conv2_wino3_weight_f32(const float* w2, float* wwp, int C, int rt, int rf, cfm_stream_t stream);
+int cfm_subsample_conv2_wino3_relu_f32(const float* h1, const float* wwp, const float* b2, float* planes, float* h2,
+                                       const int64_t* t2_len, int B, int F1, int T1, int C, int rt, int rf, cfm_stream_t stream);
 
 #define CFM_PREC_F32 0
 #define CFM_PREC_BF16 1
```
